# DRCL-USC/Hector_Simulation

Measured on NVIDIA H100. Metric: QP solves/sec (batched MPC ticks), horizon N=10, higher is better.
Workload: dtype f32 assembly (bit-exact to reference arithmetic) / f64 solve

## Files before the change

### hector_simulation_b200/csrc/hmpc_capi.cu

```cuda
#include <cuda_runtime.h>
#include <dlfcn.h>
#include <unistd.h>

#include <algorithm>
#include <chrono>
#include <cstddef>
#include <cstdint>
#include <cstdio>
#include <cstdlib>
#include <atomic>
#include <condition_variable>
#include <cstring>
#include <ctime>
#include <functional>
#include <mutex>
#include <string>
#include <thread>
#include <vector>

#include "../../include/hector_mpc_b200.h"
#include "hmpc_device.cuh"
#include "hmpc_chain.h"

static_assert(sizeof(update_data_t) == 3016, "update_data_t must match convexMPC_interface.h:19-37");
static_assert(sizeof(problem_setup) == 16, "problem_setup must match convexMPC_interface.h:11-17");

namespace {

thread_local std::string g_err;

bool cuda_fail(cudaError_t e, const char* what)
{
  if (e == cudaSuccess) return false;
  g_err = std::string(what) + ": " + cudaGetErrorString(e);
  return true;
}
#define CK(call)                          \
  do {                                    \
    if (cuda_fail((call), #call)) return HMPC_ERR_CUDA; \
  } while (0)

class HostPool {
 public:
  explicit HostPool(int nworkers)
  {
    for (int i = 0; i < nworkers; i++) workers_.emplace_back([this, i] { run(i); });
  }
  ~HostPool()
  {
    {
      std::lock_guard<std::mutex> lk(m_);
      stop_ = true;
      gen_++;
    }
    cv_.notify_all();
    for (auto& t : workers_) t.join();
  }
  int size() const { return (int)workers_.size() + 1; }
  void parallel(const std::function<void(int, int)>& fn)
  {
    const int np = size();
    if (np == 1) { fn(0, 1); return; }
    fn_ = &fn;
    pending_.store(np - 1, std::memory_order_release);
    {
      std::lock_guard<std::mutex> lk(m_);
      gen_++;
    }
    cv_.notify_all();
    fn(0, np);
    while (pending_.load(std::memory_order_acquire) != 0) std::this_thread::yield();
  }

 private:
  void run(int idx)
  {
    unsigned seen = 0;
    for (;;) {
      bool got = false;
      const auto t0 = std::chrono::steady_clock::now();
      while (std::chrono::steady_clock::now() - t0 < std::chrono::microseconds(50)) {
        if (gen_relaxed() != seen) { got = true; break; }
      }
      if (!got) {
        std::unique_lock<std::mutex> lk(m_);
        cv_.wait(lk, [&] { return gen_ != seen; });
      }
      {
        std::lock_guard<std::mutex> lk(m_);
        seen = gen_;
        if (stop_) return;
      }
      (*fn_)(idx + 1, size());
      pending_.fetch_sub(1, std::memory_order_acq_rel);
    }
  }
  unsigned gen_relaxed()
  {
    std::lock_guard<std::mutex> lk(m_);
    return gen_;
  }
  std::vector<std::thread> workers_;
  std::mutex m_;
  std::condition_variable cv_;
  unsigned gen_ = 0;
  bool stop_ = false;
  const std::function<void(int, int)>* fn_ = nullptr;
  std::atomic<int> pending_{0};
};

constexpr int NCHUNK = 4;

constexpr int EAGER_SLOT = 0, CAPTURE_SLOT = 1, CLS_SLOTS = 2;
static_assert(CAPTURE_SLOT < CLS_SLOTS, "d_cls holds CLS_SLOTS slots");

struct ResultRows { float* wrench; int* status; float* tau; size_t bytes; };

using hmpc::ClassCfg;

}

struct hmpc_ctx {
  int device = 0, max_batch = 0, horizon = 0, rec_stride = 0, sm_count = 0;
  hmpc::SolverSettings cfg;
  ClassCfg cls[3];
  int ncls = 0;
  ClassCfg ref{};
  ClassCfg mcls[3], mref{};
  float* d_mq = nullptr;
  size_t mq_off[4] = {};
  unsigned char* h_multi = nullptr;
  float* d_smtraj = nullptr;
  unsigned char* h_smulti = nullptr;
  int* d_ref = nullptr;
  unsigned char* d_rec = nullptr;
  unsigned char* d_out = nullptr;
  int* d_status = nullptr;
  int* d_counts = nullptr;
  int* d_lists = nullptr;
  int* d_cls = nullptr;
  unsigned char* h_mask = nullptr;
  unsigned eager_calls = 0;
  unsigned char* h_rec = nullptr;
  unsigned char* h_out = nullptr;
  unsigned char* d_states = nullptr;
  unsigned char* h_states = nullptr;
  int* h_cls = nullptr;
  cudaStream_t stream = nullptr;
  cudaStream_t xstream[3] = {nullptr, nullptr, nullptr};
  HostPool* pool = nullptr;
  void* nccl = nullptr;
  int shard_rank = 0, shard_world = 1;
  float* shard_buf[2] = {nullptr, nullptr};
  unsigned shard_tick = 0;
  cudaStream_t gstream = nullptr;
  cudaEvent_t solved = nullptr, gathered[2] = {nullptr, nullptr};
  int* d_ws = nullptr;
  int warm_start = 1;
  int* d_shift = nullptr;
  int* h_shift = nullptr;
  double* h_pred = nullptr;
  unsigned char* h_cert = nullptr;
  struct Pin { char* base; size_t bytes; };
  struct Run { uintptr_t lo, hi; };
  std::vector<Pin> pins;
  std::vector<Run> runs;
  bool pinned(const void* p, size_t bytes) const
  {
    const char* q = static_cast<const char*>(p);
    for (const Pin& r : pins)
      if (q >= r.base && q + bytes <= r.base + r.bytes) return true;
    return false;
  }
  size_t row_bytes() const { return (size_t)12 * horizon * 4 + 4 + 40; }
  ResultRows rows(unsigned char* base, int b0, int nb, bool tau = true) const
  {
    const size_t nw = (size_t)12 * horizon;
    unsigned char* p = base + (size_t)b0 * row_bytes();
    return {reinterpret_cast<float*>(p), reinterpret_cast<int*>(p + (size_t)nb * nw * 4),
            tau ? reinterpret_cast<float*>(p + (size_t)nb * (nw * 4 + 4)) : nullptr, (size_t)nb * (nw * 4 + 4 + (tau ? 40 : 0))};
  }
};

namespace {

cudaError_t prep_class(const ClassCfg& c, int* occ)
{
  cudaError_t e = cudaErrorInvalidDeviceFunction;
#define HMPC_PREP(ID, NT, MB, NF, CL) HMPC_PREP_K(ID, (hmpc::hmpc_solve_kernel<NT, MB, NF, CL>), NT)
#define HMPC_PREP_MQ(ID, NT, MB, NF, CL) HMPC_PREP_K(ID, (hmpc::hmpc_solve_kernel<NT, MB, NF, CL, true>), NT)
#define HMPC_PREP_K(ID, KERNEL, NT)                                                                    \
  case ID: {                                                                                           \
    auto k = KERNEL;                                                                                   \
    e = cudaFuncSetAttribute(k, cudaFuncAttributeMaxDynamicSharedMemorySize, 227 * 1024);              \
    if (e == cudaSuccess) e = cudaOccupancyMaxActiveBlocksPerMultiprocessor(occ, k, NT, c.smem);       \
    break;                                                                                             \
  }
  switch (c.variant) { HMPC_VARIANTS(HMPC_PREP) HMPC_MQ_VARIANTS(HMPC_PREP_MQ) }
#undef HMPC_PREP
#undef HMPC_PREP_MQ
#undef HMPC_PREP_K
  return e;
}

bool pdl_enabled()
{
  static const bool on = !(getenv("HMPC_PDL") && atoi(getenv("HMPC_PDL")) == 0);
  return on;
}

template <typename... KArgs, typename... Args>
cudaError_t launch_chain(void (*kernel)(KArgs...), dim3 grid, dim3 block, size_t smem, cudaStream_t st, bool pdl, Args... args)
{
  cudaLaunchConfig_t cfg{};
  cfg.gridDim = grid;
  cfg.blockDim = block;
  cfg.dynamicSmemBytes = smem;
  cfg.stream = st;
  cudaLaunchAttribute attr[1];
  attr[0].id = cudaLaunchAttributeProgrammaticStreamSerialization;
  attr[0].val.programmaticStreamSerializationAllowed = 1;
  cfg.attrs = attr;
  cfg.numAttrs = pdl ? 1 : 0;
  return cudaLaunchKernelEx(&cfg, kernel, args...);
}

int build_classes(hmpc_ctx* c)
{
  c->ncls = hmpc::plan_classes(c->horizon, c->cls, c->ref);
  if (c->ncls == 0 || hmpc::plan_classes(c->horizon, c->mcls, c->mref, true) != c->ncls) {
    g_err = "horizon too long for the built kernel variants";
    return HMPC_ERR_ARG;
  }
  size_t mq_rows = 0;
  for (int i = 0; i <= 2 * c->ncls + 1; i++) {
    const bool mq = i > c->ncls;
    const int j = mq ? i - c->ncls - 1 : i;
    ClassCfg& k = mq ? (j < c->ncls ? c->mcls[j] : c->mref) : (j < c->ncls ? c->cls[j] : c->ref);
    int occ = 0;
    if (cuda_fail(prep_class(k, &occ), "kernel attribute/occupancy (is this an sm_90a device?)")) return HMPC_ERR_CUDA;
    if (occ < 1) { g_err = "kernel does not fit on this device"; return HMPC_ERR_CUDA; }
    k.grid_cap = occ * c->sm_count;
    if (mq) {
      c->mq_off[j < c->ncls ? j : 3] = mq_rows * hmpc::mq_scratch_floats(c->horizon);
      mq_rows += hmpc::mq_scratch_ctas(k, c->max_batch);
    }
  }
  if (cuda_fail(cudaMalloc(&c->d_mq, mq_rows * hmpc::mq_scratch_floats(c->horizon) * sizeof(float)), "cudaMalloc multi-query scratch"))
    return HMPC_ERR_CUDA;
  return HMPC_OK;
}

long long* g_dbg_clk = nullptr;

int launch_class(const hmpc_ctx* c, int cls, const hmpc::SolveIO& io, const hmpc::ChainLists& lists, int count, cudaStream_t st,
                 bool pdl = false, const hmpc::MultiIO* mq = nullptr)
{
  const ClassCfg& k = cls == hmpc::REFINE_CLASS ? (mq ? c->mref : c->ref) : (mq ? c->mcls[cls] : c->cls[cls]);
  hmpc::KernelArgs ka = mq ? hmpc::multi_launch_args(c->cfg, c->horizon, c->ncls, cls, k, io, lists, *mq)
                           : hmpc::launch_args(c->cfg, c->horizon, c->ncls, cls, k, io, lists);
  ka.dbg_clk = ka.dbg_H ? nullptr : g_dbg_clk;
  const int grid = count < k.grid_cap ? count : k.grid_cap;
  cudaError_t e = cudaErrorInvalidDeviceFunction;
#define HMPC_LAUNCH(ID, NT, MB, NF, CL) \
  case ID: e = launch_chain(hmpc::hmpc_solve_kernel<NT, MB, NF, CL>, dim3(grid), dim3(NT), (size_t)k.smem, st, pdl, ka); break;
#define HMPC_LAUNCH_MQ(ID, NT, MB, NF, CL) \
  case ID: e = launch_chain(hmpc::hmpc_solve_kernel<NT, MB, NF, CL, true>, dim3(grid), dim3(NT), (size_t)k.smem, st, pdl, ka); break;
  switch (k.variant) { HMPC_VARIANTS(HMPC_LAUNCH) HMPC_MQ_VARIANTS(HMPC_LAUNCH_MQ) }
#undef HMPC_LAUNCH
#undef HMPC_LAUNCH_MQ
  CK(e);
  CK(cudaGetLastError());
  return HMPC_OK;
}

int launch_prepare(const hmpc::PrepareArgs& pa, cudaStream_t st, bool pdl)
{
  CK(launch_chain(hmpc::hmpc_prepare_kernel, dim3(hmpc::prepare_grid(pa.batch)), dim3(hmpc::PREPARE_THREADS), 0, st, pdl,
                  pa.states, pa.batch, pa.N, pa.dtMPC, pa.records, pa.rec_stride, pa.list, pa.count));
  CK(cudaGetLastError());
  return HMPC_OK;
}

int launch_prepare_traj(const hmpc::PrepareTrajArgs& pa, cudaStream_t st, bool pdl)
{
  CK(launch_chain(hmpc::hmpc_prepare_traj_kernel, dim3(hmpc::prepare_grid(pa.batch * pa.K)), dim3(hmpc::PREPARE_THREADS), 0, st,
                  pdl, pa.states, pa.batch, pa.K, pa.cmd, pa.N, pa.dtMPC, pa.traj, pa.list, pa.count));
  CK(cudaGetLastError());
  return HMPC_OK;
}

int launch_carry(const unsigned char* mask, int batch, int N, const float* prev, float* cur, cudaStream_t st)
{
  hmpc::hmpc_carry_kernel<<<hmpc::carry_grid(batch, N), hmpc::CARRY_THREADS, 0, st>>>(
      mask, batch, hmpc::carry_row_vecs(N), reinterpret_cast<const float4*>(prev), reinterpret_cast<float4*>(cur));
  CK(cudaGetLastError());
  return HMPC_OK;
}

template <typename T>
int launch_predict(const hmpc_ctx* c, const void* rows, int row_stride, int B, const unsigned char* mask, const T* wrench,
                   T* pred, cudaStream_t st)
{
  hmpc::hmpc_predict_kernel<T><<<hmpc::predict_grid(B), hmpc::PREDICT_THREADS, 0, st>>>(
      static_cast<const unsigned char*>(rows), row_stride, B, c->horizon, c->cfg.dt, mask, wrench, pred);
  CK(cudaGetLastError());
  return HMPC_OK;
}

template <typename T>
int launch_certify(const hmpc_ctx* c, const void* rows, hmpc::RowLayout lay, int B, const unsigned char* mask, const T* wrench,
                   hmpc_certificate_t* cert, T* lambda, cudaStream_t st)
{
  hmpc::hmpc_certify_kernel<T><<<hmpc::certify_grid(B), hmpc::CERT_THREADS, 0, st>>>(
      static_cast<const unsigned char*>(rows), lay, B, c->horizon, c->cfg.dt, c->cfg.f_max, mask, wrench,
      reinterpret_cast<hmpc::CertOut*>(cert), lambda, nullptr);
  CK(cudaGetLastError());
  return HMPC_OK;
}

template <typename T>
int launch_multi_cost(const hmpc_ctx* c, const void* rows, hmpc::RowLayout lay, int B, int K, const unsigned char* mask,
                      const float* traj, const T* wrench, double* cost, cudaStream_t st)
{
  hmpc::hmpc_multi_cost_kernel<T><<<hmpc::multi_cost_grid((long long)B * K), hmpc::PREDICT_THREADS, 0, st>>>(
      static_cast<const unsigned char*>(rows), lay, B, K, c->horizon, c->cfg.dt, mask, traj, wrench, cost);
  CK(cudaGetLastError());
  return HMPC_OK;
}

template <typename T>
int launch_pick(const hmpc_ctx* c, void* records, int B, int K, const unsigned char* mask, const float* traj, const T* wrench,
                const int* status, const double* cost, int* best, float* tau, cudaStream_t st)
{
  hmpc::hmpc_pick_kernel<T><<<hmpc::pick_grid(B), hmpc::PREDICT_THREADS, 0, st>>>(
      static_cast<unsigned char*>(records), c->rec_stride, B, K, c->horizon, c->cfg.f_max, mask, traj, wrench, status, cost, best,
      tau);
  CK(cudaGetLastError());
  return HMPC_OK;
}

}

static_assert(sizeof(hmpc_certificate_t) == sizeof(hmpc::CertOut) && offsetof(hmpc_certificate_t, flags) ==
              offsetof(hmpc::CertOut, flags), "hmpc_certificate_t is the kernel's CertOut");
static_assert(HMPC_CERT_PASS == hmpc::CERT_PASS && HMPC_CERT_NONFINITE == hmpc::CERT_NONFINITE &&
              HMPC_CERT_SWING == hmpc::CERT_SWING && HMPC_CERT_STATIONARITY == hmpc::CERT_STATIONARITY &&
              HMPC_CERT_PRIMAL == hmpc::CERT_PRIMAL && HMPC_CERT_COMPLEMENTARITY == hmpc::CERT_COMPL,
              "certificate flag bits");
static_assert(HMPC_CERT_STATIONARITY_TOL == hmpc::CERT_STAT_TOL && HMPC_CERT_PRIMAL_TOL == hmpc::CERT_PRIMAL_TOL &&
              HMPC_CERT_COMPLEMENTARITY_TOL == hmpc::CERT_COMPL_TOL, "certificate thresholds");
static_assert(sizeof(update_data_t) == 3016 && offsetof(update_data_t, Alpha_K) == 1896 && offsetof(update_data_t, traj) == 168 &&
              offsetof(update_data_t, gait) == 1944, "hmpc_chain.h: update_rows");

HMPC_EXTERNC size_t hmpc_record_bytes(int horizon)
{
  if (horizon < 1 || horizon > 18) return 0;
  size_t b = (size_t)(54 + 12 * horizon) * 4 + (size_t)2 * horizon;
  return (b + 15) / 16 * 16;
}

HMPC_EXTERNC int hmpc_pack_records(const update_data_t* in, int n, int horizon, void* out)
{
  const size_t stride = hmpc_record_bytes(horizon);
  if (!in || !out || n < 0 || stride == 0) { g_err = "hmpc_pack_records: bad argument"; return HMPC_ERR_ARG; }
  unsigned char* o = static_cast<unsigned char*>(out);
  for (int i = 0; i < n; i++, o += stride) {
    const update_data_t& u = in[i];
    if (i + 2 < n) {
      const char* nx = reinterpret_cast<const char*>(&in[i + 2]);
      for (int off = 0; off < (42 + 12 * horizon) * 4; off += 64) __builtin_prefetch(nx + off);
      __builtin_prefetch(nx + offsetof(update_data_t, Alpha_K));
      __builtin_prefetch(nx + offsetof(update_data_t, gait));
    }
    float* f = reinterpret_cast<float*>(o);
    memcpy(f, u.p, 42 * 4);
    memcpy(f + 42, u.Alpha_K, 48);
    memcpy(f + 54, u.traj, (size_t)48 * horizon);
    unsigned char* g = o + (size_t)(54 + 12 * horizon) * 4;
    memcpy(g, u.gait, (size_t)2 * horizon);
    memset(g + 2 * horizon, 0, stride - ((size_t)(54 + 12 * horizon) * 4 + 2 * horizon));
  }
  return HMPC_OK;
}

HMPC_EXTERNC const char* hmpc_last_error(void) { return g_err.c_str(); }

struct Id128 { char b[128]; };
namespace {
struct NcclApi {
  void* h = nullptr;
  int (*GetUniqueId)(void*) = nullptr;
  int (*CommInitRank)(void**, int, Id128, int) = nullptr;
  int (*AllGather)(const void*, void*, size_t, int, void*, cudaStream_t) = nullptr;
  int (*CommDestroy)(void*) = nullptr;
  const char* (*GetErrorString)(int) = nullptr;
};
}
namespace {
NcclApi g_nccl;
bool nccl_load()
{
  if (g_nccl.h) return true;
  void* h = dlopen("libnccl.so.2", RTLD_NOW | RTLD_GLOBAL);
  if (!h) h = dlopen("libnccl.so", RTLD_NOW | RTLD_GLOBAL);
  if (!h) { g_err = std::string("NCCL not found: ") + dlerror(); return false; }
  g_nccl.GetUniqueId = reinterpret_cast<int (*)(void*)>(dlsym(h, "ncclGetUniqueId"));
  g_nccl.CommInitRank = reinterpret_cast<int (*)(void**, int, Id128, int)>(dlsym(h, "ncclCommInitRank"));
  g_nccl.AllGather = reinterpret_cast<int (*)(const void*, void*, size_t, int, void*, cudaStream_t)>(dlsym(h, "ncclAllGather"));
  g_nccl.CommDestroy = reinterpret_cast<int (*)(void*)>(dlsym(h, "ncclCommDestroy"));
  g_nccl.GetErrorString = reinterpret_cast<const char* (*)(int)>(dlsym(h, "ncclGetErrorString"));
// ... 155 lines not shown
  if (!bad) {
    const char* br = getenv("HMPC_BLOCK_ROUNDS");
    if (br) c->cfg.block_rounds = atoi(br);
    if (const char* bm = getenv("HMPC_BLOCK_MIN")) c->cfg.block_min = atoi(bm);
    if (const char* km = getenv("HMPC_KAPPA_MAX")) c->cfg.kappa_max = atof(km);
    if (const char* kr = getenv("HMPC_KAPPA_REFINE")) c->cfg.kappa_refine = atof(kr);
    if (const char* kx = getenv("HMPC_KAPPA_MAX_REFINED")) c->cfg.kappa_max_refined = atof(kx);
    const char* ls = getenv("HMPC_LOCKSTEP");
    if (ls) c->cfg.lockstep = atoi(ls);
    const char* wm = getenv("HMPC_WARM_START");
    if (wm) c->warm_start = atoi(wm);
  }
  if (!bad && max_batch >= 256) {
    const char* e = getenv("HMPC_HOST_THREADS");
    int nt = e ? atoi(e) : 4;
    const int hw = (int)std::thread::hardware_concurrency();
    if (hw > 0 && nt > hw) nt = hw;
    if (nt > 1) c->pool = new HostPool(nt - 1);
  }
  if (bad) {
    std::string keep = g_err;
    hmpc_destroy(c);
    g_err = keep;
    return nullptr;
  }
  return c;
}

HMPC_EXTERNC int hmpc_set_problem(hmpc_ctx* c, const problem_setup* s)
{
  if (!c || !s) { g_err = "hmpc_set_problem: null argument"; return HMPC_ERR_ARG; }
  if (s->horizon != c->horizon) { g_err = "hmpc_set_problem: horizon differs from the context's"; return HMPC_ERR_ARG; }
  c->cfg.dt = s->dt;
  c->cfg.f_max = s->f_max;
  return HMPC_OK;
}

namespace {
int enqueue_solve(hmpc_ctx* c, const hmpc::SolveIO& io, cudaStream_t st, const hmpc::MultiIO* mq = nullptr)
{
  if (io.batch > c->max_batch) { g_err = "batch exceeds the context's capacity"; return HMPC_ERR_ARG; }
  CK(cudaSetDevice(c->device));
  cudaStreamCaptureStatus cap = cudaStreamCaptureStatusNone;
  CK(cudaStreamIsCapturing(st, &cap));
  const bool capturing = cap != cudaStreamCaptureStatusNone;
  const int slot = capturing ? CAPTURE_SLOT : EAGER_SLOT;
  const hmpc::ClassSlot s{c->d_cls + (size_t)slot * hmpc::ClassSlot::cls_slot_ints(c->max_batch), c->max_batch,
                          capturing ? 0 : (int)(c->eager_calls++ & 1u)};
  if (capturing) CK(cudaMemsetAsync(s.base, 0, hmpc::ClassSlot::HEAD_INTS * sizeof(int), st));
  const hmpc::ChainLists lists = hmpc::slot_lists(s, io.mask != nullptr, c->cfg.refine);
  const bool pdl = pdl_enabled();
  if (io.mask) {
    CK(launch_chain(hmpc::hmpc_select_kernel<hmpc::SELECT_THREADS>, dim3(1), dim3(hmpc::SELECT_THREADS), 0, st, pdl, io.mask,
                    io.batch, s.list0(), s.counts()));
    CK(cudaGetLastError());
  }
  if (io.states) {
    if (int rc = launch_prepare(hmpc::prepare_args(c->horizon, io, lists), st, pdl)) return rc;
    if (mq && mq->cmd)
      if (int rc = launch_prepare_traj(hmpc::prepare_traj_args(c->horizon, io, lists, *mq), st, pdl)) return rc;
  }
  const int items = mq ? io.batch * mq->K : io.batch;
  for (int i = 0; i < c->ncls; i++)
    if (int rc = launch_class(c, i, io, lists, i == 0 ? io.batch : items, st, pdl, mq)) return rc;
  if (c->cfg.refine) return launch_class(c, hmpc::REFINE_CLASS, io, lists, items, st, pdl, mq);
  return HMPC_OK;
}

hmpc::SolveIO device_call(const hmpc_ctx* c, const void* d_records, int B, float* d_wrench, int* d_status, float* d_tau, bool warm)
{
  hmpc::SolveIO io;
  io.records = d_records;
  io.batch = B;
  io.wrench = d_wrench;
  io.status = d_status;
  io.tau = d_tau;
  if (warm && c->warm_start) io.ws = c->d_ws, io.warm = true;
  return io;
}

struct Chunk { int b0, nb; cudaStream_t st; hmpc::SolveIO io; int *lists, *d_lists, *ref; };

int enqueue_solve_hostlists(hmpc_ctx* c, const Chunk& ch, bool zero_copy)
{
  int* h_block = ch.lists;
  int* d_block = zero_copy ? h_block : ch.d_lists;
  if (!zero_copy) {
    const size_t ints = h_block[1] > 0 ? hmpc::host_list(h_block, c->max_batch, 1) - h_block + h_block[1] : hmpc::HOST_LIST_HEAD + h_block[0];
    CK(cudaMemcpyAsync(d_block, h_block, ints * sizeof(int), cudaMemcpyHostToDevice, ch.st));
  }
  const hmpc::ChainLists lists = hmpc::host_lists(d_block, c->max_batch, ch.ref, false);
  if (ch.ref) CK(cudaMemsetAsync(lists.ref_count, 0, sizeof(int), ch.st));
  for (int i = 0; i < 2; i++)
    if (h_block[i] > 0)
      if (int rc = launch_class(c, i, ch.io, lists, h_block[i], ch.st)) return rc;
  return HMPC_OK;
}

int enqueue_overflow_retry(hmpc_ctx* c, const Chunk& ch, const int* h_status, const unsigned char* mask)
{
  const int mb = c->max_batch, nb = ch.nb;
  int* h_block = ch.lists;
  std::vector<char> was_cls1(nb, 0);
  for (int j = 0; j < h_block[1]; j++) was_cls1[hmpc::host_list(h_block, mb, 1)[j]] = 1;
  int n[3] = {0, 0, 0};
  for (int i = 0; i < nb; i++) {
    if ((mask && !mask[i]) || HMPC_STATUS_CODE(h_status[i]) != hmpc::ST_WS_CAP) continue;
    const int next = was_cls1[i] ? 2 : 1;
    if (next < c->ncls) hmpc::host_list(h_block, mb, next)[n[next]++] = i;
  }
  h_block[0] = 0;
  h_block[1] = n[1];
  h_block[2] = n[2];
  h_block[3] = 0;
  CK(cudaMemcpyAsync(ch.d_lists, h_block, (hmpc::host_list(h_block, mb, 2) - h_block + n[2]) * sizeof(int), cudaMemcpyHostToDevice, ch.st));
  const hmpc::ChainLists lists = hmpc::host_lists(ch.d_lists, mb, ch.ref, true);
  for (int i = 1; i < c->ncls; i++) {
    const int cnt = (i == 1) ? n[1] : n[1] + n[2];
    if (cnt > 0)
      if (int rc = launch_class(c, i, ch.io, lists, cnt, ch.st)) return rc;
  }
  return HMPC_OK;
}

int enqueue_refine_retry(hmpc_ctx* c, const Chunk& ch)
{
  return launch_class(c, hmpc::REFINE_CLASS, ch.io, hmpc::host_lists(ch.d_lists, c->max_batch, ch.ref, false), ch.nb, ch.st);
}
}

static int check_device_records(const hmpc_ctx* c, const void* d_records, int B, const char* who)
{
  if (B > c->max_batch) { g_err = std::string(who) + ": batch exceeds the context's capacity"; return HMPC_ERR_ARG; }
  if (reinterpret_cast<uintptr_t>(d_records) & 15u) { g_err = std::string(who) + ": d_records must be 16-byte aligned"; return HMPC_ERR_ARG; }
  return HMPC_OK;
}

HMPC_EXTERNC void hmpc_debug_set_clock_buffer(long long* d_buf) { g_dbg_clk = d_buf; }

namespace { int g_fail_next_solves = 0; }
HMPC_EXTERNC void hmpc_debug_fail_next_solves(int n) { g_fail_next_solves = n; }

HMPC_EXTERNC int hmpc_launches_per_solve(const hmpc_ctx* c) { return c ? c->ncls + (c->cfg.refine ? 1 : 0) : 0; }

HMPC_EXTERNC int hmpc_set_refinement(hmpc_ctx* c, int on)
{
  if (!c) { g_err = "hmpc_set_refinement: null context"; return HMPC_ERR_ARG; }
  c->cfg.refine = on ? 1 : 0;
  return HMPC_OK;
}

HMPC_EXTERNC int hmpc_class_config(const hmpc_ctx* c, int cls, int* out)
{
  if (!c || !out || cls < 0 || (cls >= c->ncls && cls != HMPC_REFINEMENT_CLASS)) return HMPC_ERR_ARG;
  const ClassCfg& k = cls == HMPC_REFINEMENT_CLASS ? c->ref : c->cls[cls];
  out[0] = k.threads; out[1] = k.smem; out[2] = k.qmax; out[3] = k.grid_cap; out[4] = k.nb_cap;
  out[5] = 8;
  return HMPC_OK;
}

HMPC_EXTERNC int hmpc_solve_device(hmpc_ctx* c, const void* d_records, int B, float* d_wrench, int* d_status,
                                   void* stream)
{
  if (!c || !d_records || !d_wrench || !d_status || B < 0) { g_err = "hmpc_solve_device: bad argument"; return HMPC_ERR_ARG; }
  if (B == 0) return HMPC_OK;
  if (int rc = check_device_records(c, d_records, B, "hmpc_solve_device")) return rc;
  return enqueue_solve(c, device_call(c, d_records, B, d_wrench, d_status, nullptr, false), static_cast<cudaStream_t>(stream));
}

HMPC_EXTERNC int hmpc_solve_device_ex(hmpc_ctx* c, const void* d_records, int B, float* d_wrench, int* d_status,
                                      float* d_tau, void* stream)
{
  if (!c || !d_records || !d_wrench || !d_status || B < 0) { g_err = "hmpc_solve_device_ex: bad argument"; return HMPC_ERR_ARG; }
  if (B == 0) return HMPC_OK;
  if (int rc = check_device_records(c, d_records, B, "hmpc_solve_device_ex")) return rc;
  return enqueue_solve(c, device_call(c, d_records, B, d_wrench, d_status, d_tau, false), static_cast<cudaStream_t>(stream));
}

HMPC_EXTERNC int hmpc_solve_device_warm(hmpc_ctx* c, const void* d_records, int B, float* d_wrench, int* d_status, float* d_tau,
                                        const int* d_shift, void* stream)
{
  if (!c || !d_records || !d_wrench || !d_status || B < 0) { g_err = "hmpc_solve_device_warm: bad argument"; return HMPC_ERR_ARG; }
  if (B == 0) return HMPC_OK;
  if (int rc = check_device_records(c, d_records, B, "hmpc_solve_device_warm")) return rc;
  hmpc::SolveIO io = device_call(c, d_records, B, d_wrench, d_status, d_tau, true);
  io.shifts = d_shift;
  return enqueue_solve(c, io, static_cast<cudaStream_t>(stream));
}

HMPC_EXTERNC int hmpc_solve_device_masked(hmpc_ctx* c, const void* d_records, int B, const unsigned char* d_mask, float* d_wrench,
                                          int* d_status, float* d_tau, const int* d_shift, void* stream)
{
  if (!c || !d_records || !d_mask || !d_wrench || !d_status || B < 0) {
    g_err = "hmpc_solve_device_masked: bad argument";
    return HMPC_ERR_ARG;
  }
  if (B == 0) return HMPC_OK;
  if (int rc = check_device_records(c, d_records, B, "hmpc_solve_device_masked")) return rc;
  hmpc::SolveIO io = device_call(c, d_records, B, d_wrench, d_status, d_tau, true);
  io.shifts = d_shift;
  io.mask = d_mask;
  return enqueue_solve(c, io, static_cast<cudaStream_t>(stream));
}

HMPC_EXTERNC int hmpc_assemble_device(hmpc_ctx* c, const void* d_records, int B, float* d_H, float* d_g,
                                      float* d_Fblk, float* d_lb, float* d_ub, void* stream)
{
  if (!c || !d_records || !d_H || !d_g || !d_Fblk || !d_lb || !d_ub || B < 0) {
    g_err = "hmpc_assemble_device: bad argument";
    return HMPC_ERR_ARG;
  }
  if (B == 0) return HMPC_OK;
  if (int rc = check_device_records(c, d_records, B, "hmpc_assemble_device")) return rc;
  CK(cudaSetDevice(c->device));
  hmpc::SolveIO io = device_call(c, d_records, B, nullptr, c->d_status, nullptr, false);
  io.dump_H = d_H;
  io.dump_g = d_g;
  io.dump_F = d_Fblk;
  io.dump_lb = d_lb;
  io.dump_ub = d_ub;
  hmpc::ChainLists lists;
  lists.counts = c->d_counts;
  return launch_class(c, c->ncls - 1, io, lists, B, static_cast<cudaStream_t>(stream));
}

static_assert(sizeof(hmpc_state_t) == 352 && offsetof(hmpc_state_t, gait) == 39 * 8, "hmpc_state_t layout (hmpc_prepare_kernel)");

HMPC_EXTERNC int hmpc_prepare_device(hmpc_ctx* c, const hmpc_state_t* d_states, int B, double dtMPC, void* d_records,
                                     void* stream)
{
  if (!c || !d_states || !d_records || B < 0) { g_err = "hmpc_prepare_device: bad argument"; return HMPC_ERR_ARG; }
  if (B == 0) return HMPC_OK;
  CK(cudaSetDevice(c->device));
  hmpc::SolveIO io;
  io.states = d_states;
  io.records = d_records;
  io.batch = B;
  io.dt_mpc = dtMPC;
  return launch_prepare(hmpc::prepare_args(c->horizon, io, hmpc::ChainLists{}), static_cast<cudaStream_t>(stream), false);
}

HMPC_EXTERNC int hmpc_solve_states_device_masked(hmpc_ctx* c, const hmpc_state_t* d_states, int B, const unsigned char* d_mask,
                                                 double dtMPC, void* d_records, float* d_wrench, int* d_status, float* d_tau,
                                                 const int* d_shift, void* stream)
{
  if (!c || !d_states || !d_mask || !d_records || !d_wrench || !d_status || B < 0) {
    g_err = "hmpc_solve_states_device_masked: bad argument";
    return HMPC_ERR_ARG;
  }
  if (B == 0) return HMPC_OK;
  if (int rc = check_device_records(c, d_records, B, "hmpc_solve_states_device_masked")) return rc;
  hmpc::SolveIO io = device_call(c, d_records, B, d_wrench, d_status, d_tau, true);
  io.shifts = d_shift;
  io.mask = d_mask;
  io.states = d_states;
  io.dt_mpc = dtMPC;
  return enqueue_solve(c, io, static_cast<cudaStream_t>(stream));
}

HMPC_EXTERNC int hmpc_predict_device(hmpc_ctx* c, const void* d_records, int B, const unsigned char* d_mask, const float* d_wrench,
                                     float* d_pred, void* stream)
{
  if (!c || !d_records || !d_wrench || !d_pred || B < 0 || B > c->max_batch) {
    g_err = "hmpc_predict_device: bad argument (null pointer or batch > capacity)";
    return HMPC_ERR_ARG;
  }
  if (B == 0) return HMPC_OK;
  CK(cudaSetDevice(c->device));
  return launch_predict(c, d_records, c->rec_stride, B, d_mask, d_wrench, d_pred, static_cast<cudaStream_t>(stream));
}

namespace { int g_predict_in_place = -1; }
HMPC_EXTERNC int hmpc_debug_last_predict_in_place(void) { return g_predict_in_place; }

HMPC_EXTERNC int hmpc_predict_batch(hmpc_ctx* c, const update_data_t* in, int B, const unsigned char* mask, const double* wrench,
                                    double* pred_out)
{
  if (!c || !in || !wrench || !pred_out || B < 0 || B > c->max_batch) {
    g_err = "hmpc_predict_batch: bad argument (null pointer or batch > capacity)";
    return HMPC_ERR_ARG;
  }
  if (B == 0) return HMPC_OK;
  if (mask && std::all_of(mask, mask + B, [](unsigned char m) { return m == 0; })) return HMPC_OK;
  CK(cudaSetDevice(c->device));
  const size_t nw = (size_t)12 * c->horizon, rs = (size_t)c->rec_stride;
  const unsigned char* m = nullptr;
  if (mask) {
    memcpy(c->h_mask, mask, (size_t)B);
    m = c->h_mask;
  }
  auto listed = [&](int i) { return !mask || mask[i] != 0; };
  if (c->pinned(in, (size_t)B * sizeof(update_data_t)) && c->pinned(wrench, B * nw * sizeof(double)) &&
      c->pinned(pred_out, B * nw * sizeof(double))) {
    g_predict_in_place = 1;
    if (int rc = launch_predict(c, in, (int)sizeof(update_data_t), B, m, wrench, pred_out, c->stream)) return rc;
    CK(cudaStreamSynchronize(c->stream));
    return HMPC_OK;
  }
  g_predict_in_place = 0;
  if (!c->h_pred) CK(cudaMallocHost(&c->h_pred, 2 * (size_t)c->max_batch * nw * sizeof(double)));
  double* hw = c->h_pred;
  double* hp = c->h_pred + (size_t)c->max_batch * nw;
  for (int i = 0; i < B; i++)
    if (listed(i)) {
      memcpy(c->h_rec + i * rs, in[i].p, 19 * sizeof(float));
      memcpy(hw + i * nw, wrench + i * nw, nw * sizeof(double));
    }
  if (int rc = launch_predict(c, c->h_rec, c->rec_stride, B, m, hw, hp, c->stream)) return rc;
// ... 835 lines not shown
```

### hector_simulation_b200/csrc/hmpc_chain.h

```cpp
#pragma once
#include <cstddef>

namespace hmpc {

constexpr int MQ_VARIANT = 100;
#define HMPC_VARIANTS(X) \
  X(0, 128, 6, 10, 0)    \
  X(1, 256, 2, 10, 1)    \
  X(20, 64, 1, 0, 3)     \
  X(21, 128, 1, 0, 3)    \
  X(22, 192, 1, 0, 3)    \
  X(23, 256, 1, 0, 3)    \
  X(24, 384, 1, 0, 3)    \
  X(10, 64, 8, 0, 0)     \
  X(11, 128, 6, 0, 0)    \
  X(12, 192, 3, 0, 0)    \
  X(13, 256, 2, 0, 0)    \
  X(14, 384, 1, 0, 0)    \
  X(15, 64, 8, 0, 1)     \
  X(16, 128, 6, 0, 1)    \
  X(17, 192, 3, 0, 1)    \
  X(18, 256, 2, 0, 1)    \
  X(19, 384, 1, 0, 1)
#define HMPC_MQ_VARIANTS(X) \
  X(100, 128, 6, 10, 0) \
  X(101, 256, 2, 10, 1) \
  X(120, 64, 1, 0, 3)   \
  X(121, 128, 1, 0, 3)  \
  X(122, 192, 1, 0, 3)  \
  X(123, 256, 1, 0, 3)  \
  X(124, 384, 1, 0, 3)  \
  X(110, 64, 8, 0, 0)   \
  X(111, 128, 6, 0, 0)  \
  X(112, 192, 3, 0, 0)  \
  X(113, 256, 2, 0, 0)  \
  X(114, 384, 1, 0, 0)  \
  X(115, 64, 8, 0, 1)   \
  X(116, 128, 6, 0, 1)  \
  X(117, 192, 3, 0, 1)  \
  X(118, 256, 2, 0, 1)  \
  X(119, 384, 1, 0, 1)

constexpr int REFINE_CLASS = 3;
constexpr int SMEM_MAX = 226 * 1024;

struct ClassCfg {
  int nb_hi, nb_cap, qmax, threads, smem, grid_cap, variant, tcap;
  Layout L;
};

inline int pick_variant(int N, int kcls, int warps, bool fixed, int* threads, bool mq = false)
{
  int v = -1;
#define HMPC_PICK(ID, NT, MB, NF, CL) \
  if (CL == kcls && NF == 0 && NT >= 32 * warps && (v < 0 || NT < *threads)) v = ID, *threads = NT;
  HMPC_VARIANTS(HMPC_PICK)
#undef HMPC_PICK
#define HMPC_PICK(ID, NT, MB, NF, CL) \
  if (CL == kcls && NF == N && fixed && v >= 0) v = ID, *threads = NT;
  HMPC_VARIANTS(HMPC_PICK)
#undef HMPC_PICK
  return (v >= 0 && mq) ? MQ_VARIANT + v : v;
}

inline int plan_classes(int N, ClassCfg cls[3], ClassCfg& ref, bool mq = false)
{
  const int rs = record_stride(N);
  for (int i = 0; i < 2; i++) {
    ClassCfg& k = cls[i];
    k = ClassCfg{};
    k.nb_cap = k.nb_hi = class_nb_cap(N, i);
    k.variant = pick_variant(N, i, class_warps(N, i), true, &k.threads, mq);
    if (k.variant < 0) return 0;
    k.qmax = class_qmax(N, i);
    k.tcap = class_tcap(N, i);
    k.L = make_layout(N, k.nb_cap, k.qmax, rs, k.threads / 32, k.tcap);
    k.smem = k.L.total;
  }
  ClassCfg& k = cls[2];
  k = cls[1];
  k.variant = pick_variant(N, 1, class_warps(N, 1), false, &k.threads, mq);
  k.qmax = 6 * k.nb_cap;
  k.tcap = 0;
  k.L = make_layout(N, k.nb_cap, k.qmax, rs, k.threads / 32, 0);
  while (k.L.total > SMEM_MAX && k.qmax > cls[1].qmax) {
    k.qmax -= 4;
    k.L = make_layout(N, k.nb_cap, k.qmax, rs, k.threads / 32, 0);
  }
  k.smem = k.L.total;
  const int ncls = k.qmax > cls[1].qmax ? 3 : 2;
  for (int nb = 2 * N;; nb = N) {
    ref = ClassCfg{};
    ref.nb_cap = ref.nb_hi = nb;
    ref.variant = pick_variant(N, REFINE_CLASS, class_warps(N, nb == N ? 0 : 1), false, &ref.threads, mq);
    if (ref.variant < 0) return 0;
    ref.qmax = 6 * nb;
    ref.L = refine_layout(N, nb, ref.qmax, rs, ref.threads / 32);
    while (ref.L.total > SMEM_MAX && ref.qmax > 4) {
      ref.qmax -= 4;
      ref.L = refine_layout(N, nb, ref.qmax, rs, ref.threads / 32);
    }
    ref.smem = ref.L.total;
    if (nb == N || (ref.L.total <= SMEM_MAX && ref.qmax >= class_qmax(N, 1))) break;
  }
  return ncls;
}

struct ClassSlot {
  enum : int { W_WAVE = 3, W_REF = 4, PARITY_INTS = 8, HEAD_INTS = 2 * PARITY_INTS };
  static_assert(W_REF < 5, "the class-0 launch clears 5 words of the next parity");
  int* base;
  int max_batch;
  int par;
  static size_t cls_slot_ints(int max_batch) { return HEAD_INTS + 4 * (size_t)max_batch; }
  int* counts() const { return base + PARITY_INTS * par; }
  int* counts_next() const { return base + PARITY_INTS * (par ^ 1); }
  unsigned* wave() const { return reinterpret_cast<unsigned*>(counts() + W_WAVE); }
  int* ref_count() const { return counts() + W_REF; }
  int* list(int i) const { return base + HEAD_INTS + (size_t)(i - 1) * max_batch; }
  int* ref_list() const { return list(3); }
  int* list0() const { return list(4); }
};

constexpr int HOST_LIST_HEAD = 4;
inline size_t host_lists_ints(int max_batch) { return HOST_LIST_HEAD + 3 * (size_t)max_batch; }
inline int* host_list(int* block, int max_batch, int i) { return block + HOST_LIST_HEAD + (size_t)i * max_batch; }

inline void classify_host(int N, float f_max, int nb_hi, const unsigned char* gait0, size_t gait_stride, int nb, int* block,
                          int max_batch, const unsigned char* mask = nullptr)
{
  for (int w = 0; w < HOST_LIST_HEAD; w++) block[w] = 0;
  for (int i = 0; i < nb; i++) {
    if (mask && !mask[i]) continue;
    int k = 0;
    for (int e = 0; e < 2 * N; e++) {
      const float ub = f_max * (float)gait0[(size_t)i * gait_stride + e];
      k += !(ub < 0.0001f && ub > -0.0001f);
    }
    const int cl = (k <= nb_hi) ? 0 : 1;
    host_list(block, max_batch, cl)[block[cl]++] = i;
  }
}

struct SolverSettings {
  float dt = 0.04f, f_max = 500.f;
  int max_iter = 500;
  double tol_kkt = 1e-9;
  double tol_dep = 1e-11;
  double kappa_max = 1.5e5;
  double kappa_refine = 1.5e4;
  double kappa_max_refined = 1e9;
  int refine = 0;
  int block_rounds = 4;
  int block_min = 2;
  int lockstep = 1;
};

struct SolveIO {
  const void* records = nullptr;
  const void* raw = nullptr;
  const void* states = nullptr;
  double dt_mpc = 0.0;
  int batch = 0;
  float* wrench = nullptr;
  double* wrench64 = nullptr;
  int* status = nullptr;
  float* tau = nullptr;
  int* ws = nullptr;
  bool warm = false;
  int shift = 1;
  const int* shifts = nullptr;
  const unsigned char* mask = nullptr;
  float *dump_H = nullptr, *dump_g = nullptr, *dump_F = nullptr, *dump_lb = nullptr, *dump_ub = nullptr;
};

struct ChainLists {
  int* counts = nullptr;
  int* list[3] = {};
  int* ref_count = nullptr;
  int* ref_list = nullptr;
  int* counts_next = nullptr;
  unsigned* wave = nullptr;
  bool escalate = false;
};

inline ChainLists slot_lists(const ClassSlot& s, bool masked, bool refine)
{
  ChainLists l;
  l.counts = s.counts();
  l.list[0] = masked ? s.list0() : nullptr;
  l.list[1] = s.list(1);
  l.list[2] = s.list(2);
  if (refine) l.ref_count = s.ref_count(), l.ref_list = s.ref_list();
  l.escalate = true;
  l.counts_next = s.counts_next();
  l.wave = s.wave();
  return l;
}

inline ChainLists host_lists(int* block, int max_batch, int* ref, bool escalate)
{
  ChainLists l;
  l.counts = block;
  for (int i = 0; i < 3; i++) l.list[i] = host_list(block, max_batch, i);
  if (ref) l.ref_count = ref, l.ref_list = ref + 1;
  l.escalate = escalate;
  return l;
}

constexpr int PREPARE_THREADS = 64;
inline int prepare_grid(int batch) { return (batch + PREPARE_THREADS - 1) / PREPARE_THREADS; }
struct PrepareArgs {
  const unsigned char* states;
  int batch, N;
  double dtMPC;
  unsigned char* records;
  int rec_stride;
  const int* list;
  const int* count;
};
inline PrepareArgs prepare_args(int N, const SolveIO& io, const ChainLists& lists)
{
  PrepareArgs pa{};
  pa.states = static_cast<const unsigned char*>(io.states);
  pa.batch = io.batch;
  pa.N = N;
  pa.dtMPC = io.dt_mpc;
  pa.records = static_cast<unsigned char*>(const_cast<void*>(io.records));
  pa.rec_stride = record_stride(N);
  pa.list = lists.list[0];
  pa.count = lists.list[0] ? lists.counts : nullptr;
  return pa;
}

inline int carry_row_vecs(int N) { return 3 * N; }
inline int carry_grid(int batch, int N)
{
  return (int)(((long long)batch * carry_row_vecs(N) + CARRY_THREADS - 1) / CARRY_THREADS);
}

inline int predict_grid(int batch)
{
  constexpr int warps = PREDICT_THREADS / 32;
  return (batch + warps - 1) / warps;
}

inline int certify_grid(int batch)
{
  constexpr int warps = CERT_THREADS / 32;
  return (batch + warps - 1) / warps;
}
inline RowLayout packed_rows(int N) { return RowLayout{record_stride(N), 42 * 4, 54 * 4, (54 + 12 * N) * 4}; }
inline RowLayout update_rows() { return RowLayout{3016, 1896, 168, 1944}; }

inline KernelArgs launch_args(const SolverSettings& S, int N, int ncls, int cls, const ClassCfg& k, const SolveIO& io,
                              const ChainLists& lists)
{
  const bool refinement = cls == REFINE_CLASS;
// ... 94 lines not shown
```

### hector_simulation_b200/csrc/hmpc_device.cuh

```cuda
#pragma once
#include <cuda_runtime.h>
#include <stdint.h>

namespace hmpc {

#define FM(a, b) __fmul_rn((a), (b))
#define FA(a, b) __fadd_rn((a), (b))
#define FS(a, b) __fsub_rn((a), (b))
#define FD(a, b) __fdiv_rn((a), (b))
#define DM(a, b) __dmul_rn((a), (b))
#define DA(a, b) __dadd_rn((a), (b))
#define DS(a, b) __dsub_rn((a), (b))

enum : int { ST_OK = 0, ST_ITER_CAP = 1, ST_WS_CAP = 2, ST_INFEASIBLE = 3, ST_NOT_SPD = 4 };

struct Layout {
  int H, gq, x0, nrm, fz, blk, keep, misc, uni;
  int T, Sv, lam, dv, rr, wsl, zb;
  int Pb, Ws;
  int rec, x0f, Acd, Bcd, P, M, dd, fbl, comb;
  int Hc, gc;
  int total;
};

__host__ __device__ constexpr int align16(int x) { return (x + 15) & ~15; }

__host__ __device__ constexpr int toff(int I, int J) { return (I * (I + 1) / 2 + J) * 64; }

__host__ __device__ constexpr Layout make_layout(int N, int nb_cap, int qmax, int rec_stride, int nwarps, int tcap)
{
  Layout L{};
  const int n = 6 * nb_cap;
  const int nt8 = (n + 7) / 8, ntile = nt8 * (nt8 + 1) / 2;
  int o = 0;
  L.H = o;    o += ntile * 64 * 8;
  L.gq = o;   o += nt8 * 8 * 8;
  L.x0 = o;   o += n * 8;
  L.nrm = o;  o += 2 * 10 * 6 * 8;
  L.fz = o;   o += align16(nb_cap * 8);
  L.blk = o;  o += align16((nb_cap + 2 * N) * 4);
  L.keep = o; o += 64;
  L.misc = o; o += 512;
  L.uni = o;
  int s = L.uni;
  const int ns = qmax + 1;
  L.T = s;    s += (tcap + 1) * n * 8;
  L.Sv = s;   s += ns * (ns + 1) / 2 * 8;
  L.lam = s;  s += ns * 8;
  L.dv = s;   s += 2 * (ns + 2) * 8;
  L.rr = s;   s += ns * 8;
  L.wsl = s;  s += align16(ns * 4);
  L.zb = L.gq;
  const int sweep_bytes = 2 * nt8 * 64 * 8 + nwarps * 2 * 64 * 8;
  int w = (sweep_bytes <= ntile * 64 * 8) ? L.H : L.uni;
  L.Pb = w;   w += 2 * nt8 * 64 * 8;
  L.Ws = w;   w += nwarps * 2 * 64 * 8;
  if (sweep_bytes <= ntile * 64 * 8) w = L.uni;
  int a = L.uni;
  L.rec = a;  a += align16(rec_stride);
  L.x0f = a;  a += 16 * 4;
  L.Acd = a;  a += align16(169 * 4);
  L.Bcd = a;  a += align16(156 * 4);
  L.P = a;    a += 2 * align16(169 * 4);
  L.M = a;    a += align16(N * 72 * 4);
  L.dd = a;   a += align16(12 * N * 4);
  L.fbl = a;  a += 192 * 4;
  L.comb = a; a += align16(4 * N * 4);
  int m = s > a ? s : a;
  m = m > w ? m : w;
  L.total = align16(m);
  return L;
}

__host__ __device__ constexpr Layout refine_layout(int N, int nb_cap, int qmax, int rec_stride, int nwarps)
{
  Layout L = make_layout(N, nb_cap, qmax, rec_stride, nwarps, 0);
  const int n = 6 * nb_cap, nt8 = (n + 7) / 8;
  L.Hc = L.total;
  L.gc = L.Hc + align16(nt8 * (nt8 + 1) / 2 * 64 * 4);
  L.total = align16(L.gc + n * 8);
  return L;
}

__host__ __device__ constexpr int record_stride(int N) { return align16((54 + 12 * N) * 4 + 2 * N); }

__host__ __device__ constexpr int class_nb_cap(int N, int cls) { return N * (1 + cls); }
__host__ __device__ constexpr int class_tcap(int N, int cls)
{
  const int n = 6 * class_nb_cap(N, cls);
  const int t = cls == 0 ? N + 4 : (N <= 10 ? 31 : 0);
  return t < n ? t : n;
}
__host__ __device__ constexpr int class_qmax(int N, int cls)
{
  const int n = 6 * class_nb_cap(N, cls);
  const int q = cls == 0 ? 2 * N + 4 : (N <= 10 ? 31 : 96);
  return q < n ? q : n;
}
__host__ __device__ constexpr int class_warps(int N, int cls)
{
  const int nb = class_nb_cap(N, cls), n = 6 * nb, nt8 = (n + 7) / 8;
  const int w_sweep = (nt8 + 1) / 2, w_rows = (nb + 2) / 3;
  return w_sweep > w_rows ? w_sweep : w_rows;
}
__host__ __device__ constexpr Layout class_layout(int N, int cls, int nwarps)
{
  return make_layout(N, class_nb_cap(N, cls), class_qmax(N, cls), record_stride(N), nwarps, class_tcap(N, cls));
}

struct KernelArgs {
  const unsigned char* records;
  const unsigned char* raw_records;
  int rec_stride;
  int batch;
  int horizon;
  float dt;
  float f_max;
  const int* list;
  int* counts;
  int cls;
  int* esc_list;
  int split_nb;
  int* ref_list;
  int* ref_count;
  int* counts_next;
  unsigned* wave_sync;
  int nb_cap;
  int qmax;
  int max_iter;
  double tol_kkt;
  double tol_dep;
  int tcap;
  int block_rounds;
  int block_min;
  double kappa_max;
  int warm_start;
  int ws_shift;
  const int* ws_shifts;
  int* ws_state;
  float* wrench;
  double* wrench64;
  int* status;
  float* dbg_H;
  float* dbg_g;
  float* dbg_F;
  float* dbg_lb;
  float* dbg_ub;
  float* tau;
  long long* dbg_clk;
  Layout L;
  const float* mq_traj;
  int mq_k;
  float* mq_scratch;
};

__host__ __device__ constexpr int mq_scratch_floats(int N) { return 16 + 172 + 156 + 12 + 72 * N; }

__device__ __forceinline__ uint32_t smem_u32(const void* p) { return (uint32_t)__cvta_generic_to_shared(p); }

__device__ __forceinline__ void pdl_trigger() { asm volatile("griddepcontrol.launch_dependents;" ::: "memory"); }
__device__ __forceinline__ void pdl_wait() { asm volatile("griddepcontrol.wait;" ::: "memory"); }

__device__ __forceinline__ void mbar_init(uint64_t* bar, int count)
{
  asm volatile("mbarrier.init.shared::cta.b64 [%0], %1;" ::"r"(smem_u32(bar)), "r"(count));
}
__device__ __forceinline__ void mbar_expect_tx(uint64_t* bar, uint32_t bytes)
{
  asm volatile("mbarrier.arrive.expect_tx.shared::cta.b64 _, [%0], %1;" ::"r"(smem_u32(bar)), "r"(bytes) : "memory");
}
__device__ __forceinline__ void mbar_wait(uint64_t* bar, uint32_t phase)
{
  asm volatile(
      "{\n\t.reg .pred p;\n\t"
      "WAIT_%=:\n\t"
      "mbarrier.try_wait.parity.shared::cta.b64 p, [%0], %1;\n\t"
      "@p bra DONE_%=;\n\t"
      "bra WAIT_%=;\n\t"
      "DONE_%=:\n\t}" ::"r"(smem_u32(bar)), "r"(phase) : "memory");
}
__device__ __forceinline__ void bulk_g2s(void* dst, const void* src, uint32_t bytes, uint64_t* bar)
{
  asm volatile("cp.async.bulk.shared::cluster.global.mbarrier::complete_tx::bytes [%0], [%1], %2, [%3];" ::"r"(
                   smem_u32(dst)),
               "l"(src), "r"(bytes), "r"(smem_u32(bar))
               : "memory");
}

__device__ __forceinline__ int leg_of(int c12) { return (c12 / 3) & 1; }
__device__ __forceinline__ int loc_of(int c12) { return (c12 % 3) + (c12 >= 6 ? 3 : 0); }
__device__ __forceinline__ int col12_of(int leg, int loc) { return (loc < 3) ? 3 * leg + loc : 6 + 3 * leg + (loc - 3); }

__device__ __forceinline__ void hput(float* Hf, int i, int j, float v)
{
  const int I = i >> 3, J = j >> 3;
  Hf[toff(I, J) + ((i & 7) << 3) + (j & 7)] = v;
  if (I == J) Hf[toff(I, I) + ((j & 7) << 3) + (i & 7)] = v;
}

__device__ __forceinline__ double hinv_dot6(const double* Hi, int i, int j0, const double* v)
{
  const int I = i >> 3, ir = i & 7;
  const int J0 = j0 >> 3, c0 = j0 & 7, J1 = J0 + 1;
  const int sA = (I >= J0) ? 1 : 8, sB = (I >= J1) ? 1 : 8;
  const double* pA = Hi + ((I >= J0) ? toff(I, J0) + ir * 8 + c0 : toff(J0, I) + c0 * 8 + ir);
  const double* pB = Hi + ((I >= J1) ? toff(I, J1) + ir * 8 : toff(J1, I) + ir) - (8 - c0) * sB;
  double acc = 0.0;
#pragma unroll
  for (int c = 0; c < 6; c++) acc = fma((c0 + c < 8) ? pA[c * sA] : pB[c * sB], v[c], acc);
  return acc;
}

__device__ __forceinline__ double hinv_rowdot(const double* Hi, int i, int nt8, const double* v)
{
  const int I = i >> 3, ir = i & 7;
  double acc0 = 0.0, acc1 = 0.0;
  for (int J = 0; J < nt8; J++) {
    const double* p = Hi + ((J <= I) ? toff(I, J) + ir * 8 : toff(J, I) + ir);
    const int st = (J <= I) ? 1 : 8;
    const double* vv = v + 8 * J;
#pragma unroll
    for (int c = 0; c < 8; c += 2) {
      acc0 = fma(p[c * st], vv[c], acc0);
      acc1 = fma(p[(c + 1) * st], vv[c + 1], acc1);
    }
  }
  return acc0 + acc1;
}

__device__ __forceinline__ double dot6(const double* a, const double* b)
{
  double acc = a[0] * b[0];
#pragma unroll
  for (int c = 1; c < 6; c++) acc = fma(a[c], b[c], acc);
  return acc;
}

__device__ __forceinline__ void dmma884(double& c0, double& c1, double a, double b)
{
  asm("mma.sync.aligned.m8n8k4.row.col.f64.f64.f64.f64 {%0,%1}, {%2}, {%3}, {%0,%1};" : "+d"(c0), "+d"(c1) : "d"(a), "d"(b));
}

__device__ __forceinline__ int frag_pair(int lane) { return ((lane & 2) << 4) + ((lane >> 2) << 2) + ((lane & 1) << 1); }
__device__ __forceinline__ int frag_elem(int r, int c) { return ((c >> 2) << 5) + (r << 2) + (c & 3); }

__device__ __forceinline__ float cof3(const float* m, int i, int j)
{
  int i1 = (i + 1) % 3, i2 = (i + 2) % 3, j1 = (j + 1) % 3, j2 = (j + 2) % 3;
  return FS(FM(m[i1 * 3 + j1], m[i2 * 3 + j2]), FM(m[i1 * 3 + j2], m[i2 * 3 + j1]));
}
__device__ inline void inverse3(const float* m, float* inv)
{
  float c00 = cof3(m, 0, 0), c10 = cof3(m, 1, 0), c20 = cof3(m, 2, 0);
  float det = FA(FA(FM(c00, m[0]), FM(c10, m[3])), FM(c20, m[6]));
  float id = FD(1.0f, det);
  inv[0] = FM(c00, id);
  inv[1] = FM(c10, id);
  inv[2] = FM(c20, id);
  inv[3] = FM(cof3(m, 0, 1), id);
  inv[4] = FM(cof3(m, 1, 1), id);
  inv[5] = FM(cof3(m, 2, 1), id);
  inv[6] = FM(cof3(m, 0, 2), id);
  inv[7] = FM(cof3(m, 1, 2), id);
  inv[8] = FM(cof3(m, 2, 2), id);
}
__device__ inline void mul3(const float* A, const float* B, float* C)
{
  for (int i = 0; i < 3; i++)
    for (int j = 0; j < 3; j++) {
      float acc = FM(A[i * 3], B[j]);
      acc = FA(acc, FM(A[i * 3 + 1], B[3 + j]));
      acc = FA(acc, FM(A[i * 3 + 2], B[6 + j]));
      C[i * 3 + j] = acc;
    }
}
__device__ inline void quat_to_R(const float* qq, float* R)
{
  float w = qq[0], x = qq[1], y = qq[2], z = qq[3];
  float tx = FM(2.f, x), ty = FM(2.f, y), tz = FM(2.f, z);
  float twx = FM(tx, w), twy = FM(ty, w), twz = FM(tz, w);
  float txx = FM(tx, x), txy = FM(ty, x), txz = FM(tz, x);
  float tyy = FM(ty, y), tyz = FM(tz, y), tzz = FM(tz, z);
  R[0] = FS(1.f, FA(tyy, tzz));
  R[1] = FS(txy, twz);
  R[2] = FA(txz, twy);
  R[3] = FA(txy, twz);
  R[4] = FS(1.f, FA(txx, tzz));
  R[5] = FS(tyz, twx);
  R[6] = FS(txz, twy);
  R[7] = FA(tyz, twx);
  R[8] = FS(1.f, FA(txx, tyy));
}

__device__ __noinline__ void sincos_f64(double x, double* s, double* c) { sincos(x, s, c); }
__device__ __noinline__ double fmod_f64(double x, double y) { return fmod(x, y); }
__device__ __noinline__ double atan2_f64(double y, double x) { return atan2(y, x); }
__device__ __noinline__ double asin_f64(double x) { return asin(x); }

__device__ inline void foot_rotation(const double* sc, float* Rf)
{
  const double s0 = sc[0], c0 = sc[1], s1 = sc[2], c1 = sc[3], s2 = sc[4], c2 = sc[5], s3 = sc[6], c3 = sc[7], s4 = sc[8],
               c4 = sc[9], s234 = sc[10], c234 = sc[11];
  double a = DA(DM(c0, s2), DM(DM(c2, s0), s1));
  double b = DS(DM(c0, c2), DM(DM(s0, s1), s2));
  double c = DA(DM(c2, s0), DM(DM(c0, s1), s2));
  double d = DS(DM(s0, s2), DM(DM(c0, c2), s1));
  double c3a_s3b = DA(DM(c3, a), DM(s3, b));
  double s3a_c3b = DS(DM(s3, a), DM(c3, b));
  double c3c_s3d = DS(DM(c3, c), DM(s3, d));
  double s3c_c3d = DA(DM(s3, c), DM(c3, d));
  Rf[0] = (float)DS(DM(-s4, c3a_s3b), DM(c4, s3a_c3b));
  Rf[1] = (float)DM(-c1, s0);
  Rf[2] = (float)DS(DM(c4, c3a_s3b), DM(s4, s3a_c3b));
  Rf[3] = (float)DS(DM(c4, c3c_s3d), DM(s4, s3c_c3d));
  Rf[4] = (float)DM(c0, c1);
  Rf[5] = (float)DA(DM(c4, s3c_c3d), DM(s4, c3c_s3d));
  Rf[6] = (float)DM(-s234, c1);
  Rf[7] = (float)s1;
  Rf[8] = (float)DM(c234, c1);
}

__device__ inline void role_leg(const float* rf, int lane, float* Fblk, unsigned char* scr)
{
  const double PI = 3.14159265359;
  float* qf = reinterpret_cast<float*>(scr);
  double* sc = reinterpret_cast<double*>(scr + 48);
  if (lane < 10) {
    const int i = lane % 5;
    float q = rf[19 + lane];
    if (i == 2) q = (float)DA((double)q, DM(0.3, PI));
    if (i == 3) q = (float)DS((double)q, DM(0.6, PI));
    if (i == 4) q = (float)DA((double)q, DM(0.3, PI));
    q = (float)fmod_f64((double)q, DM(2.0, PI));
    qf[lane] = q;
    sincos_f64((double)q, sc + 12 * (lane / 5) + 2 * i, sc + 12 * (lane / 5) + 2 * i + 1);
  }
  __syncwarp();
  if (lane >= 2) return;
  const int leg = lane;
  const float* q = qf + 5 * leg;
  const float q234 = FA(FA(q[2], q[3]), q[4]);
  sincos_f64((double)q234, sc + 12 * leg + 10, sc + 12 * leg + 11);
  float R[9], Rf[9];
  quat_to_R(rf + 6, R);
  foot_rotation(sc + 12 * leg, Rf);
  const float mu = 2.0f, lt = 0.09f, lh = 0.06f;
  const int r0 = 8 * leg, cF = 3 * leg, cM = 6 + 3 * leg;
  Fblk[(r0 + 0) * 12 + cF + 0] = -mu; Fblk[(r0 + 0) * 12 + cF + 2] = 1.f;
  Fblk[(r0 + 1) * 12 + cF + 0] = mu;  Fblk[(r0 + 1) * 12 + cF + 2] = 1.f;
  Fblk[(r0 + 2) * 12 + cF + 1] = -mu; Fblk[(r0 + 2) * 12 + cF + 2] = 1.f;
  Fblk[(r0 + 3) * 12 + cF + 1] = mu;  Fblk[(r0 + 3) * 12 + cF + 2] = 1.f;
  float v1t[3] = {FM(-lt, Rf[2]), FM(-lt, Rf[5]), FM(-lt, Rf[8])};
  float v1h[3] = {FM(-lh, Rf[2]), FM(-lh, Rf[5]), FM(-lh, Rf[8])};
  for (int j = 0; j < 3; j++) {
    float xw = FA(FA(FM(Rf[0], R[j * 3]), FM(Rf[3], R[j * 3 + 1])), FM(Rf[6], R[j * 3 + 2]));
    float yw = FA(FA(FM(Rf[1], R[j * 3]), FM(Rf[4], R[j * 3 + 1])), FM(Rf[7], R[j * 3 + 2]));
    float zt = FA(FA(FM(v1t[0], R[j * 3]), FM(v1t[1], R[j * 3 + 1])), FM(v1t[2], R[j * 3 + 2]));
    float zh = FA(FA(FM(v1h[0], R[j * 3]), FM(v1h[1], R[j * 3 + 1])), FM(v1h[2], R[j * 3 + 2]));
    Fblk[(r0 + 4) * 12 + cM + j] = xw;
    Fblk[(r0 + 5) * 12 + cF + j] = zt;
    Fblk[(r0 + 5) * 12 + cM + j] = yw;
    Fblk[(r0 + 6) * 12 + cF + j] = zh;
    Fblk[(r0 + 6) * 12 + cM + j] = (leg == 0) ? -yw : yw;
  }
  Fblk[(r0 + 7) * 12 + cF + 2] = 2.f;
}
__device__ inline void role_state(const float* rf, float dt, float* x0f, float* Acd, int lane, unsigned char* scr)
{
  float* rpy = reinterpret_cast<float*>(scr);
  double* sc = reinterpret_cast<double*>(scr + 16);
  if (lane < 3) {
    const float qw = rf[6], qx = rf[7], qy = rf[8], qz = rf[9];
    if (lane == 0) {
      rpy[0] = (float)atan2_f64((double)FM(2.f, FA(FM(qw, qx), FM(qy, qz))), DS(1.0, (double)FM(2.f, FA(FM(qx, qx), FM(qy, qy)))));
    } else if (lane == 1) {
      double as_d = DM(2.0, (double)FS(FM(qw, qy), FM(qx, qz)));
      if (!(as_d < .99999)) as_d = .99999;
      const float as = (float)as_d;
      rpy[1] = (float)asin_f64((double)as);
    } else {
      rpy[2] = (float)atan2_f64((double)FM(2.f, FA(FM(qw, qz), FM(qx, qy))), DS(1.0, (double)FM(2.f, FA(FM(qy, qy), FM(qz, qz)))));
    }
  }
  __syncwarp();
  if (lane < 2) sincos_f64((double)rpy[1 + lane], sc + 2 * lane, sc + 2 * lane + 1);
  __syncwarp();
  if (lane != 0) return;
// ... 383 lines not shown
        rel = fmin(fmax(rel, -0.4), 0.4);
        feet[3 * leg + a] = np_[a] + R[a * 3] * hip[0] + R[a * 3 + 1] * hip[1] + R[a * 3 + 2] * hip[2] + rel;
      }
      feet[3 * leg + 2] = 0.0;
    }
  }
  for (int st = 0; st < N; st++)
    for (int leg = 0; leg < 2; leg++) gait[2 * st + leg] = (unsigned char)gait_contact(it + st, N, li[leg], li[2 + leg]);
  for (int leg = 0; leg < 2; leg++) {
    const double hip[3] = {-0.005, leg == 0 ? -0.057 : 0.057, -0.126};
    const double d0 = feet[3 * leg] - np_[0], d1 = feet[3 * leg + 1] - np_[1], d2 = feet[3 * leg + 2] - np_[2];
    for (int a = 0; a < 3; a++) lp[3 * leg + a] = R[a] * d0 + R[3 + a] * d1 + R[6 + a] * d2 - hip[a];
  }
}

__device__ __forceinline__ double bezier_f64(double y0, double yf, double x)
{
  const double b = DA(DM(DM(x, x), x), DM(3.0, DM(DM(x, x), DS(1.0, x))));
  return DA(y0, DM(b, DS(yf, y0)));
}
__device__ __forceinline__ double clamp_f64(double v, double lo, double hi) { return fmax(lo, fmin(v, hi)); }
__device__ __forceinline__ double dot3_rn(double a0, double b0, double a1, double b1, double a2, double b2)
{
  return DA(DA(DM(a0, b0), DM(a1, b1)), DM(a2, b2));
}
__global__ void hmpc_swing_kernel(const unsigned char* states, const unsigned char* loop, const double* phase,
                                  unsigned char* swing, int batch, int n_iterations, double dt, double dtSwing,
                                  unsigned char* cmd)
{
  const int i = blockIdx.x * blockDim.x + threadIdx.x;
  if (i >= batch) return;
  const double* s = reinterpret_cast<const double*>(states + (size_t)i * 352);
  const double* pos = s; const double* vw = s + 3; const double* qt = s + 6;
  const double* lq = s + 16; const double* lp = s + 26; const double* sd = s + 32;
  const int* li = reinterpret_cast<const int*>(loop + (size_t)i * 80 + 48);
  double* sw_p0 = reinterpret_cast<double*>(swing + (size_t)i * 72);
  double* sw_time = sw_p0 + 6;
  int* sw_first = reinterpret_cast<int*>(swing + (size_t)i * 72 + 64);
  double* out = reinterpret_cast<double*>(cmd + (size_t)i * 232);
  int* out_swing = reinterpret_cast<int*>(cmd + (size_t)i * 232 + 224);
  for (int k = 0; k < 28; k++) out[k] = 0.0;
  out_swing[0] = out_swing[1] = 0;
  double R[9];
  quat_to_R_f64(qt, R);
  const double hipy[2] = {-0.057, 0.057};
  double pfw[2][3];
  for (int leg = 0; leg < 2; leg++) {
    const double hp0 = DA(-0.005, lp[3 * leg]), hp1 = DA(hipy[leg], lp[3 * leg + 1]), hp2 = DA(-0.126, lp[3 * leg + 2]);
    for (int a = 0; a < 3; a++) pfw[leg][a] = DA(pos[a], dot3_rn(R[a * 3], hp0, R[a * 3 + 1], hp1, R[a * 3 + 2], hp2));
    pfw[leg][2] = 0.0;
  }
  double sst[2];
  for (int leg = 0; leg < 2; leg++) {
    const double offp = __ddiv_rn((double)li[leg], (double)n_iterations);
    const double durp = __ddiv_rn((double)li[2 + leg], (double)n_iterations);
    double so = DA(offp, durp);
    if (so > 1) so = DS(so, 1.);
    const double sdur = DS(1., durp);
    double pr = DS(phase[i], so);
    if (pr < 0) pr = DA(pr, 1.);
    if (pr > sdur) pr = 0.;
    else pr = __ddiv_rn(pr, sdur);
    sst[leg] = pr;
  }
  const int g_stance = li[2], g_swing = n_iterations - li[2];
  for (int leg = 0; leg < 2; leg++) {
    if (sw_first[leg]) {
      sw_time[leg] = DM(dtSwing, (double)g_swing);
    } else {
      sw_time[leg] = DS(sw_time[leg], dt);
      if (sw_time[leg] <= 0) sw_first[leg] = 1;
    }
  }
  double vdw[3];
  for (int a = 0; a < 3; a++) vdw[a] = dot3_rn(R[a * 3], sd[2], R[a * 3 + 1], sd[3], R[a * 3 + 2], 0.0);
  double Pf[2][3];
  for (int leg = 0; leg < 2; leg++) {
    for (int a = 0; a < 3; a++)
      Pf[leg][a] = DA(DA(pos[a], dot3_rn(R[a * 3], -0.005, R[a * 3 + 1], hipy[leg], R[a * 3 + 2], -0.126)), DM(vw[a], sw_time[leg]));
    for (int a = 0; a < 2; a++) {
      const double rel = DA(DM(DM(DM(DM(1.75, vw[a]), 0.5), (double)g_stance), dtSwing), DM(0.1, DS(vw[a], vdw[a])));
      const float relf = fminf(fmaxf((float)rel, -(float)0.3), (float)0.3);
      Pf[leg][a] = DA(Pf[leg][a], (double)relf);
    }
    Pf[leg][2] = 0.0;
    for (int a = 0; a < 3; a++) out[3 * leg + a] = Pf[leg][a];
  }
  const double PI = 3.14159265358979323846;
  for (int leg = 0; leg < 2; leg++) {
    if (!(sst[leg] > 0)) continue;
    out_swing[leg] = 1;
    if (sw_first[leg]) {
      sw_first[leg] = 0;
      for (int a = 0; a < 3; a++) sw_p0[3 * leg + a] = pfw[leg][a];
    }
    const double ph = sst[leg], height = 0.15;
    const double* p0 = sw_p0 + 3 * leg;
    double pd[3];
    for (int a = 0; a < 2; a++) pd[a] = bezier_f64(p0[a], Pf[leg][a], ph);
    pd[2] = (ph < 0.5) ? bezier_f64(p0[2], DA(p0[2], height), DM(ph, 2.0)) : bezier_f64(DA(p0[2], height), Pf[leg][2], DS(DM(ph, 2.0), 1.0));
    const double side_w = (leg == 1) ? 1.0 : -1.0;
    const double hoff[3] = {-0.015, DM(side_w, -0.055), 0.0};
    const double d0 = DS(pd[0], pos[0]), d1 = DS(pd[1], pos[1]), d2 = DS(pd[2], pos[2]);
    double pb[3];
    for (int a = 0; a < 3; a++) {
      pb[a] = DA(dot3_rn(R[a], d0, R[3 + a], d1, R[6 + a], d2), hoff[a]);
      out[6 + 3 * leg + a] = pb[a];
      out[12 + 3 * leg + a] = dot3_rn(R[a], DS(0.0, vw[0]), R[3 + a], DS(0.0, vw[1]), R[6 + a], DS(0.0, vw[2]));
    }
    const double side = (leg == 0) ? -1.0 : 1.0;
    const double f0 = DS(pb[0], DS(0.0465, 0.06)), f1 = DS(pb[1], 0.0), f2 = DS(pb[2], DA(-0.126, DM(-0.0705, 2.0)));
    const double d3 = sqrt(DA(DA(DM(f0, f0), DM(f1, f1)), DM(f2, f2)));
    const double dyz = sqrt(DA(DM(f1, f1), DM(f2, f2)));
    const double dh = 0.0205;
    const double dv_ = sqrt(fmax(0.00001, DS(DM(dyz, dyz), DM(dh, dh))));
    const double dxz = sqrt(DS(DM(d3, d3), DM(dh, dh)));
    const double a1 = clamp_f64(__ddiv_rn(dxz, DM(2.0, 0.22)), -1.0, 1.0);
    const double a2 = clamp_f64(__ddiv_rn(dv_, dxz), -1.0, 1.0);
    double divisor = fabs(f0);
    divisor = (divisor == 0.0) ? 1e-6 : divisor;
    double* q = out + 18 + 5 * leg;
    q[0] = 0.0;
    q[1] = DA(asin(clamp_f64(__ddiv_rn(f1, dyz), -1.0, 1.0)), asin(clamp_f64(__ddiv_rn(DM(dh, side), dyz), -1.0, 1.0)));
    q[2] = DS(acos(a1), __ddiv_rn(DM(acos(a2), f0), divisor));
    q[3] = DS(DM(2.0, asin(clamp_f64(__ddiv_rn(__ddiv_rn(dxz, 2.0), 0.22), -1.0, 1.0))), PI);
    q[4] = DS(-lq[5 * leg + 3], lq[5 * leg + 2]);
    q[2] = DS(q[2], DM(0.3, PI));
    q[3] = DA(q[3], DM(0.6, PI));
    q[4] = DS(q[4], DM(0.3, PI));
  }
}

#ifdef HMPC_WARP_STAMPS
#define HMPC_STAMP(i) do { } while (0)
#define HMPC_WSTAMP(e) do { if (ka.dbg_clk && lane == 0 && wid < 4 && k == HMPC_WARP_STAMPS) ka.dbg_clk[(size_t)inst * 32 + wid * 8 + (e)] = clock64(); } while (0)
#else
#define HMPC_STAMP(i) do { if (ka.dbg_clk && tid == 0) ka.dbg_clk[(size_t)inst * 32 + (i)] = clock64(); } while (0)
#define HMPC_WSTAMP(e) do { } while (0)
#endif
constexpr int WS_STATE_INTS = 40;

__device__ __forceinline__ int mq_robot(int ent, int K, bool items) { return !items ? ent : (ent < 0 ? -1 - ent : ent / K); }
__device__ __forceinline__ int mq_first(int ent, int K, bool items) { return (items && ent >= 0) ? ent % K : 0; }
__device__ __forceinline__ int mq_end(int ent, int K, bool items) { return (items && ent >= 0) ? ent % K + 1 : K; }

template <int NT, int MINB, int NF, int CLS, bool MQ = false>
__global__ void __launch_bounds__(NT, MINB) hmpc_solve_kernel(const KernelArgs ka)
{
  extern __shared__ __align__(16) unsigned char smem[];
  const int tid = threadIdx.x;
  const int lane = tid & 31, wid = tid >> 5;
  constexpr int NW = NT / 32;
  constexpr bool FIX = NF > 0;
  const int N = FIX ? NF : ka.horizon;
  const int nb_cap = FIX ? class_nb_cap(NF, CLS) : ka.nb_cap;
  const int qmax = FIX ? class_qmax(NF > 0 ? NF : 1, CLS) : ka.qmax;
  const int rec_stride = FIX ? record_stride(NF) : ka.rec_stride;
  const int tcap = FIX ? class_tcap(NF > 0 ? NF : 1, CLS) : ka.tcap;
  Layout L;
  if constexpr (FIX) {
    constexpr Layout LC = class_layout(NF, CLS, NW);
    L = LC;
  } else {
    L = ka.L;
  }
  const bool dump = (ka.dbg_H != nullptr);

  float* Hf = reinterpret_cast<float*>(smem + L.H);
  double* Hd = reinterpret_cast<double*>(smem + L.H);
  double* gq = reinterpret_cast<double*>(smem + L.gq);
  double* x0 = reinterpret_cast<double*>(smem + L.x0);
  double* nrm = reinterpret_cast<double*>(smem + L.nrm);
  double* fz = reinterpret_cast<double*>(smem + L.fz);
  int* blk_sl = reinterpret_cast<int*>(smem + L.blk);
  int* sl_blk = blk_sl + nb_cap;
  unsigned* redk = reinterpret_cast<unsigned*>(smem + L.misc);
  int* redi = reinterpret_cast<int*>(smem + L.misc + 128);
  double* redv = reinterpret_cast<double*>(smem + L.misc + 256);
  int* flags = reinterpret_cast<int*>(smem + L.misc + 384);
  uint64_t* bar = reinterpret_cast<uint64_t*>(smem + L.misc + 448);
  double* dsc = reinterpret_cast<double*>(smem + L.misc + 456);
  unsigned* amask = reinterpret_cast<unsigned*>(smem + L.misc + 480);

  double* T = reinterpret_cast<double*>(smem + L.T);
  double* Sv = reinterpret_cast<double*>(smem + L.Sv);
  double* lam = reinterpret_cast<double*>(smem + L.lam);
  double* dvs = reinterpret_cast<double*>(smem + L.dv);
  double* rr = reinterpret_cast<double*>(smem + L.rr);
  int* wsl = reinterpret_cast<int*>(smem + L.wsl);
  double* zb = reinterpret_cast<double*>(smem + L.zb);

  unsigned char* rec = smem + L.rec;
  const float* rf = reinterpret_cast<const float*>(rec);
  float* x0f = reinterpret_cast<float*>(smem + L.x0f);
  float* Acd = reinterpret_cast<float*>(smem + L.Acd);
  float* Bcd = reinterpret_cast<float*>(smem + L.Bcd);
  float* Mb = reinterpret_cast<float*>(smem + L.M);
  float* dd = reinterpret_cast<float*>(smem + L.dd);
  float* Fblk = reinterpret_cast<float*>(smem + L.fbl);
  int* comb = reinterpret_cast<int*>(smem + L.comb);

  pdl_trigger();
  if (tid == 0) {
    mbar_init(bar, 1);
    asm volatile("fence.mbarrier_init.release.cluster;" ::: "memory");
  }
  __syncthreads();
  uint32_t phase = 0;
  pdl_wait();
  if (ka.counts_next && blockIdx.x == 0 && tid < 5) ka.counts_next[tid] = 0;
  const int count = ka.list ? ka.counts[ka.cls] : ka.batch;

  const int trips = (count + (int)gridDim.x - 1) / (int)gridDim.x;
  bool lockstep = ka.wave_sync != nullptr && trips > 2;
  for (int trip = 0; trip < trips; trip++) {
    const int idx = blockIdx.x + trip * gridDim.x;
    if (lockstep && trip > 0) {
      if (tid == 0) {
        __threadfence();
        atomicAdd(ka.wave_sync, 1u);
        const unsigned target = (unsigned)trip * gridDim.x;
        const long long t0 = clock64();
        bool ok = true;
        while (atomicAdd(ka.wave_sync, 0u) < target) {
          if (clock64() - t0 > 400000ll) { ok = false; break; }
        }
        flags[15] = ok ? 1 : 0;
      }
      __syncthreads();
      if (!flags[15]) lockstep = false;
      __syncthreads();
    }
    if (idx >= count) continue;
    const int inst = MQ ? mq_robot(ka.list ? ka.list[idx] : idx, ka.mq_k, CLS == 3 || ka.cls > 0)
                        : (ka.list ? ka.list[idx] : idx);
    const int k0 = MQ ? mq_first(ka.list ? ka.list[idx] : idx, ka.mq_k, CLS == 3 || ka.cls > 0) : 0;
    const int k1 = MQ ? mq_end(ka.list ? ka.list[idx] : idx, ka.mq_k, CLS == 3 || ka.cls > 0) : 1;
    HMPC_STAMP(0);
    const bool raw = ka.raw_records != nullptr;
    if (raw) {
      const unsigned char* src = ka.raw_records + (size_t)inst * 3016;
      const int nt = 6 * N, ng = (2 * N + 7) / 8;
      for (int e = tid; e < 27 + nt + ng; e += NT) {
        int so, dw;
        if (e < 21) { so = 8 * e; dw = e; }
        else if (e < 27) { so = 1896 + 8 * (e - 21); dw = e; }
        else if (e < 27 + nt) { so = 168 + 8 * (e - 27); dw = e; }
        else { so = 1944 + 8 * (e - 27 - nt); dw = e; }
        reinterpret_cast<uint2*>(rec)[dw] = *reinterpret_cast<const uint2*>(src + so);
      }
    } else if (tid == 0) {
      asm volatile("fence.proxy.async.shared::cta;" ::: "memory");
      mbar_expect_tx(bar, (uint32_t)rec_stride);
      bulk_g2s(rec, ka.records + (size_t)inst * rec_stride, (uint32_t)rec_stride, bar);
    }
    if (raw) {
      __syncthreads();
    } else {
      mbar_wait(bar, phase);
      phase ^= 1;
    }

    const unsigned char* gait = rec + (54 + 12 * N) * 4;
    if (wid == 0) {
      bool stance = false;
      if (lane < 2 * N) {
        const float ub = FM(ka.f_max, (float)gait[lane]);
        stance = !(ub < 0.0001f && ub > -0.0001f) || dump;
      }
      const unsigned mask = __ballot_sync(0xffffffffu, stance);
      const int k = __popc(mask & ((1u << lane) - 1u));
      if (lane < 2 * N) {
        sl_blk[lane] = (stance && k < nb_cap) ? k : -1;
        if (stance && k < nb_cap) {
          blk_sl[k] = lane;
          fz[k] = (double)FM(ka.f_max, (float)gait[lane]);
        }
      }
      unsigned st0 = 0, st1 = 0;
      for (int s = 0; s < N; s++) {
        st0 |= ((mask >> (2 * s)) & 1u) << s;
        st1 |= ((mask >> (2 * s + 1)) & 1u) << s;
      }
      int ncomb = 0;
      {
        int pk[2], km[2];
#pragma unroll
        for (int h = 0; h < 2; h++) {
          const int c = 32 * h + lane;
          const int li = (c / N) >> 1, lj = (c / N) & 1, delta = c % N;
          unsigned need = 0;
          if (c < 4 * N) need = (li ? st1 : st0) & ((lj ? st1 : st0) >> delta);
          km[h] = need ? N - 1 - delta - (__ffs(need) - 1) : -1;
          pk[h] = li | (lj << 1) | (delta << 2) | (km[h] << 8);
        }
        const unsigned lt = (1u << lane) - 1u;
        for (int v = N - 1; v >= 0; v--) {
#pragma unroll
          for (int h = 0; h < 2; h++) {
            const unsigned has = __ballot_sync(0xffffffffu, km[h] == v);
            if (km[h] == v) comb[ncomb + __popc(has & lt)] = pk[h];
            ncomb += __popc(has);
          }
        }
      }
      if (lane == 0) {
        flags[0] = __popc(mask);
        flags[1] = (int)st0;
        flags[2] = (int)st1;
        flags[3] = ST_OK;
        flags[6] = ncomb;
      }
    }
    if (tid < 14) reinterpret_cast<float*>(smem + L.keep)[tid] = (tid < 10) ? rf[19 + tid] : rf[6 + tid - 10];
    {
      constexpr int WL = (NW > 3) ? 3 : 0, W1 = (NW > 1) ? 1 : 0, W2 = (NW > 2) ? 2 : 0;
      unsigned char* scr = smem + L.P;
      if (wid == WL) {
        for (int e = lane; e < 192; e += 32) Fblk[e] = 0.f;
        __syncwarp();
        role_leg(rf, lane, Fblk, scr);
      }
      if (wid == W1) {
        for (int e = lane; e < 169; e += 32) Acd[e] = 0.f;
        __syncwarp();
        role_state(rf, ka.dt, x0f, Acd, lane, scr + 256);
      }
      if (wid == W2) {
        for (int e = lane; e < 156; e += 32) Bcd[e] = 0.f;
        __syncwarp();
        if (lane == 31) role_inertia(rf, ka.dt, Bcd);
      }
    }
    __syncthreads();
    const int NB = flags[0];
    if constexpr (CLS == 3) {
      if (NB > nb_cap) {
        __syncthreads();
        continue;
      }
    }
    if (ka.split_nb >= 0 && NB > ka.split_nb) {
      if (tid == 0) {
        const int slot = atomicAdd(&ka.counts[ka.cls + 1], 1);
        ka.esc_list[slot] = MQ ? -1 - inst : inst;
      }
      __syncthreads();
      continue;
    }
    const int n = 6 * NB, m = 10 * NB;
    const int NT8 = (n + 7) >> 3;
    const unsigned stmask[2] = {(unsigned)flags[1], (unsigned)flags[2]};

    for (int e = n + tid; e < 8 * NT8; e += NT) gq[e] = 0.0;
    __syncthreads();

    for (int e = tid; e < 2 * 10 * 6; e += NT) {
      const int leg = e / 60, t = (e / 6) % 10, c = e % 6;
      const int col = col12_of(leg, c);
      const int row = (t < 5) ? t : (t == 5 ? 4 : (t < 8 ? t - 1 : 7));
      const bool neg = (t == 5 || t == 6 || t == 7 || t == 9);
      const float v = Fblk[(8 * leg + row) * 12 + col];
      nrm[e] = (double)(neg ? -v : v);
    }

    float* const mqs = MQ ? ka.mq_scratch + (size_t)blockIdx.x * mq_scratch_floats(N) : nullptr;
    bool illc_h = false;
    int kq = k0;
  next_candidate:
    const bool first = kq == k0;
    const int row = MQ ? inst * ka.mq_k + kq : inst;
    const float* trj = MQ ? ka.mq_traj + (size_t)row * 12 * N : nullptr;
    if (MQ && !first) {
      float* wts = reinterpret_cast<float*>(rec) + 30;
      for (int e = tid; e < mq_scratch_floats(N); e += NT) {
        const float v = mqs[e];
        if (e < 16) x0f[e] = v;
        else if (e < 16 + 172) { if (e < 16 + 169) Acd[e - 16] = v; }
        else if (e < 344) Bcd[e - 188] = v;
        else if (e < 356) wts[e - 344] = v;
        else Mb[e - 356] = v;
      }
      __syncthreads();
    }

    HMPC_STAMP(1);
    for (int it = tid; it < 48; it += NT) {
      if (it < 36) {
        if (MQ && !first) continue;
        const int r = it / 12, c = it % 12;
        const float a0 = Acd[r * 13 + 6], a1 = Acd[r * 13 + 7], a2 = Acd[r * 13 + 8], ad = Acd[(3 + r) * 13 + 9 + r];
        const float b6 = Bcd[6 * 12 + c], b7 = Bcd[7 * 12 + c], b8 = Bcd[8 * 12 + c], b9 = Bcd[(9 + r) * 12 + c];
        float p0 = 0.f, p1 = 0.f, p2 = 0.f, pd = 0.f;
        float* dst = Mb + r * 12 + leg_of(c) * 6 + loc_of(c);
        for (int k = 0; k < N; k++) {
          dst[k * 72] = FA(FA(FM(p0, b6), FM(p1, b7)), FM(p2, b8));
          dst[k * 72 + 36] = FM(pd, b9);
          p0 = FA(a0, p0);
          p1 = FA(a1, p1);
          p2 = FA(a2, p2);
          pd = FA(ad, pd);
        }
      } else {
        const int r = it - 36;
        const float xr_ = x0f[r];
        if (r < 3) {
          const float a0 = Acd[r * 13 + 6], a1 = Acd[r * 13 + 7], a2 = Acd[r * 13 + 8];
          float p0 = 0.f, p1 = 0.f, p2 = 0.f;
          for (int s = 0; s < N; s++) {
            p0 = FA(a0, p0);
            p1 = FA(a1, p1);
            p2 = FA(a2, p2);
            const float acc = FA(FA(FA(xr_, FM(p0, x0f[6])), FM(p1, x0f[7])), FM(p2, x0f[8]));
            dd[12 * s + r] = FS(acc, (MQ ? trj[12 * s + r] : rf[54 + 12 * s + r]));
          }
        } else if (r < 6) {
          const float ad = Acd[r * 13 + r + 6], ag = Acd[11 * 13 + 12];
          float pd = 0.f, p5 = 0.f;
          for (int s = 0; s < N; s++) {
            p5 = FA(FM(pd, ag), p5);
            pd = FA(ad, pd);
            float acc = FA(xr_, FM(pd, x0f[r + 6]));
            if (r == 5) acc = FA(acc, FM(p5, x0f[12]));
            dd[12 * s + r] = FS(acc, (MQ ? trj[12 * s + r] : rf[54 + 12 * s + r]));
          }
        } else {
          const float ag = Acd[11 * 13 + 12];
          float p11 = 0.f;
          for (int s = 0; s < N; s++) {
            p11 = FA(ag, p11);
            const float acc = (r == 11) ? FA(xr_, FM(p11, x0f[12])) : xr_;
            dd[12 * s + r] = FS(acc, (MQ ? trj[12 * s + r] : rf[54 + 12 * s + r]));
          }
        }
      }
    }
    __syncthreads();
    if (MQ && first && k1 - k0 > 1) {
      for (int e = tid; e < mq_scratch_floats(N); e += NT) {
        float v = 0.f;
        if (e < 16) v = x0f[e];
        else if (e < 16 + 172) { if (e < 16 + 169) v = Acd[e - 16]; }
        else if (e < 344) v = Bcd[e - 188];
        else if (e < 356) v = rf[30 + e - 344];
        else v = Mb[e - 356];
        mqs[e] = v;
      }
    }

    HMPC_STAMP(2);
    if (dump) {
      float* oF = ka.dbg_F + (size_t)inst * 192;
      for (int e = tid; e < 192; e += NT) oF[e] = Fblk[e];
      float* olb = ka.dbg_lb + (size_t)inst * 16 * N;
      float* oub = ka.dbg_ub + (size_t)inst * 16 * N;
      for (int e = tid; e < 16 * N; e += NT) {
        const int s = e / 16, r = e % 16, leg = r / 8, rr_ = r % 8;
        float lo = 0.f, hi = 0.f;
        if (rr_ < 4) hi = (float)5e10;
        else if (rr_ == 4) hi = 0.01f;
        else if (rr_ < 7) lo = (float)(-5e10);
        else hi = FM(ka.f_max, (float)gait[2 * s + leg]);
        olb[e] = lo;
        oub[e] = hi;
      }
    }
    {
      float wr[12];
#pragma unroll
      for (int r = 0; r < 12; r++) wr[r] = rf[30 + r];
      const int nitems = (!MQ || first) ? flags[6] * 6 : 0;
      for (int chunk = wid; chunk * 32 < nitems; chunk += NW) {
        const int it = chunk * 32 + lane;
        if (it >= nitems) continue;
        const int cm = comb[it / 6], ci = it % 6;
        const int li = cm & 1, lj = (cm >> 1) & 1, delta = (cm >> 2) & 63, Kmax = cm >> 8;
        const unsigned need = stmask[li] & (stmask[lj] >> delta);
        const int ii = col12_of(li, ci);
        float acc[6] = {0.f, 0.f, 0.f, 0.f, 0.f, 0.f};
        float prod[3][6];
#pragma unroll
        for (int r = 0; r < 3; r++) {
          const float tv = FM(Bcd[(6 + r) * 12 + ii], wr[6 + r]);
#pragma unroll
          for (int c = 0; c < 6; c++) prod[r][c] = FM(tv, Bcd[(6 + r) * 12 + col12_of(lj, c)]);
        }
        const bool fax = ci < 3;
        const int rax = fax ? ci : 0;
        const float w3 = rf[30 + 3 + rax];
        const float prod9 = FM(FM(Bcd[(9 + rax) * 12 + ii], rf[30 + 9 + rax]), Bcd[(9 + rax) * 12 + col12_of(lj, rax)]);
        for (int K = 0; K <= Kmax; K++) {
          const float* Mi = Mb + (K + delta) * 72 + 6 * li + ci;
          const float2* Mj = reinterpret_cast<const float2*>(Mb + K * 72 + 6 * lj);
          float mi[3];
          float2 mj[3][3];
#pragma unroll
          for (int r = 0; r < 3; r++) {
            mi[r] = Mi[r * 12];
            mj[r][0] = Mj[r * 6];
            mj[r][1] = Mj[r * 6 + 1];
            mj[r][2] = Mj[r * 6 + 2];
          }
          const float m3i = Mi[(3 + rax) * 12];
          const float m3j = Mb[K * 72 + (3 + rax) * 12 + 6 * lj + rax];
#pragma unroll
          for (int r = 0; r < 3; r++) {
            const float tv = FM(mi[r], wr[r]);
            acc[0] = FA(acc[0], FM(tv, mj[r][0].x));
            acc[1] = FA(acc[1], FM(tv, mj[r][0].y));
            acc[2] = FA(acc[2], FM(tv, mj[r][1].x));
            acc[3] = FA(acc[3], FM(tv, mj[r][1].y));
            acc[4] = FA(acc[4], FM(tv, mj[r][2].x));
            acc[5] = FA(acc[5], FM(tv, mj[r][2].y));
          }
          if (fax) {
            const float t3 = FM(FM(m3i, w3), m3j);
#pragma unroll
            for (int c = 0; c < 3; c++) acc[c] = (c == rax) ? FA(acc[c], t3) : acc[c];
          }
#pragma unroll
          for (int r = 0; r < 3; r++)
#pragma unroll
            for (int c = 0; c < 6; c++) acc[c] = FA(acc[c], prod[r][c]);
          if (fax) {
#pragma unroll
            for (int c = 0; c < 3; c++) acc[c] = (c == rax) ? FA(acc[c], prod9) : acc[c];
          }
          const int a = N - 1 - K - delta, b = a + delta;
          if ((need >> a) & 1u) {
            if (!dump && delta > 0) {
              const int col = 6 * sl_blk[2 * a + li] + ci, row0 = 6 * sl_blk[2 * b + lj];
              const int I0 = row0 >> 3, r0 = row0 & 7, Jc = col >> 3, cb = col & 7;
              float* t0 = Hf + toff(I0, Jc);
              float* t1 = t0 + (I0 + 1) * 64;
#pragma unroll
              for (int cj = 0; cj < 6; cj++) {
                const float hv = FM(2.f, FA(acc[cj], 0.f));
                const int r = r0 + cj;
                float* t = (r < 8) ? t0 : t1;
                t[((r & 7) << 3) + cb] = hv;
                if (((r < 8) ? I0 : I0 + 1) == Jc) t[(cb << 3) + (r & 7)] = hv;
              }
            } else {
              const int ka_ = dump ? 0 : sl_blk[2 * a + li], kb_ = dump ? 0 : sl_blk[2 * b + lj];
#pragma unroll
              for (int cj = 0; cj < 6; cj++) {
                const int jj = col12_of(lj, cj);
                if (delta == 0 && ii > jj) continue;
                const float alpha = (delta == 0 && ii == jj) ? rf[42 + ii] : 0.f;
                const float hv = FM(2.f, FA(acc[cj], alpha));
                if (dump) {
                  float* oH = ka.dbg_H + (size_t)inst * (144 * N * N);
                  oH[(size_t)(12 * a + ii) * (12 * N) + 12 * b + jj] = hv;
                  oH[(size_t)(12 * b + jj) * (12 * N) + 12 * a + ii] = hv;
                } else {
                  const int gi = 6 * ka_ + ci, gj = 6 * kb_ + cj;
                  hput(Hf, gi > gj ? gi : gj, gi > gj ? gj : gi, hv);
                }
              }
            }
          }
        }
      }
    HMPC_STAMP(7);
      for (int e = tid; e < N * 12; e += NT) {
        const int a = e / 12, ii = e % 12, li = leg_of(ii);
        if (!((stmask[li] >> a) & 1u)) continue;
        float acc = 0.f;
        float t6[6];
#pragma unroll
        for (int r = 0; r < 6; r++) t6[r] = FM(FM(Bcd[(6 + r) * 12 + ii], wr[6 + r]), 2.f);
        for (int s = a; s < N; s++) {
          const float* Mi = Mb + (s - a) * 72 + 6 * li + loc_of(ii);
          const float* dk = dd + 12 * s;
          float mi[6], dkr[12];
#pragma unroll
          for (int r = 0; r < 6; r++) mi[r] = Mi[r * 12];
#pragma unroll
          for (int r = 0; r < 12; r++) dkr[r] = dk[r];
#pragma unroll
          for (int r = 0; r < 6; r++) acc = FA(acc, FM(FM(FM(mi[r], wr[r]), 2.f), dkr[r]));
#pragma unroll
          for (int r = 0; r < 6; r++) acc = FA(acc, FM(t6[r], dkr[6 + r]));
        }
        if (dump) ka.dbg_g[(size_t)inst * 12 * N + e] = acc;
        else gq[6 * sl_blk[2 * a + li] + loc_of(ii)] = (double)acc;
      }
    }
    __syncthreads();
    if (dump) continue;

    if (NB == 0) {
      if constexpr (MQ) {
        const size_t r0 = (size_t)inst * ka.mq_k + kq;
        for (int e = tid; e < (k1 - kq) * 12 * N; e += NT) {
          if (ka.wrench) ka.wrench[r0 * 12 * N + e] = 0.f;
          if (ka.wrench64) ka.wrench64[r0 * 12 * N + e] = 0.0;
        }
        for (int e = tid; e < k1 - kq; e += NT) ka.status[r0 + e] = ST_OK;
      } else {
        for (int e = tid; e < 12 * N; e += NT) {
          if (ka.wrench) ka.wrench[(size_t)inst * 12 * N + e] = 0.f;
          if (ka.wrench64) ka.wrench64[(size_t)inst * 12 * N + e] = 0.0;
        }
        if (ka.tau && tid < 10) ka.tau[(size_t)inst * 10 + tid] = 0.f;
        if (tid == 0) {
          ka.status[inst] = ST_OK;
          if (ka.ws_state) ka.ws_state[(size_t)inst * WS_STATE_INTS] = 0;
        }
      }
      __syncthreads();
      continue;
    }
    if constexpr (CLS == 3) {
      float* Hc = reinterpret_cast<float*>(smem + L.Hc);
      double* gc = reinterpret_cast<double*>(smem + L.gc);
      if (!MQ || first)
        for (int e = tid; e < tri(NT8) * 64; e += NT) Hc[e] = Hf[e];
      for (int e = tid; e < n; e += NT) gc[e] = gq[e];
    }

    HMPC_STAMP(3);
    if (!MQ || first) {
      constexpr int TS = 2 * NW + 1;
      const int rA = wid, rB = NT8 - 1 - wid;
      const bool hasA = rA <= rB, hasB = rA < rB;
      const int g = lane >> 2, t4 = lane & 3;
      const int fp = frag_pair(lane);
      const int ft = frag_elem(2 * t4, g);
      double c0[TS], c1[TS];
#pragma unroll
      for (int t = 0; t < TS; t++) { c0[t] = 0.0; c1[t] = 0.0; }
      for (int i = tid; i < n; i += NT) x0[i] = (double)Hf[toff(i >> 3, i >> 3) + (i & 7) * 9];
      {
        const int i = 8 * rB + g, j = 2 * t4;
        const float* src = Hf + toff(rB, 0) + g * 8 + 2 * t4;
#pragma unroll
        for (int J = 0; J < 2 * NW; J++)
          if (hasB && J <= rB) {
            const float2 v = *reinterpret_cast<const float2*>(src + J * 64);
            c0[J] = (i < n && 8 * J + j < n) ? (double)v.x : (i == 8 * J + j ? 1.0 : 0.0);
            c1[J] = (i < n && 8 * J + j + 1 < n) ? (double)v.y : (i == 8 * J + j + 1 ? 1.0 : 0.0);
          }
      }
      {
        const int i = 8 * rA + g, j = 2 * t4;
        const float* src = Hf + toff(rA, 0) + g * 8 + 2 * t4;
#pragma unroll
        for (int J = 0; J < NW; J++)
          if (hasA && J <= rA) {
            const float2 v = *reinterpret_cast<const float2*>(src + J * 64);
            c0[TS - 1 - J] = (i < n && 8 * J + j < n) ? (double)v.x : (i == 8 * J + j ? 1.0 : 0.0);
            c1[TS - 1 - J] = (i < n && 8 * J + j + 1 < n) ? (double)v.y : (i == 8 * J + j + 1 ? 1.0 : 0.0);
          }
      }
      double* Pbuf = reinterpret_cast<double*>(smem + L.Pb);
      double* WsA = reinterpret_cast<double*>(smem + L.Ws) + wid * 128;
      double* WsB = WsA + 64;
      bool bad = false;
      __syncthreads();
      if (hasB) *reinterpret_cast<double2*>(Pbuf + rB * 64 + fp) = make_double2(c0[0], c1[0]);
      if (hasA) {
        double d0 = c0[TS - 1], d1 = c1[TS - 1];
        if (rA == 0) bad |= tile_inverse_spd(d0, d1, lane);
        *reinterpret_cast<double2*>(Pbuf + rA * 64 + fp) = make_double2(d0, d1);
      }
      __syncthreads();
      for (int k = 0; k < NT8; k++) {
        const double* pbl = Pbuf + (k & 1) * NT8 * 64 + lane;
        double* Pn = Pbuf + ((k + 1) & 1) * NT8 * 64;
        const int kn = k + 1;
        const bool genA = hasA && rA != k, genB = hasB && rB != k;
        double wA0 = 0.0, wA1 = 0.0, wB0 = 0.0, wB1 = 0.0;
        HMPC_WSTAMP(0);
        {
          const double di0 = pbl[k * 64], di1 = pbl[k * 64 + 32];
          if (genA) {
            double W0 = 0.0, W1 = 0.0;
            dmma884(W0, W1, pbl[rA * 64], di0);
            dmma884(W0, W1, pbl[rA * 64 + 32], di1);
            *reinterpret_cast<double2*>(WsA + fp) = make_double2(-W0, -W1);
          }
          if (genB) {
            double W0 = 0.0, W1 = 0.0;
            dmma884(W0, W1, pbl[rB * 64], di0);
            dmma884(W0, W1, pbl[rB * 64 + 32], di1);
            *reinterpret_cast<double2*>(WsB + fp) = make_double2(-W0, -W1);
          }
          __syncwarp();
          if (genA) { wA0 = WsA[lane]; wA1 = WsA[32 + lane]; }
          if (genB) { wB0 = WsB[lane]; wB1 = WsB[32 + lane]; }
        }
        if (k == 1) HMPC_STAMP(20);
        HMPC_WSTAMP(1);
        if (kn < NT8 && ((hasA && rA == kn) || (hasB && rB == kn))) {
          const bool inA = hasA && rA == kn;
          double d0 = 0.0, d1 = 0.0;
#pragma unroll
          for (int J = 0; J < 2 * NW; J++)
            if (J == kn) {
              if (J < NW && inA) { d0 = c0[TS - 1 - (J < NW ? J : 0)]; d1 = c1[TS - 1 - (J < NW ? J : 0)]; }
              else { d0 = c0[J]; d1 = c1[J]; }
            }
          dmma884(d0, d1, inA ? wA0 : wB0, pbl[kn * 64]);
          dmma884(d0, d1, inA ? wA1 : wB1, pbl[kn * 64 + 32]);
          bad |= tile_inverse_spd(d0, d1, lane);
          *reinterpret_cast<double2*>(Pn + kn * 64 + fp) = make_double2(d0, d1);
        }
        if (k == 1) HMPC_STAMP(21);
        HMPC_WSTAMP(2);
        {
          const int limA = genA ? rA : -1, limB = genB ? rB : -1;
          const int pubA = (hasA && rA > kn) ? kn : -1, pubB = (hasB && rB > kn) ? kn : -1;
          double* PnA = Pn + rA * 64 + fp;
          double* PnB = Pn + rB * 64 + fp;
#pragma unroll
          for (int J = 0; J < 2 * NW; J++) {
            if (J > limB && J > limA) break;
            const double p0 = pbl[J * 64], p1 = pbl[J * 64 + 32];
            if (J <= limB) {
              if (J == k) {
                const double2 d = *reinterpret_cast<const double2*>(WsB + fp);
                c0[J] = -d.x;
                c1[J] = -d.y;
              } else {
                dmma884(c0[J], c1[J], wB0, p0);
                dmma884(c0[J], c1[J], wB1, p1);
              }
              if (J == pubB) *reinterpret_cast<double2*>(PnB) = make_double2(c0[J], c1[J]);
            }
            if (J < NW && J <= limA) {
              constexpr int dummy = 0;
              const int sa = TS - 1 - (J < NW ? J : dummy);
              if (J == k) {
                const double2 d = *reinterpret_cast<const double2*>(WsA + fp);
                c0[sa] = -d.x;
                c1[sa] = -d.y;
              } else {
                dmma884(c0[sa], c1[sa], wA0, p0);
                dmma884(c0[sa], c1[sa], wA1, p1);
              }
              if (J == pubA) *reinterpret_cast<double2*>(PnA) = make_double2(c0[sa], c1[sa]);
            }
          }
        }
        if (k == 1) HMPC_STAMP(22);
        HMPC_WSTAMP(3);
        if ((hasB && rB == k) || (hasA && rA == k)) {
          const bool inA = hasA && rA == k;
          const double di0 = pbl[k * 64], di1 = pbl[k * 64 + 32];
          const double2 dk = *reinterpret_cast<const double2*>(Pbuf + (k & 1) * NT8 * 64 + k * 64 + fp);
#pragma unroll
          for (int J = 0; J < 2 * NW; J++) {
            if (J > k) break;
            double v0 = -dk.x, v1 = -dk.y;
            if (J < k) {
              v0 = 0.0;
              v1 = 0.0;
              dmma884(v0, v1, di0, pbl[J * 64]);
              dmma884(v0, v1, di1, pbl[J * 64 + 32]);
            }
            if (J < NW && inA) { c0[TS - 1 - (J < NW ? J : 0)] = v0; c1[TS - 1 - (J < NW ? J : 0)] = v1; }
            else { c0[J] = v0; c1[J] = v1; }
          }
        }
        if (kn < NT8 && ((hasB && rB == kn) || (hasA && rA == kn))) {
          const bool inA = hasA && rA == kn;
#pragma unroll
          for (int J = 0; J < 2 * NW; J++) {
            if (J >= kn) break;
            const double v0 = (J < NW && inA) ? c0[TS - 1 - (J < NW ? J : 0)] : c0[J];
            const double v1 = (J < NW && inA) ? c1[TS - 1 - (J < NW ? J : 0)] : c1[J];
            Pn[J * 64 + ft] = v0;
            Pn[J * 64 + ft + 4] = v1;
          }
        }
        if (k == 1) HMPC_STAMP(23);
        HMPC_WSTAMP(4);
        __syncthreads();
        HMPC_WSTAMP(5);
        if (k == 1) HMPC_STAMP(24);
        if (k == 0) HMPC_STAMP(19);
      }
      {
        double* dstB = Hd + toff(rB, 0) + g * 8 + 2 * t4;
        double* dstA = Hd + toff(rA, 0) + g * 8 + 2 * t4;
#pragma unroll
        for (int J = 0; J < 2 * NW; J++) {
          if (hasB && J <= rB) *reinterpret_cast<double2*>(dstB + J * 64) = make_double2(-c0[J], -c1[J]);
          if (J < NW && hasA && J <= rA)
            *reinterpret_cast<double2*>(dstA + J * 64) = make_double2(-c0[TS - 1 - (J < NW ? J : 0)], -c1[TS - 1 - (J < NW ? J : 0)]);
        }
      }
      if (__any_sync(0xffffffffu, bad) && lane == 0) flags[3] = ST_NOT_SPD;
      __syncthreads();
    }

    HMPC_STAMP(4);
    const int vi = NT - 1 - tid;
    const int ke = 3 * wid + lane / 10;
    const bool isvar = vi < n, iscon = lane < 30 && ke < NB;
    const int erow = iscon ? 10 * ke + (lane - 10 * (lane / 10)) : 0x7fffffff;
    double xreg = 0.0;
    bool illc = false;
    if (isvar) {
      xreg = -hinv_rowdot(Hd, vi, NT8, gq);
      if (!MQ || first) illc_h = x0[vi] * Hd[toff(vi >> 3, vi >> 3) + (vi & 7) * 9] > ka.kappa_max;
      illc = illc_h;
      x0[vi] = xreg;
    }
    {
      const unsigned key = __float_as_uint(fabsf((float)xreg));
      const unsigned kmax = __reduce_max_sync(0xffffffffu, key);
      if (lane == 0) redk[16 + wid] = kmax;
    }
    if (tid < 8) amask[tid] = 0u;
    if (tid == 0) { flags[7] = 0; flags[8] = 0; flags[9] = 0; flags[11] = 0; }
    const int ill = __syncthreads_or((int)illc);
    double tol;
    {
      unsigned kx = redk[16];
      for (int w = 1; w < NW; w++) kx = redk[16 + w] > kx ? redk[16 + w] : kx;
      tol = ka.tol_kkt * fmax(1.0, (double)__uint_as_float(kx));
    }
    double ne[6] = {0.0, 0.0, 0.0, 0.0, 0.0, 0.0};
    double se = 0.0, rhs_e = 0.0;
    int nie = 0, myslot = -1;
    bool act = false;
    if (iscon) {
      const int te = lane - 10 * (lane / 10);
      nie = (blk_sl[ke] & 1) * 10 + te;
      const double* nn = nrm + nie * 6;
#pragma unroll
      for (int c = 0; c < 6; c++) ne[c] = nn[c];
      rhs_e = (te == 5) ? -(double)0.01f : ((te == 9) ? -fz[ke] : 0.0);
      se = dot6(ne, x0 + 6 * ke) - rhs_e;
    }

    int q = 0, iters = 0;
    int code = flags[3];
    if (ill && code == ST_OK) code = ST_NOT_SPD;

    if (qmax <= 31 && tcap > 0) {
      int* newslot = reinterpret_cast<int*>(rr);
      int slot_cap = (int)((sqrtf(8.f * (float)NT + 1.f) - 1.f) * 0.5f);
      while (tri(slot_cap + 1) <= NT) slot_cap++;
      while (tri(slot_cap) > NT) slot_cap--;
      slot_cap = slot_cap < tcap ? slot_cap : tcap;
      double* colb = dvs;
      const int cst = qmax + 3;
      bool warm = false;
      unsigned* wmark = reinterpret_cast<unsigned*>(redi + 16);
      if (ka.warm_start && ka.ws_state) {
        const int* ws = ka.ws_state + (size_t)inst * WS_STATE_INTS;
        const int cnt = ws[0];
        const int shift = ka.ws_shifts ? ka.ws_shifts[inst] : ka.ws_shift;
        if (shift >= 0 && cnt > 0 && cnt < WS_STATE_INTS) {
          if (tid < 16) wmark[tid] = 0u;
          __syncthreads();
          if (tid < cnt) {
            const int ent = ws[1 + tid];
            const int sl = (ent >> 8) - 2 * shift;
            if (sl >= 0 && sl < 2 * N) {
              const int kb = sl_blk[sl];
              if (kb >= 0) {
                const int e = 10 * kb + (ent & 0xff) % 10;
                atomicOr(&wmark[e >> 5], 1u << (e & 31));
              }
            }
            if ((ent >> 8) >= 2 * (N - 1)) {
              for (int sn = sl + 2; sn >= 0 && sn < 2 * N; sn += 2) {
                const int kb = sl_blk[sn];
                if (kb >= 0) {
                  const int e = 10 * kb + (ent & 0xff) % 10;
                  atomicOr(&wmark[e >> 5], 1u << (e & 31));
                }
              }
            }
          }
          __syncthreads();
          warm = true;
        }
      }
      for (int round = 0; code == ST_OK && round < ka.block_rounds; round++) {
        if (round == 0) HMPC_STAMP(8);
        const unsigned gm = (lane < 30) ? (0x3ffu << (10 * (lane / 10))) : (1u << lane);
        const float sf = (iscon && !act) ? (float)se : 3.0e38f;
        const unsigned key = fkey(sf);
        const unsigned kmin = __reduce_min_sync(gm, key);
        const unsigned tie = __ballot_sync(0xffffffffu, key == kmin) & gm;
        bool cand = iscon && !act && se < -tol && key == kmin && (__ffs(tie) - 1) == lane;
        if (warm) cand = iscon && ((wmark[erow >> 5] >> (erow & 31)) & 1u);
        const bool warm_round = warm;
        warm = false;
        const unsigned cm = __ballot_sync(0xffffffffu, cand);
        if (lane == 0) redi[wid] = __popc(cm);
        __syncthreads();
        int nadd = 0, rank = __popc(cm & ((1u << lane) - 1u));
        for (int w = 0; w < NW; w++) {
          const int c = redi[w];
          nadd += c;
          if (w < wid) rank += c;
        }
        const unsigned am0 = amask[0];
        __syncthreads();
        if (nadd == 0 || (am0 >> slot_cap) != 0u) break;
        if (round > 0 && nadd < ka.block_min) break;
        const int room = slot_cap - __popc(am0);
        if (nadd > room) nadd = room;
        if (nadd <= 0) break;
        if (rank >= nadd) cand = false;
        unsigned mybit = 0u;
        if (cand) {
          unsigned fm = ~am0;
          for (int r = 0; r < rank; r++) fm &= fm - 1;
          const int sl = __ffs(fm) - 1;
          myslot = sl;
          wsl[sl] = ws_pack(ke, nie);
          newslot[rank] = sl;
          mybit = 1u << sl;
        }
        mybit = __reduce_or_sync(0xffffffffu, mybit);
        if (lane == 0 && mybit) atomicOr(&amask[0], mybit);
        __syncthreads();
        if (round == 0) HMPC_STAMP(9);
        if (isvar) {
          for (int r = 0; r < nadd; r++) {
            const int sl = newslot[r], w = wsl[sl];
            T[sl * n + vi] = hinv_dot6(Hd, vi, 6 * (w >> 8), nrm + (w & 0xff) * 6);
          }
        }
        __syncthreads();
        if (round == 0) HMPC_STAMP(10);
        int verdict = 0;
        for (int attempt = 0; attempt < 4; attempt++) {
          const unsigned am = amask[0];
          const int qh = 32 - __clz(am);
          const bool own = tid < tri(qh);
          int i = 0, j = 0;
          double a = 0.0, bi = 0.0;
          if (own) {
            i = (int)((sqrtf(8.f * (float)tid + 1.f) - 1.f) * 0.5f);
            while (tri(i + 1) <= tid) i++;
            while (tri(i) > tid) i--;
            j = tid - tri(i);
            const bool ui = (am >> i) & 1u, uj = (am >> j) & 1u;
            a = (i == j) ? 1.0 : 0.0;
            if (ui && uj) {
              const int w = wsl[i], ki = w >> 8;
              const double* ni = nrm + (w & 0xff) * 6;
              a = dot6(ni, T + j * n + 6 * ki);
              if (i == j) {
                const int te = (w & 0xff) % 10;
                bi = ((te == 5) ? -(double)0.01f : ((te == 9) ? -fz[ki] : 0.0)) - dot6(ni, x0 + 6 * ki);
              }
            } else if (ui != uj) {
              a = 0.0;
            }
          }
          const bool diag = own && i == j;
          bool sing = false;
          if (own && j == 0) {
            colb[i] = a;
            if (i == 0) {
              colb[qh] = bi;
              colb[qh + 1] = fast_rcp(a);
              sing = !(a > 1e-13);
            }
          }
          if (round == 0 && attempt == 0) HMPC_STAMP(11);
          __syncthreads();
          for (int pv = 0; pv < qh; pv++) {
            if (own) {
              const double* cc = colb + (pv & 1) * cst;
              double* cn = colb + ((pv + 1) & 1) * cst;
              const double inv = cc[qh + 1];
              const double ci = cc[i], cj = cc[j];
              if (diag) bi = (i == pv) ? cc[qh] * inv : fma(-ci * inv, cc[qh], bi);
              if (i == pv) a = (j == pv) ? -inv : cj * inv;
              else if (j == pv) a = ci * inv;
              else a = fma(-ci * inv, cj, a);
              const int pn = pv + 1;
              if (pn < qh) {
                if (j == pn) cn[i] = a;
                else if (i == pn) cn[j] = a;
                if (diag && i == pn) {
                  cn[qh] = bi;
                  cn[qh + 1] = fast_rcp(a);
                  sing |= !(a > 1e-13);
                }
              }
            }
            __syncthreads();
          }
          if (round == 0 && attempt == 0) HMPC_STAMP(12);
          bool neg = false;
          if (own) {
            Sv[tid] = -a;
            if (diag) {
              const bool used = (am >> i) & 1u;
              lam[i] = used ? bi : 0.0;
              neg = used && !(bi > 0.0);
            }
          }
          const int anyneg = __syncthreads_or((int)neg | ((int)sing << 1));
          if (anyneg & 2) { verdict = 1; break; }
          if (!(anyneg & 1)) break;
          if (attempt == 3) { verdict = 1; break; }
          if (myslot >= 0 && !(lam[myslot] > 0.0)) {
            atomicAnd(&amask[0], ~(1u << myslot));
            myslot = -1;
            act = false;
            atomicAdd(&flags[11], 1);
          }
          __syncthreads();
        }
        if (round == 0) HMPC_STAMP(13);
        if (verdict != 0 || amask[0] == 0u) {
          __syncthreads();
          if (tid == 0) { amask[0] = 0u; flags[7] = 0; flags[8] = 0; flags[9] = 0; }
          q = 0;
          act = false;
          myslot = -1;
          if (isvar) xreg = x0[vi];
          if (iscon) se = dot6(ne, x0 + 6 * ke) - rhs_e;
          __syncthreads();
          break;
        }
        const unsigned amf = amask[0];
        const int qhf2 = 32 - __clz(amf);
        if (iscon) act = myslot >= 0;
        q = __popc(amf);
        if (!warm_round) iters += nadd;
        if (tid == 0) {
          flags[9] = qhf2;
          flags[7] = __ffs(~amf) - 1;
        }
        if (isvar) {
          double acc = x0[vi];
          for (int j = 0; j < qhf2; j++)
            if ((amf >> j) & 1u) acc = fma(lam[j], T[j * n + vi], acc);
          xreg = acc;
          zb[vi] = acc;
        }
        __syncthreads();
        if (round == 0) HMPC_STAMP(14);
        if (iscon) se = dot6(ne, zb + 6 * ke) - rhs_e;
        if (round == 0) HMPC_STAMP(15);
      }
      iters += flags[11];
    }
    HMPC_STAMP(16);
    bool noise_stop = false;
    while (code == ST_OK) {
      const float sf = (iscon && !act) ? (float)se : 3.0e38f;
      const unsigned key = fkey(sf);
      const unsigned kmin = __reduce_min_sync(0xffffffffu, key);
      const int imin = __reduce_min_sync(0xffffffffu, key == kmin ? erow : 0x7fffffff);
      if (iscon && erow == imin) redv[wid] = se;
      if (lane == 0) { redk[wid] = kmin; redi[wid] = imin; }
      __syncthreads();
      unsigned kb = redk[0];
      int p = redi[0], wb = 0;
      for (int w = 1; w < NW; w++) {
        const unsigned ok = redk[w];
        if (ok < kb) { kb = ok; p = redi[w]; wb = w; }
      }
      if (kb == fkey(3.0e38f)) break;
      double sp = redv[wb];
      if (!(sp < -tol)) break;
      const int kp = p / 10, nip = (blk_sl[kp] & 1) * 10 + (p - 10 * kp);
      const double* np_ = nrm + nip * 6;
      const int f = flags[7];
      double* Tf = T + (f < tcap ? f : tcap) * n;
      if (isvar) Tf[vi] = hinv_dot6(Hd, vi, 6 * kp, np_);
      __syncthreads();

      double lam_p = 0.0;
      while (true) {
        iters++;
        if (iters > ka.max_iter) { code = ST_ITER_CAP; break; }
        if (wid == 0) {
          const int qhi = flags[9];
          for (int s2 = lane; s2 < qhi; s2 += 32) {
            double d = 0.0;
            if ((amask[s2 >> 5] >> (s2 & 31)) & 1u) {
              const int w = wsl[s2];
              d = dot6(nrm + (w & 0xff) * 6, Tf + 6 * (w >> 8));
            }
            dvs[s2] = d;
          }
          const double cHc = dot6(np_, Tf + 6 * kp);
          __syncwarp();
          double part = 0.0, tloc = __longlong_as_double(0x7ff0000000000000ll);
          int lloc = 0x7fffffff;
          for (int s2 = lane; s2 < qhi; s2 += 32) {
            const int rs = tri(s2);
            double a0 = 0.0, a1 = 0.0;
            int j = 0;
            for (; j + 1 < qhi; j += 2) {
              a0 = fma((j <= s2) ? Sv[rs + j] : Sv[tri(j) + s2], dvs[j], a0);
              a1 = fma((j + 1 <= s2) ? Sv[rs + j + 1] : Sv[tri(j + 1) + s2], dvs[j + 1], a1);
            }
            if (j < qhi) a0 = fma((j <= s2) ? Sv[rs + j] : Sv[tri(j) + s2], dvs[j], a0);
            const double acc = a0 + a1;
            rr[s2] = acc;
            part = fma(dvs[s2], acc, part);
            if (acc > 0.0) {
              const double ratio = lam[s2] * fast_rcp(acc);
              if (ratio < tloc) { tloc = ratio; lloc = s2; }
            }
          }
#pragma unroll
          for (int o = 16; o > 0; o >>= 1) part += __shfl_xor_sync(0xffffffffu, part, o);
          const double zn = cHc - part;
          const unsigned thi = (unsigned)__double2hiint(tloc), tlo = (unsigned)__double2loint(tloc);
          const unsigned mhi = __reduce_min_sync(0xffffffffu, thi);
          const unsigned mlo = __reduce_min_sync(0xffffffffu, thi == mhi ? tlo : 0xffffffffu);
          const int l1 = __reduce_min_sync(0xffffffffu, (thi == mhi && tlo == mlo) ? lloc : 0x7fffffff);
          const double t1 = (l1 == 0x7fffffff) ? 1e300 : __hiloint2double((int)mhi, (int)mlo);
          const bool dependent = !(zn > ka.tol_dep * cHc);
          const double t2 = dependent ? 1e300 : fmax(0.0, -sp * fast_rcp(zn));
          const double t = fmin(t1, t2);
          int decision;
          if (!(t < 1e299)) decision = (-sp <= 100.0 * tol) ? 4 : 2;
          else if (t2 <= t1) decision = (q >= qmax) ? 3 : 0;
          else decision = 1;
          __syncwarp();
          if (decision < 2) {
            for (int s2 = lane; s2 < qhi; s2 += 32) lam[s2] = fmax(0.0, lam[s2] - t * rr[s2]);
          }
          int qhn = qhi;
          if (decision == 0) {
            const double izn = fast_rcp(zn);
            qhn = (f + 1 > qhi) ? f + 1 : qhi;
            for (int s2 = lane; s2 < qhn; s2 += 32) {
              const int rs = tri(s2);
              if (s2 == f) {
                for (int j = 0; j < f; j++) Sv[rs + j] = -rr[j] * izn;
                Sv[rs + f] = izn;
              } else {
                const double rs_ = rr[s2] * izn;
                for (int j = 0; j <= s2; j++) Sv[rs + j] = (j == f) ? -rs_ : fma(rs_, rr[j], Sv[rs + j]);
              }
            }
            __syncwarp();
            if (lane == 0) {
              wsl[f] = ws_pack(kp, nip);
              lam[f] = lam_p + t;
              amask[f >> 5] |= 1u << (f & 31);
            }
          } else if (decision == 1) {
            lam_p += t;
            for (int s2 = lane; s2 < qhi; s2 += 32) dvs[s2] = (s2 >= l1) ? Sv[tri(s2) + l1] : Sv[tri(l1) + s2];
            __syncwarp();
            const double ipv = fast_rcp(dvs[l1]);
            for (int s2 = lane; s2 < qhi; s2 += 32) {
              const int rs = tri(s2);
              const double cs = dvs[s2] * ipv;
              for (int j = 0; j <= s2; j++) Sv[rs + j] = (j == l1 || s2 == l1) ? 0.0 : fma(-cs, dvs[j], Sv[rs + j]);
            }
            if (lane == 0) {
              const int w = wsl[l1];
              flags[5] = (w >> 8) * 10 + ((w & 0xff) % 10);
              lam[l1] = 0.0;
              amask[l1 >> 5] &= ~(1u << (l1 & 31));
            }
          }
          __syncwarp();
          if (lane == 0) {
            flags[4] = decision;
            flags[8] = qhi;
            flags[9] = qhn;
            dsc[0] = dependent ? 0.0 : t;
            int fn = 0;
            if (qmax <= 31) fn = __ffs(~amask[0]) - 1;
            else
              while (fn < qmax && ((amask[fn >> 5] >> (fn & 31)) & 1u)) fn++;
            flags[7] = fn;
          }
        }
        __syncthreads();
        const int decision = flags[4];
        if (decision >= 2) {
          if (decision == 4) { noise_stop = true; break; }
          code = (decision == 2) ? ST_INFEASIBLE : ST_WS_CAP;
          break;
        }
        const double t = dsc[0];
        {
          const int qhe = flags[8];
          const int qc = qhe < tcap ? qhe : tcap;
          double z = 0.0;
          if (isvar) {
            double z0 = Tf[vi], z1 = 0.0;
            int j = 0;
            for (; j + 1 < qc; j += 2) {
              z0 = fma(-rr[j], T[j * n + vi], z0);
              z1 = fma(-rr[j + 1], T[(j + 1) * n + vi], z1);
            }
            if (j < qc) z0 = fma(-rr[j], T[j * n + vi], z0);
            z = z0 + z1;
          }
          if (qhe > tcap) {
            if (isvar) {
              const int kb = vi / 6, c = vi - 6 * kb;
              double acc = 0.0;
              for (int j = tcap; j < qhe; j++) {
                const int w = wsl[j];
                if ((w >> 8) == kb) acc = fma(rr[j], nrm[(w & 0xff) * 6 + c], acc);
              }
              gq[vi] = acc;
            }
            __syncthreads();
            if (isvar) z -= hinv_rowdot(Hd, vi, NT8, gq);
            __syncthreads();
          }
          if (isvar) {
            zb[vi] = z;
            xreg = fma(t, z, xreg);
          }
        }
        __syncthreads();
        if (iscon && t != 0.0) se = fma(t, dot6(ne, zb + 6 * ke), se);
        if (decision == 0) {
          if (erow == p) { act = true; myslot = f; }
          q++;
          break;
        }
        if (erow == flags[5]) { act = false; myslot = -1; }
        if (erow == p) dsc[1] = se;
        q--;
        __syncthreads();
        sp = dsc[1];
      }
      if (noise_stop) break;
    }

    HMPC_STAMP(5);
    __syncthreads();
    const int qhf = flags[9];
    const bool polish = code == ST_OK && !noise_stop;
    const int nref = (polish && q > 24) ? 2 : 0;
    for (int round = 0;; round++) {
      const bool beyond = polish && qhf > tcap;
      if (beyond) {
        if (isvar) {
          const int kb = vi / 6, c = vi - 6 * kb;
          double acc = 0.0;
          for (int j = tcap; j < qhf; j++) {
            const int w = wsl[j];
            if (((amask[j >> 5] >> (j & 31)) & 1u) && (w >> 8) == kb) acc = fma(lam[j], nrm[(w & 0xff) * 6 + c], acc);
          }
          gq[vi] = acc;
        }
        __syncthreads();
      }
      double xfin = xreg;
      if (isvar && polish) {
        xfin = x0[vi];
        const int qc = qhf < tcap ? qhf : tcap;
        for (int j = 0; j < qc; j++)
          if ((amask[j >> 5] >> (j & 31)) & 1u) xfin = fma(lam[j], T[j * n + vi], xfin);
        if (beyond) xfin += hinv_rowdot(Hd, vi, NT8, gq);
      }
      if (beyond) __syncthreads();
      if (isvar) zb[vi] = xfin;
      __syncthreads();
      if (round == nref) break;
      if (wid == 0) {
        for (int s2 = lane; s2 < qhf; s2 += 32) {
          double acc = 0.0;
          if ((amask[s2 >> 5] >> (s2 & 31)) & 1u) {
            const int w = wsl[s2], ki = w >> 8, te = (w & 0xff) % 10;
            acc = ((te == 5) ? -(double)0.01f : ((te == 9) ? -fz[ki] : 0.0)) - dot6(nrm + (w & 0xff) * 6, zb + 6 * ki);
          }
          dvs[s2] = acc;
        }
        __syncwarp();
        for (int s2 = lane; s2 < qhf; s2 += 32) {
          if (!((amask[s2 >> 5] >> (s2 & 31)) & 1u)) continue;
          const int rs = tri(s2);
          double acc = 0.0;
          for (int j = 0; j < qhf; j++) acc = fma((j <= s2) ? Sv[rs + j] : Sv[tri(j) + s2], dvs[j], acc);
          lam[s2] = fmax(0.0, lam[s2] + acc);
        }
      }
      __syncthreads();
    }

    if (ka.ws_state && wid == 0 && code != ST_WS_CAP) {
      int* ws = ka.ws_state + (size_t)inst * WS_STATE_INTS;
      const unsigned am = (code == ST_OK && qmax <= 31 && CLS != 3) ? amask[0] : 0u;
      if ((am >> lane) & 1u) {
        const int w = wsl[lane];
        ws[1 + __popc(am & ((1u << lane) - 1u))] = (blk_sl[w >> 8] << 8) | (w & 0xff);
      }
      if (lane == 0) ws[0] = __popc(am);
    }

    bool refined = false;
    if constexpr (CLS == 3) {
      const float* Hc = reinterpret_cast<const float*>(smem + L.Hc);
      const double* gc = reinterpret_cast<const double*>(smem + L.gc);
      double* xr = x0;
      double* ub = gq;
      double* yb = T;
      if (code == ST_OK) {
        if (isvar) xr[vi] = zb[vi];
        __syncthreads();
        bool conv = false, contracting = false;
        double dlast = 1e300;
        for (int round = 0; round < 4 && !conv; round++) {
          double rx = 0.0;
          if (isvar) {
            const int I = vi >> 3, ir = vi & 7;
            double hx = 0.0;
            for (int j = 0; j < n; j++) {
              const int J = j >> 3;
              const float h = (J <= I) ? Hc[toff(I, J) + ir * 8 + (j & 7)] : Hc[toff(J, I) + (j & 7) * 8 + ir];
              hx = fma((double)h, xr[j], hx);
            }
            const int kb = vi / 6, c = vi - 6 * kb;
            double atl = 0.0;
            for (int j = 0; j < qhf; j++) {
              const int w = wsl[j];
              if (((amask[j >> 5] >> (j & 31)) & 1u) && (w >> 8) == kb) atl = fma(lam[j], nrm[(w & 0xff) * 6 + c], atl);
            }
            rx = DS(DS(atl, hx), gc[vi]);
            ub[vi] = rx;
          }
          if (wid == 0) {
            for (int s2 = lane; s2 < qhf; s2 += 32) {
              double acc = 0.0;
              if ((amask[s2 >> 5] >> (s2 & 31)) & 1u) {
                const int w = wsl[s2], ki = w >> 8, te = (w & 0xff) % 10;
                acc = ((te == 5) ? -(double)0.01f : ((te == 9) ? -fz[ki] : 0.0)) - dot6(nrm + (w & 0xff) * 6, xr + 6 * ki);
              }
              dvs[s2] = acc;
            }
          }
          __syncthreads();
          if (isvar) yb[vi] = hinv_rowdot(Hd, vi, NT8, ub);
          __syncthreads();
          if (wid == 0) {
            for (int s2 = lane; s2 < qhf; s2 += 32) {
              double acc = 0.0;
              if ((amask[s2 >> 5] >> (s2 & 31)) & 1u) {
                const int w = wsl[s2];
                acc = dvs[s2] - dot6(nrm + (w & 0xff) * 6, yb + 6 * (w >> 8));
              }
              rr[s2] = acc;
            }
            __syncwarp();
            for (int s2 = lane; s2 < qhf; s2 += 32) {
              double acc = 0.0;
              if ((amask[s2 >> 5] >> (s2 & 31)) & 1u) {
                const int rs = tri(s2);
                for (int j = 0; j < qhf; j++) acc = fma((j <= s2) ? Sv[rs + j] : Sv[tri(j) + s2], rr[j], acc);
              }
              dvs[s2] = acc;
              lam[s2] += acc;
            }
          }
          __syncthreads();
          if (isvar) {
            const int kb = vi / 6, c = vi - 6 * kb;
            double acc = rx;
            for (int j = 0; j < qhf; j++) {
              const int w = wsl[j];
              if (((amask[j >> 5] >> (j & 31)) & 1u) && (w >> 8) == kb) acc = fma(dvs[j], nrm[(w & 0xff) * 6 + c], acc);
            }
            ub[vi] = acc;
          }
          __syncthreads();
          double dx = 0.0;
          if (isvar) {
            dx = hinv_rowdot(Hd, vi, NT8, ub);
            xr[vi] += dx;
          }
          {
            const unsigned km = __reduce_max_sync(0xffffffffu, __float_as_uint((float)fabs(dx)));
            if (lane == 0) redk[16 + wid] = km;
          }
          __syncthreads();
          unsigned kx = redk[16];
          for (int w = 1; w < NW; w++) kx = redk[16 + w] > kx ? redk[16 + w] : kx;
          const double dmax = (double)__uint_as_float(kx);
          contracting = dmax <= 0.5 * dlast;
          dlast = dmax;
          conv = dmax <= tol;
        }
        bool bad = !(conv || (contracting && dlast <= 1e3 * tol));
        if (iscon) bad |= dot6(ne, xr + 6 * ke) - rhs_e < -tol;
        if (wid == 0)
          for (int s2 = lane; s2 < qhf; s2 += 32) bad |= ((amask[s2 >> 5] >> (s2 & 31)) & 1u) && lam[s2] < -tol;
        refined = !__syncthreads_or((int)bad);
        if (isvar) zb[vi] = xr[vi];
        __syncthreads();
      }
      if (!refined) code = ST_NOT_SPD;
    }

    for (int e = tid; e < 12 * N; e += NT) {
      const int s = e / 12, c12 = e % 12, leg = leg_of(c12);
      const int k = sl_blk[2 * s + leg];
      const double v = (k >= 0) ? zb[6 * k + loc_of(c12)] : 0.0;
      if (ka.wrench) ka.wrench[(size_t)row * 12 * N + e] = (float)v;
      if (ka.wrench64) ka.wrench64[(size_t)row * 12 * N + e] = v;
    }
    if (ka.tau && tid < 10) {
      const float* kp_ = reinterpret_cast<const float*>(smem + L.keep);
      const int leg = tid / 5, j = tid % 5;
      const double PI = 3.14159265359;
      double q5[5];
#pragma unroll
      for (int i = 0; i < 5; i++) q5[i] = (double)kp_[5 * leg + i];
      q5[2] -= 0.3 * PI;
      q5[3] += 0.6 * PI;
      q5[4] -= 0.3 * PI;
      const double qw = kp_[10], qx = kp_[11], qy = kp_[12], qz = kp_[13];
      const double R[9] = {1 - 2 * (qy * qy + qz * qz), 2 * (qx * qy - qw * qz), 2 * (qx * qz + qw * qy),
                           2 * (qx * qy + qw * qz), 1 - 2 * (qx * qx + qz * qz), 2 * (qy * qz - qw * qx),
                           2 * (qx * qz - qw * qy), 2 * (qy * qz + qw * qx), 1 - 2 * (qx * qx + qy * qy)};
      const int k0 = sl_blk[leg];
      double fw[6] = {0, 0, 0, 0, 0, 0};
      if (k0 >= 0) {
        const double* w = zb + 6 * k0;
#pragma unroll
        for (int r = 0; r < 3; r++) {
          fw[r] = -(R[0 * 3 + r] * (double)(float)w[0] + R[1 * 3 + r] * (double)(float)w[1] + R[2 * 3 + r] * (double)(float)w[2]);
          fw[3 + r] = -(R[0 * 3 + r] * (double)(float)w[3] + R[1 * 3 + r] * (double)(float)w[4] + R[2 * 3 + r] * (double)(float)w[5]);
        }
      }
      ka.tau[(size_t)inst * 10 + tid] = (float)leg_torque(q5, leg, j, fw);
    }
    HMPC_STAMP(6);
    if (tid == 0) {
      if (code == ST_WS_CAP && ka.esc_list) {
        const int slot = atomicAdd(&ka.counts[ka.cls + 1], 1);
        ka.esc_list[slot] = row;
      }
      if (code == ST_NOT_SPD && flags[3] == ST_OK && ka.ref_list) {
        const int slot = atomicAdd(ka.ref_count, 1);
        ka.ref_list[slot] = row;
      }
      int sw = (code & 0xff) | ((iters & 0xfff) << 8) | ((q & 0xff) << 20);
      if constexpr (CLS == 3) sw |= refined ? (1 << 28) : 0;
      ka.status[row] = sw;
    }
    __syncthreads();
    if constexpr (MQ) {
      if (++kq < k1) goto next_candidate;
    }
  }
}

constexpr int SELECT_THREADS = 512;

template <int NT>
__global__ void __launch_bounds__(NT) hmpc_select_kernel(const unsigned char* mask, int batch, int* list, int* count)
{
  constexpr int NW = NT / 32;
  __shared__ int wtot[NW];
  const int tid = threadIdx.x, lane = tid & 31, wid = tid >> 5;
  pdl_trigger();
  pdl_wait();
  int base = 0;
  for (int t0 = 0; t0 < batch; t0 += NT) {
    const int i = t0 + tid;
    const bool on = i < batch && mask[i] != 0;
    const unsigned bal = __ballot_sync(0xffffffffu, on);
    if (lane == 0) wtot[wid] = __popc(bal);
    __syncthreads();
    int off = base, tot = 0;
    for (int w = 0; w < NW; w++) {
      const int n = wtot[w];
      off += w < wid ? n : 0;
      tot += n;
    }
    if (on) list[off + __popc(bal & ((1u << lane) - 1u))] = i;
    base += tot;
    __syncthreads();
  }
  if (tid == 0) *count = base;
}

constexpr int CARRY_THREADS = 256;

__global__ void __launch_bounds__(CARRY_THREADS) hmpc_carry_kernel(const unsigned char* mask, int batch, int row_vecs,
                                                                    const float4* prev, float4* cur)
{
  const long long v = (long long)blockIdx.x * blockDim.x + threadIdx.x;
  if (v >= (long long)batch * row_vecs) return;
  if (mask[v / row_vecs] == 0) cur[v] = prev[v];
}

template <bool ABS>
struct PlanRow {
  int nx, nu, xs[3], us[12];
  double ax[3], bu[12];
  __device__ __forceinline__ PlanRow(const float* Acd, const float* Bcd, int lane)
  {
    const int r = lane < 12 ? lane : 0;
    nx = r < 3 ? 3 : (r < 6 || r == 11) ? 1 : 0;
    nu = (r >= 6 && r < 9) ? 12 : (r >= 9 ? 2 : 0);
#pragma unroll
    for (int t = 0; t < 3; t++) {
      xs[t] = r < 3 ? 6 + t : (r < 6 ? r + 6 : 12);
      ax[t] = t < nx ? (double)Acd[r * 13 + xs[t]] : 0.0;
      if (ABS) ax[t] = fabs(ax[t]);
    }
#pragma unroll
    for (int t = 0; t < 12; t++) {
      us[t] = r < 9 ? t : (t == 0 ? r - 9 : r - 6);
      bu[t] = t < nu ? (double)Bcd[r * 12 + us[t]] : 0.0;
      if (ABS) bu[t] = fabs(bu[t]);
    }
  }
  __device__ __forceinline__ double step(double x, double u) const
  {
    double acc = x;
#pragma unroll
    for (int t = 0; t < 3; t++) {
      const double v = __shfl_sync(0xffffffffu, x, xs[t]);
      if (t < nx) acc = DA(acc, DM(ax[t], v));
    }
#pragma unroll
    for (int t = 0; t < 12; t++) {
      const double v = __shfl_sync(0xffffffffu, u, us[t]);
      if (t < nu) acc = DA(acc, DM(bu[t], v));
    }
    return acc;
  }
};

__device__ __forceinline__ double cost_step(double cost, double S, double Al, double x, double xd, double u)
{
  const double e = DS(x, xd);
  cost = DA(cost, DM(DM(S, e), e));
// ... 472 lines not shown
```

### hector_simulation_b200/interface.py

```python
from __future__ import annotations

import ctypes
import os

import numpy as np

from .scenarios import COMMAND_DTYPE, STATE_DTYPE, UPDATE_DTYPE

_HERE = os.path.dirname(os.path.abspath(__file__))
LIB_PATH = os.path.join(_HERE, "libhector_mpc_b200.so")

HMPC_OK, HMPC_ERR_ARG, HMPC_ERR_CUDA, HMPC_ERR_NOT_CONVERGED = 0, 1, 2, 3
ST_OK, ST_ITER_CAP, ST_WS_CAP, ST_INFEASIBLE, ST_NOT_SPD = 0, 1, 2, 3, 4

EXPORTS = [
    "setup_problem", "get_solution", "update_solver_settings", "update_problem_data",
    "hmpc_record_bytes", "hmpc_pack_records", "hmpc_create", "hmpc_destroy", "hmpc_last_error",
    "hmpc_set_problem", "hmpc_solve_batch", "hmpc_solve_device", "hmpc_launches_per_solve",
    "hmpc_assemble_device", "hmpc_class_config", "hmpc_solve_batch_ex", "hmpc_solve_device_ex",
    "hmpc_prepare_device", "hmpc_solve_batch_states", "hmpc_rollout_device", "hmpc_reset_warm_start",
    "hmpc_shard_unique_id", "hmpc_shard_init", "hmpc_solve_batch_sharded", "hmpc_shard_wait",
    "hmpc_pin_host_buffer", "hmpc_unpin_host_buffer", "hmpc_swing_device",
    "hmpc_reference_last_status", "hmpc_reference_last_rc",
    "hmpc_solve_device_warm", "hmpc_solve_batch_warm", "hmpc_reference_set_warm_start",
    "hmpc_set_refinement", "hmpc_reference_set_refinement",
    "hmpc_solve_device_masked", "hmpc_solve_batch_masked",
    "hmpc_solve_states_device_masked", "hmpc_solve_batch_states_warm", "hmpc_solve_batch_states_masked",
    "hmpc_solve_batch_sharded_warm", "hmpc_solve_batch_states_sharded_warm",
    "hmpc_predict_device", "hmpc_predict_batch", "hmpc_certify_device", "hmpc_certify_batch",
    "hmpc_solve_device_multi", "hmpc_solve_batch_multi",
    "hmpc_solve_states_device_multi", "hmpc_solve_batch_states_multi",
]
CERTIFICATE_DTYPE = np.dtype([("cost", "<f8"), ("stationarity", "<f8"), ("primal", "<f8"), ("complementarity", "<f8"),
                              ("n_active", "<i4"), ("flags", "<i4")])
CERT_PASS, CERT_NONFINITE, CERT_SWING, CERT_STATIONARITY, CERT_PRIMAL, CERT_COMPLEMENTARITY = 1, 2, 4, 8, 16, 32
REFINEMENT_CLASS = 3

SETUP_DTYPE = np.dtype([("dt", "<f4"), ("mu", "<f4"), ("f_max", "<f4"), ("horizon", "<i4")], align=True)

_lib = None


class HmpcError(RuntimeError):
    pass


def lib() -> ctypes.CDLL:
    global _lib
    if _lib is None:
        if not os.path.exists(LIB_PATH):
            raise HmpcError(f"{LIB_PATH} is missing: run `python -c 'import __graft_entry__ as g; g.build()'`")
        L = ctypes.CDLL(LIB_PATH)
        L.setup_problem.argtypes = [ctypes.c_double, ctypes.c_int, ctypes.c_double, ctypes.c_double]
        L.setup_problem.restype = None
        L.get_solution.argtypes = [ctypes.c_int]
        L.get_solution.restype = ctypes.c_double
        L.update_solver_settings.argtypes = [ctypes.c_int] + [ctypes.c_double] * 5
        L.update_solver_settings.restype = None
        dp = ctypes.POINTER(ctypes.c_double)
        L.update_problem_data.argtypes = [dp, dp, dp, dp, dp, dp, ctypes.c_double, dp, dp, dp, ctypes.POINTER(ctypes.c_int)]
        L.update_problem_data.restype = None
        L.hmpc_record_bytes.argtypes = [ctypes.c_int]
        L.hmpc_record_bytes.restype = ctypes.c_size_t
        L.hmpc_pack_records.argtypes = [ctypes.c_void_p, ctypes.c_int, ctypes.c_int, ctypes.c_void_p]
        L.hmpc_pack_records.restype = ctypes.c_int
        L.hmpc_create.argtypes = [ctypes.c_int, ctypes.c_int, ctypes.c_int]
        L.hmpc_create.restype = ctypes.c_void_p
        L.hmpc_destroy.argtypes = [ctypes.c_void_p]
        L.hmpc_destroy.restype = None
        L.hmpc_last_error.restype = ctypes.c_char_p
        L.hmpc_set_problem.argtypes = [ctypes.c_void_p, ctypes.c_void_p]
        L.hmpc_set_problem.restype = ctypes.c_int
        L.hmpc_solve_batch.argtypes = [ctypes.c_void_p, ctypes.c_void_p, ctypes.c_int, ctypes.c_void_p, ctypes.c_void_p]
        L.hmpc_solve_batch.restype = ctypes.c_int
        L.hmpc_solve_device.argtypes = [ctypes.c_void_p, ctypes.c_void_p, ctypes.c_int, ctypes.c_void_p, ctypes.c_void_p, ctypes.c_void_p]
        L.hmpc_solve_device.restype = ctypes.c_int
        L.hmpc_launches_per_solve.argtypes = [ctypes.c_void_p]
        L.hmpc_launches_per_solve.restype = ctypes.c_int
        L.hmpc_assemble_device.argtypes = [ctypes.c_void_p] * 2 + [ctypes.c_int] + [ctypes.c_void_p] * 6
        L.hmpc_assemble_device.restype = ctypes.c_int
        L.hmpc_reference_last_status.restype = ctypes.c_int
        L.hmpc_reference_last_rc.restype = ctypes.c_int
        L.hmpc_solve_batch_ex.argtypes = [ctypes.c_void_p, ctypes.c_void_p, ctypes.c_int] + [ctypes.c_void_p] * 3
        L.hmpc_solve_batch_ex.restype = ctypes.c_int
        L.hmpc_solve_device_ex.argtypes = [ctypes.c_void_p, ctypes.c_void_p, ctypes.c_int] + [ctypes.c_void_p] * 4
        L.hmpc_solve_device_ex.restype = ctypes.c_int
        L.hmpc_prepare_device.argtypes = [ctypes.c_void_p, ctypes.c_void_p, ctypes.c_int, ctypes.c_double, ctypes.c_void_p, ctypes.c_void_p]
        L.hmpc_prepare_device.restype = ctypes.c_int
        L.hmpc_solve_batch_states.argtypes = [ctypes.c_void_p, ctypes.c_void_p, ctypes.c_int, ctypes.c_double] + [ctypes.c_void_p] * 3
        L.hmpc_solve_batch_states.restype = ctypes.c_int
        L.hmpc_rollout_device.argtypes = [ctypes.c_void_p, ctypes.c_void_p, ctypes.c_void_p, ctypes.c_int, ctypes.c_int, ctypes.c_double,
                                          ctypes.c_void_p, ctypes.c_void_p, ctypes.c_void_p]
        L.hmpc_rollout_device.restype = ctypes.c_int
        L.hmpc_reset_warm_start.argtypes = [ctypes.c_void_p, ctypes.c_void_p]
        L.hmpc_reset_warm_start.restype = ctypes.c_int
        L.hmpc_shard_unique_id.argtypes = [ctypes.c_void_p]
        L.hmpc_shard_unique_id.restype = ctypes.c_int
        L.hmpc_shard_init.argtypes = [ctypes.c_void_p, ctypes.c_int, ctypes.c_int, ctypes.c_void_p]
        L.hmpc_shard_init.restype = ctypes.c_int
        L.hmpc_solve_batch_sharded.argtypes = [ctypes.c_void_p, ctypes.c_void_p, ctypes.c_int, ctypes.c_void_p, ctypes.c_void_p, ctypes.c_void_p]
        L.hmpc_solve_batch_sharded.restype = ctypes.c_int
        L.hmpc_shard_wait.argtypes = [ctypes.c_void_p]
        L.hmpc_shard_wait.restype = ctypes.c_int
        L.hmpc_pin_host_buffer.argtypes = [ctypes.c_void_p, ctypes.c_void_p, ctypes.c_size_t]
        L.hmpc_pin_host_buffer.restype = ctypes.c_int
        L.hmpc_unpin_host_buffer.argtypes = [ctypes.c_void_p, ctypes.c_void_p]
        L.hmpc_unpin_host_buffer.restype = ctypes.c_int
        L.hmpc_swing_device.argtypes = [ctypes.c_void_p] * 5 + [ctypes.c_int, ctypes.c_double, ctypes.c_double, ctypes.c_void_p, ctypes.c_void_p]
        L.hmpc_swing_device.restype = ctypes.c_int
        L.hmpc_class_config.argtypes = [ctypes.c_void_p, ctypes.c_int, ctypes.c_void_p]
        L.hmpc_class_config.restype = ctypes.c_int
        L.hmpc_solve_device_warm.argtypes = [ctypes.c_void_p, ctypes.c_void_p, ctypes.c_int] + [ctypes.c_void_p] * 5
        L.hmpc_solve_device_warm.restype = ctypes.c_int
        L.hmpc_solve_batch_warm.argtypes = [ctypes.c_void_p, ctypes.c_void_p, ctypes.c_int] + [ctypes.c_void_p] * 4
        L.hmpc_solve_batch_warm.restype = ctypes.c_int
        L.hmpc_reference_set_warm_start.argtypes = [ctypes.c_int]
        L.hmpc_reference_set_warm_start.restype = None
        L.hmpc_set_refinement.argtypes = [ctypes.c_void_p, ctypes.c_int]
        L.hmpc_set_refinement.restype = ctypes.c_int
        L.hmpc_reference_set_refinement.argtypes = [ctypes.c_int]
        L.hmpc_reference_set_refinement.restype = None
        L.hmpc_solve_device_masked.argtypes = [ctypes.c_void_p, ctypes.c_void_p, ctypes.c_int] + [ctypes.c_void_p] * 6
        L.hmpc_solve_device_masked.restype = ctypes.c_int
        L.hmpc_solve_batch_masked.argtypes = [ctypes.c_void_p, ctypes.c_void_p, ctypes.c_int] + [ctypes.c_void_p] * 5
        L.hmpc_solve_batch_masked.restype = ctypes.c_int
        L.hmpc_solve_states_device_masked.argtypes = ([ctypes.c_void_p, ctypes.c_void_p, ctypes.c_int, ctypes.c_void_p, ctypes.c_double]
                                                      + [ctypes.c_void_p] * 6)
        L.hmpc_solve_states_device_masked.restype = ctypes.c_int
        L.hmpc_solve_batch_states_warm.argtypes = [ctypes.c_void_p, ctypes.c_void_p, ctypes.c_int, ctypes.c_double] + [ctypes.c_void_p] * 4
        L.hmpc_solve_batch_states_warm.restype = ctypes.c_int
        L.hmpc_solve_batch_states_masked.argtypes = ([ctypes.c_void_p, ctypes.c_void_p, ctypes.c_int, ctypes.c_void_p, ctypes.c_double]
                                                     + [ctypes.c_void_p] * 4)
        L.hmpc_solve_batch_states_masked.restype = ctypes.c_int
        L.hmpc_solve_batch_sharded_warm.argtypes = [ctypes.c_void_p, ctypes.c_void_p, ctypes.c_int] + [ctypes.c_void_p] * 6
        L.hmpc_solve_batch_sharded_warm.restype = ctypes.c_int
        L.hmpc_solve_batch_states_sharded_warm.argtypes = ([ctypes.c_void_p, ctypes.c_void_p, ctypes.c_int, ctypes.c_void_p, ctypes.c_double]
                                                           + [ctypes.c_void_p] * 5)
        L.hmpc_solve_batch_states_sharded_warm.restype = ctypes.c_int
        L.hmpc_predict_device.argtypes = [ctypes.c_void_p, ctypes.c_void_p, ctypes.c_int] + [ctypes.c_void_p] * 4
        L.hmpc_predict_device.restype = ctypes.c_int
        L.hmpc_predict_batch.argtypes = [ctypes.c_void_p, ctypes.c_void_p, ctypes.c_int] + [ctypes.c_void_p] * 3
        L.hmpc_predict_batch.restype = ctypes.c_int
        L.hmpc_certify_device.argtypes = [ctypes.c_void_p, ctypes.c_void_p, ctypes.c_int] + [ctypes.c_void_p] * 5
        L.hmpc_certify_device.restype = ctypes.c_int
        L.hmpc_certify_batch.argtypes = [ctypes.c_void_p, ctypes.c_void_p, ctypes.c_int] + [ctypes.c_void_p] * 4
        L.hmpc_certify_batch.restype = ctypes.c_int
        L.hmpc_solve_device_multi.argtypes = [ctypes.c_void_p, ctypes.c_void_p, ctypes.c_int, ctypes.c_int] + [ctypes.c_void_p] * 6
        L.hmpc_solve_device_multi.restype = ctypes.c_int
        L.hmpc_solve_batch_multi.argtypes = [ctypes.c_void_p, ctypes.c_void_p, ctypes.c_int, ctypes.c_int] + [ctypes.c_void_p] * 5
        L.hmpc_solve_batch_multi.restype = ctypes.c_int
        L.hmpc_solve_states_device_multi.argtypes = ([ctypes.c_void_p, ctypes.c_void_p, ctypes.c_int, ctypes.c_int] + [ctypes.c_void_p] * 2
                                                     + [ctypes.c_double] + [ctypes.c_void_p] * 8)
        L.hmpc_solve_states_device_multi.restype = ctypes.c_int
        L.hmpc_solve_batch_states_multi.argtypes = ([ctypes.c_void_p, ctypes.c_void_p, ctypes.c_int, ctypes.c_int] + [ctypes.c_void_p] * 2
                                                    + [ctypes.c_double] + [ctypes.c_void_p] * 5)
        L.hmpc_solve_batch_states_multi.restype = ctypes.c_int
        _lib = L
    return _lib


def last_error() -> str:
    return lib().hmpc_last_error().decode()


def _check(rc: int, allow_not_converged: bool = False) -> int:
    if rc == HMPC_OK or (allow_not_converged and rc == HMPC_ERR_NOT_CONVERGED):
        return rc
    raise HmpcError(f"libhector_mpc_b200 rc={rc}: {last_error()}")


def setup_problem(dt: float, horizon: int, mu: float, f_max: float) -> None:
    lib().setup_problem(dt, horizon, mu, f_max)


def update_problem_data(p, v, q, w, r, joint_angles, yaw, weights, state_trajectory, Alpha_K, gait) -> None:
    def d(a):
        a = np.ascontiguousarray(a, dtype=np.float64)
        return a, a.ctypes.data_as(ctypes.POINTER(ctypes.c_double))
    keep = [d(a) for a in (p, v, q, w, r, joint_angles, weights, state_trajectory, Alpha_K)]
    g = np.ascontiguousarray(gait, dtype=np.int32)
    ptr = [k[1] for k in keep]
    lib().update_problem_data(ptr[0], ptr[1], ptr[2], ptr[3], ptr[4], ptr[5], float(yaw), ptr[6], ptr[7], ptr[8],
                              g.ctypes.data_as(ctypes.POINTER(ctypes.c_int)))


def get_solution(index: int) -> float:
    return lib().get_solution(index)


# ... 410 lines not shown
```

### include/hector_mpc_b200.h

```cpp
#ifndef HECTOR_MPC_B200_H
#define HECTOR_MPC_B200_H

#include <stddef.h>
#include <stdint.h>

#ifdef __cplusplus
#define HMPC_EXTERNC extern "C"
#else
#define HMPC_EXTERNC
#endif


#define K_MAX_GAIT_SEGMENTS 36

struct problem_setup
{
  float dt;
  float mu;
  float f_max;
  int horizon;
};

struct update_data_t
{
// ... 40 lines not shown
#define HMPC_MAX_HORIZON 16

HMPC_EXTERNC size_t hmpc_record_bytes(int horizon);
HMPC_EXTERNC int hmpc_pack_records(const struct update_data_t* in, int n, int horizon, void* out);

HMPC_EXTERNC hmpc_ctx* hmpc_create(int max_batch, int horizon, int device);
HMPC_EXTERNC void hmpc_destroy(hmpc_ctx* ctx);
HMPC_EXTERNC const char* hmpc_last_error(void);

HMPC_EXTERNC int hmpc_set_problem(hmpc_ctx* ctx, const struct problem_setup* setup);

HMPC_EXTERNC int hmpc_solve_batch(hmpc_ctx* ctx, const struct update_data_t* in, int B,
                                  double* wrench_out, int* status);

HMPC_EXTERNC int hmpc_solve_device(hmpc_ctx* ctx, const void* d_records, int B, float* d_wrench,
                                   int* d_status, void* stream);

HMPC_EXTERNC int hmpc_solve_batch_ex(hmpc_ctx* ctx, const struct update_data_t* in, int B, double* wrench_out,
                                     double* tau_out, int* status);
HMPC_EXTERNC int hmpc_solve_device_ex(hmpc_ctx* ctx, const void* d_records, int B, float* d_wrench, int* d_status,
                                      float* d_tau, void* stream);

HMPC_EXTERNC int hmpc_pin_host_buffer(hmpc_ctx* ctx, void* ptr, size_t bytes);
HMPC_EXTERNC int hmpc_unpin_host_buffer(hmpc_ctx* ctx, void* ptr);

struct hmpc_state_t
{
  double position[3];
  double vWorld[3];
  double orientation[4];
  double omegaWorld[3];
  double rpy[3];
  double leg_q[10];
  double leg_p[6];
  double state_des[5];
  double world_position_desired[2];
  unsigned char gait[K_MAX_GAIT_SEGMENTS];
  unsigned char pad[4];
};
HMPC_EXTERNC int hmpc_prepare_device(hmpc_ctx* ctx, const struct hmpc_state_t* d_states, int B, double dtMPC,
                                     void* d_records, void* stream);
HMPC_EXTERNC int hmpc_solve_batch_states(hmpc_ctx* ctx, const struct hmpc_state_t* in, int B, double dtMPC,
                                         double* wrench_out, double* tau_out, int* status);

struct hmpc_rollout_t
{
  double feet_world[6];
  int gait_offset[2];
  int gait_duration[2];
  int iteration;
  int failures;
  int iters_total;
  int ticks;
};
HMPC_EXTERNC int hmpc_reset_warm_start(hmpc_ctx* ctx, void* stream);

HMPC_EXTERNC int hmpc_solve_device_warm(hmpc_ctx* ctx, const void* d_records, int B, float* d_wrench, int* d_status,
                                        float* d_tau, const int* d_shift, void* stream);
HMPC_EXTERNC int hmpc_solve_batch_warm(hmpc_ctx* ctx, const struct update_data_t* in, int B, double* wrench_out,
                                       double* tau_out, int* status, const int* shift);
HMPC_EXTERNC int hmpc_solve_device_masked(hmpc_ctx* ctx, const void* d_records, int B, const unsigned char* d_mask,
                                          float* d_wrench, int* d_status, float* d_tau, const int* d_shift, void* stream);
HMPC_EXTERNC int hmpc_solve_batch_masked(hmpc_ctx* ctx, const struct update_data_t* in, int B, const unsigned char* mask,
                                         double* wrench_out, double* tau_out, int* status, const int* shift);
HMPC_EXTERNC int hmpc_solve_states_device_masked(hmpc_ctx* ctx, const struct hmpc_state_t* d_states, int B,
                                                 const unsigned char* d_mask, double dtMPC, void* d_records, float* d_wrench,
                                                 int* d_status, float* d_tau, const int* d_shift, void* stream);
HMPC_EXTERNC int hmpc_solve_batch_states_warm(hmpc_ctx* ctx, const struct hmpc_state_t* in, int B, double dtMPC,
                                              double* wrench_out, double* tau_out, int* status, const int* shift);
HMPC_EXTERNC int hmpc_solve_batch_states_masked(hmpc_ctx* ctx, const struct hmpc_state_t* in, int B, const unsigned char* mask,
                                                double dtMPC, double* wrench_out, double* tau_out, int* status,
                                                const int* shift);
HMPC_EXTERNC int hmpc_predict_device(hmpc_ctx* ctx, const void* d_records, int B, const unsigned char* d_mask,
                                     const float* d_wrench, float* d_pred, void* stream);
HMPC_EXTERNC int hmpc_predict_batch(hmpc_ctx* ctx, const struct update_data_t* in, int B, const unsigned char* mask,
                                    const double* wrench, double* pred_out);
typedef struct hmpc_certificate_t {
  double cost, stationarity, primal, complementarity;
  int n_active, flags;
} hmpc_certificate_t;
#define HMPC_CERT_PASS 1
#define HMPC_CERT_NONFINITE 2
#define HMPC_CERT_SWING 4
#define HMPC_CERT_STATIONARITY 8
#define HMPC_CERT_PRIMAL 16
#define HMPC_CERT_COMPLEMENTARITY 32
#define HMPC_CERT_STATIONARITY_TOL 2e-6
#define HMPC_CERT_PRIMAL_TOL 2e-7
#define HMPC_CERT_COMPLEMENTARITY_TOL 1e-9
HMPC_EXTERNC int hmpc_certify_device(hmpc_ctx* ctx, const void* d_records, int B, const unsigned char* d_mask,
                                     const float* d_wrench, hmpc_certificate_t* d_cert, float* d_lambda, void* stream);
HMPC_EXTERNC int hmpc_certify_batch(hmpc_ctx* ctx, const struct update_data_t* in, int B, const unsigned char* mask,
                                    const double* wrench, hmpc_certificate_t* cert_out, double* lambda_out);
HMPC_EXTERNC int hmpc_solve_device_multi(hmpc_ctx* ctx, const void* d_records, int B, int K, const float* d_traj,
                                         const unsigned char* d_mask, float* d_wrench, int* d_status, double* d_cost,
                                         void* stream);
HMPC_EXTERNC int hmpc_solve_batch_multi(hmpc_ctx* ctx, const struct update_data_t* in, int B, int K, const float* traj,
                                        const unsigned char* mask, double* wrench_out, int* status, double* cost_out);
HMPC_EXTERNC int hmpc_debug_last_multi_in_place(void);
struct hmpc_command_t {
  double state_des[5];
  double world_position_desired[2];
};
HMPC_EXTERNC int hmpc_solve_states_device_multi(hmpc_ctx* ctx, const struct hmpc_state_t* d_states, int B, int K,
                                                const struct hmpc_command_t* d_cmd, const unsigned char* d_mask, double dtMPC,
                                                void* d_records, float* d_traj, float* d_wrench, int* d_status, double* d_cost,
                                                int* d_best, float* d_tau, void* stream);
HMPC_EXTERNC int hmpc_solve_batch_states_multi(hmpc_ctx* ctx, const struct hmpc_state_t* in, int B, int K,
                                               const struct hmpc_command_t* cmd, const unsigned char* mask, double dtMPC,
                                               double* wrench_out, int* status, double* cost_out, int* best, double* tau_out);
HMPC_EXTERNC int hmpc_debug_last_states_multi_in_place(void);
HMPC_EXTERNC void hmpc_reference_set_warm_start(int on);
HMPC_EXTERNC int hmpc_rollout_device(hmpc_ctx* ctx, struct hmpc_state_t* d_states, struct hmpc_rollout_t* d_loop, int B,
                                     int ticks, double dtMPC, float* d_wrench_log, void* d_record_log, void* stream);

#define HMPC_SHARD_ID_BYTES 128
HMPC_EXTERNC int hmpc_shard_unique_id(void* id128);
HMPC_EXTERNC int hmpc_shard_init(hmpc_ctx* ctx, int rank, int world, const void* id128);
HMPC_EXTERNC int hmpc_solve_batch_sharded(hmpc_ctx* ctx, const update_data_t* in_local, int B_local, double* wrench_local,
                                          int* status_local, float* d_all);
HMPC_EXTERNC int hmpc_shard_wait(hmpc_ctx* ctx);
HMPC_EXTERNC int hmpc_solve_batch_sharded_warm(hmpc_ctx* ctx, const struct update_data_t* in_local, int B_local,
                                               const unsigned char* mask_local, double* wrench_local, double* tau_local,
                                               int* status_local, const int* shift_local, float* d_all);
HMPC_EXTERNC int hmpc_solve_batch_states_sharded_warm(hmpc_ctx* ctx, const struct hmpc_state_t* in_local, int B_local,
                                                      const unsigned char* mask_local, double dtMPC, double* wrench_local,
                                                      double* tau_local, int* status_local, const int* shift_local,
                                                      float* d_all);

struct hmpc_swing_t
{
  double p0[6];
  double swing_time[2];
  int first_swing[2];
};
struct hmpc_swing_cmd_t
{
  double pf[6];
  double p_des[6];
  double v_des[6];
  double q_des[10];
  int swing[2];
};
HMPC_EXTERNC int hmpc_swing_device(hmpc_ctx* ctx, const struct hmpc_state_t* d_states, const struct hmpc_rollout_t* d_loop,
                                   const double* d_phase, struct hmpc_swing_t* d_swing, int B, double dt, double dtSwing,
                                   struct hmpc_swing_cmd_t* d_cmd, void* stream);


HMPC_EXTERNC int hmpc_set_refinement(hmpc_ctx* ctx, int on);
HMPC_EXTERNC void hmpc_reference_set_refinement(int on);

HMPC_EXTERNC int hmpc_launches_per_solve(const hmpc_ctx* ctx);
#define HMPC_REFINEMENT_CLASS 3
HMPC_EXTERNC int hmpc_class_config(const hmpc_ctx* ctx, int cls, int* out);

HMPC_EXTERNC int hmpc_assemble_device(hmpc_ctx* ctx, const void* d_records, int B, float* d_H,
                                      float* d_g, float* d_Fblk, float* d_lb, float* d_ub,
                                      void* stream);

#endif
```

Before: 6.221 million.

## Add compact-smem class-0 variant so large batches fit in one wave

Adds a fixed-horizon class-0 kernel variant (128 threads, 8 CTAs/SM) that uses a compacted shared-memory layout: the last H tile row is trimmed to the real width, constraint normals are stored as float, the misc area is sized per warp count, and qmax is reduced by 4. It is launched only when the batch exceeds the normal class-0 grid capacity but fits in the larger one-wave capacity, so the tail wave is avoided. This trades a smaller active-set capacity and float normals for more resident CTAs per SM. Tile offset helpers are templated to handle the irregular last tile row.

```diff
diff --git a/hector_simulation_b200/csrc/hmpc_capi.cu b/hector_simulation_b200/csrc/hmpc_capi.cu
--- a/hector_simulation_b200/csrc/hmpc_capi.cu
+++ b/hector_simulation_b200/csrc/hmpc_capi.cu
@@ -126,6 +126,7 @@
   ClassCfg cls[3];
   int ncls = 0;
   ClassCfg ref{};
+  ClassCfg one_wave{};
   ClassCfg mcls[3], mref{};
   float* d_mq = nullptr;
   size_t mq_off[4] = {};
@@ -246,6 +247,11 @@
       mq_rows += hmpc::mq_scratch_ctas(k, c->max_batch);
     }
   }
+  if (hmpc::plan_one_wave(c->horizon, c->one_wave)) {
+    int occ = 0;
+    if (cuda_fail(prep_class(c->one_wave, &occ), "kernel attribute/occupancy (is this an sm_90a device?)")) return HMPC_ERR_CUDA;
+    c->one_wave.grid_cap = occ * c->sm_count > c->cls[0].grid_cap ? occ * c->sm_count : 0;
+  }
   if (cuda_fail(cudaMalloc(&c->d_mq, mq_rows * hmpc::mq_scratch_floats(c->horizon) * sizeof(float)), "cudaMalloc multi-query scratch"))
     return HMPC_ERR_CUDA;
   return HMPC_OK;
@@ -256,7 +262,9 @@
 int launch_class(const hmpc_ctx* c, int cls, const hmpc::SolveIO& io, const hmpc::ChainLists& lists, int count, cudaStream_t st,
                  bool pdl = false, const hmpc::MultiIO* mq = nullptr)
 {
-  const ClassCfg& k = cls == hmpc::REFINE_CLASS ? (mq ? c->mref : c->ref) : (mq ? c->mcls[cls] : c->cls[cls]);
+  const bool one_wave = cls == 0 && !mq && count > c->cls[0].grid_cap && count <= c->one_wave.grid_cap;
+  const ClassCfg& k = cls == hmpc::REFINE_CLASS ? (mq ? c->mref : c->ref)
+                                                : (mq ? c->mcls[cls] : (one_wave ? c->one_wave : c->cls[cls]));
   hmpc::KernelArgs ka = mq ? hmpc::multi_launch_args(c->cfg, c->horizon, c->ncls, cls, k, io, lists, *mq)
                            : hmpc::launch_args(c->cfg, c->horizon, c->ncls, cls, k, io, lists);
   ka.dbg_clk = ka.dbg_H ? nullptr : g_dbg_clk;
@@ -718,8 +726,9 @@
 
 HMPC_EXTERNC int hmpc_class_config(const hmpc_ctx* c, int cls, int* out)
 {
-  if (!c || !out || cls < 0 || (cls >= c->ncls && cls != HMPC_REFINEMENT_CLASS)) return HMPC_ERR_ARG;
-  const ClassCfg& k = cls == HMPC_REFINEMENT_CLASS ? c->ref : c->cls[cls];
+  if (!c || !out || cls < 0 || (cls >= c->ncls && cls != HMPC_REFINEMENT_CLASS && cls != HMPC_ONE_WAVE_CLASS))
+    return HMPC_ERR_ARG;
+  const ClassCfg& k = cls == HMPC_REFINEMENT_CLASS ? c->ref : (cls == HMPC_ONE_WAVE_CLASS ? c->one_wave : c->cls[cls]);
   out[0] = k.threads; out[1] = k.smem; out[2] = k.qmax; out[3] = k.grid_cap; out[4] = k.nb_cap;
   out[5] = 8;
   return HMPC_OK;
diff --git a/hector_simulation_b200/csrc/hmpc_chain.h b/hector_simulation_b200/csrc/hmpc_chain.h
--- a/hector_simulation_b200/csrc/hmpc_chain.h
+++ b/hector_simulation_b200/csrc/hmpc_chain.h
@@ -6,6 +6,7 @@
 constexpr int MQ_VARIANT = 100;
 #define HMPC_VARIANTS(X) \
   X(0, 128, 6, 10, 0)    \
+  X(2, 128, 8, 10, 0)    \
   X(1, 256, 2, 10, 1)    \
   X(20, 64, 1, 0, 3)     \
   X(21, 128, 1, 0, 3)    \
@@ -49,7 +50,7 @@
   Layout L;
 };
 
-inline int pick_variant(int N, int kcls, int warps, bool fixed, int* threads, bool mq = false)
+inline int pick_variant(int N, int kcls, int warps, bool fixed, int* threads, bool mq = false, bool one_wave = false)
 {
   int v = -1;
 #define HMPC_PICK(ID, NT, MB, NF, CL) \
@@ -57,7 +58,7 @@
   HMPC_VARIANTS(HMPC_PICK)
 #undef HMPC_PICK
 #define HMPC_PICK(ID, NT, MB, NF, CL) \
-  if (CL == kcls && NF == N && fixed && v >= 0) v = ID, *threads = NT;
+  if (CL == kcls && NF == N && fixed && v >= 0 && class_compact(NF, CL, NT / 32, MB) == one_wave) v = ID, *threads = NT;
   HMPC_VARIANTS(HMPC_PICK)
 #undef HMPC_PICK
   return (v >= 0 && mq) ? MQ_VARIANT + v : v;
@@ -104,6 +105,24 @@
     if (nb == N || (ref.L.total <= SMEM_MAX && ref.qmax >= class_qmax(N, 1))) break;
   }
   return ncls;
+}
+
+inline bool plan_one_wave(int N, ClassCfg& k)
+{
+  k = ClassCfg{};
+  k.nb_cap = k.nb_hi = class_nb_cap(N, 0);
+  k.variant = pick_variant(N, 0, class_warps(N, 0), true, &k.threads, false, true);
+  bool found = false;
+#define HMPC_ONE_WAVE(ID, NT, MB, NF, CL) \
+  if (ID == k.variant) found = class_compact(NF, CL, NT / 32, MB);
+  HMPC_VARIANTS(HMPC_ONE_WAVE)
+#undef HMPC_ONE_WAVE
+  if (!found) return false;
+  k.qmax = class_qmax(N, 0, true);
+  k.tcap = class_tcap(N, 0);
+  k.L = make_layout(N, k.nb_cap, k.qmax, record_stride(N), k.threads / 32, k.tcap, true);
+  k.smem = k.L.total;
+  return true;
 }
 
 struct ClassSlot {
diff --git a/hector_simulation_b200/csrc/hmpc_device.cuh b/hector_simulation_b200/csrc/hmpc_device.cuh
--- a/hector_simulation_b200/csrc/hmpc_device.cuh
+++ b/hector_simulation_b200/csrc/hmpc_device.cuh
@@ -1,6 +1,7 @@
 #pragma once
 #include <cuda_runtime.h>
 #include <stdint.h>
+#include <type_traits>
 
 namespace hmpc {
 
@@ -25,22 +26,40 @@
 
 __host__ __device__ constexpr int align16(int x) { return (x + 15) & ~15; }
 
-__host__ __device__ constexpr int toff(int I, int J) { return (I * (I + 1) / 2 + J) * 64; }
-
-__host__ __device__ constexpr Layout make_layout(int N, int nb_cap, int qmax, int rec_stride, int nwarps, int tcap)
+template <int LAST = -1, int ROWS = 8>
+__host__ __device__ constexpr int toff(int I, int J)
+{
+  if constexpr (LAST < 0) return (I * (I + 1) / 2 + J) * 64;
+  else return I * (I + 1) / 2 * 64 + J * (I == LAST ? 8 * ROWS : 64);
+}
+
+struct MiscMap {
+  int kh, redi, redv, flags, bar, dsc, amask, amask_words, wmark, wmark_words, bytes;
+};
+__host__ __device__ constexpr MiscMap misc_map(bool compact, int nwarps, int qmax)
+{
+  if (!compact) return MiscMap{16, 128, 256, 384, 448, 456, 480, 8, 192, 16, 512};
+  const int aw = (qmax + 1 + 31) / 32, o = 20 * nwarps;
+  return MiscMap{nwarps, 8 * nwarps, 12 * nwarps, o, o + 64, o + 72, o + 88, aw, 12 * nwarps, 2 * nwarps,
+                 align16(o + 88 + 4 * aw)};
+}
+
+__host__ __device__ constexpr Layout make_layout(int N, int nb_cap, int qmax, int rec_stride, int nwarps, int tcap,
+                                                 bool compact = false)
 {
   Layout L{};
   const int n = 6 * nb_cap;
   const int nt8 = (n + 7) / 8, ntile = nt8 * (nt8 + 1) / 2;
+  const int hbytes = (ntile * 64 - (compact ? nt8 * 8 * (8 * nt8 - n) : 0)) * 8;
   int o = 0;
-  L.H = o;    o += ntile * 64 * 8;
+  L.H = o;    o += hbytes;
   L.gq = o;   o += nt8 * 8 * 8;
   L.x0 = o;   o += n * 8;
-  L.nrm = o;  o += 2 * 10 * 6 * 8;
+  L.nrm = o;  o += 2 * 10 * 6 * (compact ? 4 : 8);
   L.fz = o;   o += align16(nb_cap * 8);
   L.blk = o;  o += align16((nb_cap + 2 * N) * 4);
   L.keep = o; o += 64;
-  L.misc = o; o += 512;
+  L.misc = o; o += misc_map(compact, nwarps, qmax).bytes;
   L.uni = o;
   int s = L.uni;
   const int ns = qmax + 1;
@@ -52,10 +71,10 @@
   L.wsl = s;  s += align16(ns * 4);
   L.zb = L.gq;
   const int sweep_bytes = 2 * nt8 * 64 * 8 + nwarps * 2 * 64 * 8;
-  int w = (sweep_bytes <= ntile * 64 * 8) ? L.H : L.uni;
+  int w = (sweep_bytes <= hbytes) ? L.H : L.uni;
   L.Pb = w;   w += 2 * nt8 * 64 * 8;
   L.Ws = w;   w += nwarps * 2 * 64 * 8;
-  if (sweep_bytes <= ntile * 64 * 8) w = L.uni;
+  if (sweep_bytes <= hbytes) w = L.uni;
   int a = L.uni;
   L.rec = a;  a += align16(rec_stride);
   L.x0f = a;  a += 16 * 4;
@@ -91,10 +110,10 @@
   const int t = cls == 0 ? N + 4 : (N <= 10 ? 31 : 0);
   return t < n ? t : n;
 }
-__host__ __device__ constexpr int class_qmax(int N, int cls)
+__host__ __device__ constexpr int class_qmax(int N, int cls, bool compact = false)
 {
   const int n = 6 * class_nb_cap(N, cls);
-  const int q = cls == 0 ? 2 * N + 4 : (N <= 10 ? 31 : 96);
+  const int q = cls == 0 ? 2 * N + (compact ? 0 : 4) : (N <= 10 ? 31 : 96);
   return q < n ? q : n;
 }
 __host__ __device__ constexpr int class_warps(int N, int cls)
@@ -103,9 +122,15 @@
   const int w_sweep = (nt8 + 1) / 2, w_rows = (nb + 2) / 3;
   return w_sweep > w_rows ? w_sweep : w_rows;
 }
-__host__ __device__ constexpr Layout class_layout(int N, int cls, int nwarps)
-{
-  return make_layout(N, class_nb_cap(N, cls), class_qmax(N, cls), record_stride(N), nwarps, class_tcap(N, cls));
+__host__ __device__ constexpr Layout class_layout(int N, int cls, int nwarps, bool compact = false)
+{
+  return make_layout(N, class_nb_cap(N, cls), class_qmax(N, cls, compact), record_stride(N), nwarps, class_tcap(N, cls),
+                     compact);
+}
+constexpr int SMEM_PER_SM = 228 * 1024, SMEM_RESERVED_PER_CTA = 1024;
+__host__ __device__ constexpr bool class_compact(int NF, int cls, int nwarps, int min_ctas)
+{
+  return NF > 0 && cls == 0 && min_ctas * (class_layout(NF, 0, nwarps).total + SMEM_RESERVED_PER_CTA) > SMEM_PER_SM;
 }
 
 struct KernelArgs {
@@ -191,32 +216,35 @@
 __device__ __forceinline__ int loc_of(int c12) { return (c12 % 3) + (c12 >= 6 ? 3 : 0); }
 __device__ __forceinline__ int col12_of(int leg, int loc) { return (loc < 3) ? 3 * leg + loc : 6 + 3 * leg + (loc - 3); }
 
+template <int HL = -1, int HR = 8>
 __device__ __forceinline__ void hput(float* Hf, int i, int j, float v)
 {
   const int I = i >> 3, J = j >> 3;
-  Hf[toff(I, J) + ((i & 7) << 3) + (j & 7)] = v;
-  if (I == J) Hf[toff(I, I) + ((j & 7) << 3) + (i & 7)] = v;
-}
-
-__device__ __forceinline__ double hinv_dot6(const double* Hi, int i, int j0, const double* v)
+  Hf[toff<HL, HR>(I, J) + ((i & 7) << 3) + (j & 7)] = v;
+  if (I == J) Hf[toff<HL, HR>(I, I) + ((j & 7) << 3) + (i & 7)] = v;
+}
+
+template <int HL = -1, int HR = 8, typename V>
+__device__ __forceinline__ double hinv_dot6(const double* Hi, int i, int j0, const V* v)
 {
   const int I = i >> 3, ir = i & 7;
   const int J0 = j0 >> 3, c0 = j0 & 7, J1 = J0 + 1;
   const int sA = (I >= J0) ? 1 : 8, sB = (I >= J1) ? 1 : 8;
-  const double* pA = Hi + ((I >= J0) ? toff(I, J0) + ir * 8 + c0 : toff(J0, I) + c0 * 8 + ir);
-  const double* pB = Hi + ((I >= J1) ? toff(I, J1) + ir * 8 : toff(J1, I) + ir) - (8 - c0) * sB;
+  const double* pA = Hi + ((I >= J0) ? toff<HL, HR>(I, J0) + ir * 8 + c0 : toff<HL, HR>(J0, I) + c0 * 8 + ir);
+  const double* pB = Hi + ((I >= J1) ? toff<HL, HR>(I, J1) + ir * 8 : toff<HL, HR>(J1, I) + ir) - (8 - c0) * sB;
   double acc = 0.0;
 #pragma unroll
-  for (int c = 0; c < 6; c++) acc = fma((c0 + c < 8) ? pA[c * sA] : pB[c * sB], v[c], acc);
+  for (int c = 0; c < 6; c++) acc = fma((c0 + c < 8) ? pA[c * sA] : pB[c * sB], (double)v[c], acc);
   return acc;
 }
 
+template <int HL = -1, int HR = 8>
 __device__ __forceinline__ double hinv_rowdot(const double* Hi, int i, int nt8, const double* v)
 {
   const int I = i >> 3, ir = i & 7;
   double acc0 = 0.0, acc1 = 0.0;
   for (int J = 0; J < nt8; J++) {
-    const double* p = Hi + ((J <= I) ? toff(I, J) + ir * 8 : toff(J, I) + ir);
+    const double* p = Hi + ((J <= I) ? toff<HL, HR>(I, J) + ir * 8 : toff<HL, HR>(J, I) + ir);
     const int st = (J <= I) ? 1 : 8;
     const double* vv = v + 8 * J;
 #pragma unroll
@@ -228,11 +256,12 @@
   return acc0 + acc1;
 }
 
-__device__ __forceinline__ double dot6(const double* a, const double* b)
-{
-  double acc = a[0] * b[0];
-#pragma unroll
-  for (int c = 1; c < 6; c++) acc = fma(a[c], b[c], acc);
+template <typename A>
+__device__ __forceinline__ double dot6(const A* a, const double* b)
+{
+  double acc = (double)a[0] * b[0];
+#pragma unroll
+  for (int c = 1; c < 6; c++) acc = fma((double)a[c], b[c], acc);
   return acc;
 }
 
@@ -922,35 +951,41 @@
   const int lane = tid & 31, wid = tid >> 5;
   constexpr int NW = NT / 32;
   constexpr bool FIX = NF > 0;
+  constexpr bool CMP = class_compact(NF, CLS, NW, MINB);
   const int N = FIX ? NF : ka.horizon;
   const int nb_cap = FIX ? class_nb_cap(NF, CLS) : ka.nb_cap;
-  const int qmax = FIX ? class_qmax(NF > 0 ? NF : 1, CLS) : ka.qmax;
+  const int qmax = FIX ? class_qmax(NF > 0 ? NF : 1, CLS, CMP) : ka.qmax;
   const int rec_stride = FIX ? record_stride(NF) : ka.rec_stride;
   const int tcap = FIX ? class_tcap(NF > 0 ? NF : 1, CLS) : ka.tcap;
   Layout L;
   if constexpr (FIX) {
-    constexpr Layout LC = class_layout(NF, CLS, NW);
+    constexpr Layout LC = class_layout(NF, CLS, NW, CMP);
     L = LC;
   } else {
     L = ka.L;
   }
+  constexpr int NCAP = 6 * class_nb_cap(CMP ? NF : 1, 0), HL = CMP ? (NCAP + 7) / 8 - 1 : -1, HR = CMP ? NCAP - 8 * HL : 8;
+  using NrmT = typename std::conditional<CMP, float, double>::type;
+  constexpr MiscMap MM = misc_map(CMP, NW, class_qmax(CMP ? NF : 1, 0, true));
+  static_assert(!CMP || MM.redv % 8 == 0, "misc_map: an even number of warps");
+  static_assert(!CMP || 10 * class_nb_cap(NF, 0) <= 32 * MM.wmark_words, "misc_map: the row bitmap holds every row");
   const bool dump = (ka.dbg_H != nullptr);
 
   float* Hf = reinterpret_cast<float*>(smem + L.H);
   double* Hd = reinterpret_cast<double*>(smem + L.H);
   double* gq = reinterpret_cast<double*>(smem + L.gq);
   double* x0 = reinterpret_cast<double*>(smem + L.x0);
-  double* nrm = reinterpret_cast<double*>(smem + L.nrm);
+  NrmT* nrm = reinterpret_cast<NrmT*>(smem + L.nrm);
   double* fz = reinterpret_cast<double*>(smem + L.fz);
   int* blk_sl = reinterpret_cast<int*>(smem + L.blk);
   int* sl_blk = blk_sl + nb_cap;
   unsigned* redk = reinterpret_cast<unsigned*>(smem + L.misc);
-  int* redi = reinterpret_cast<int*>(smem + L.misc + 128);
-  double* redv = reinterpret_cast<double*>(smem + L.misc + 256);
-  int* flags = reinterpret_cast<int*>(smem + L.misc + 384);
-  uint64_t* bar = reinterpret_cast<uint64_t*>(smem + L.misc + 448);
-  double* dsc = reinterpret_cast<double*>(smem + L.misc + 456);
-  unsigned* amask = reinterpret_cast<unsigned*>(smem + L.misc + 480);
+  int* redi = reinterpret_cast<int*>(smem + L.misc + MM.redi);
+  double* redv = reinterpret_cast<double*>(smem + L.misc + MM.redv);
+  int* flags = reinterpret_cast<int*>(smem + L.misc + MM.flags);
+  uint64_t* bar = reinterpret_cast<uint64_t*>(smem + L.misc + MM.bar);
+  double* dsc = reinterpret_cast<double*>(smem + L.misc + MM.dsc);
+  unsigned* amask = reinterpret_cast<unsigned*>(smem + L.misc + MM.amask);
 
   double* T = reinterpret_cast<double*>(smem + L.T);
   double* Sv = reinterpret_cast<double*>(smem + L.Sv);
@@ -1131,7 +1166,7 @@
       const int row = (t < 5) ? t : (t == 5 ? 4 : (t < 8 ? t - 1 : 7));
       const bool neg = (t == 5 || t == 6 || t == 7 || t == 9);
       const float v = Fblk[(8 * leg + row) * 12 + col];
-      nrm[e] = (double)(neg ? -v : v);
+      nrm[e] = (NrmT)(neg ? -v : v);
     }
 
     float* const mqs = MQ ? ka.mq_scratch + (size_t)blockIdx.x * mq_scratch_floats(N) : nullptr;
@@ -1301,8 +1336,8 @@
             if (!dump && delta > 0) {
               const int col = 6 * sl_blk[2 * a + li] + ci, row0 = 6 * sl_blk[2 * b + lj];
               const int I0 = row0 >> 3, r0 = row0 & 7, Jc = col >> 3, cb = col & 7;
-              float* t0 = Hf + toff(I0, Jc);
-              float* t1 = t0 + (I0 + 1) * 64;
+              float* t0 = Hf + toff<HL, HR>(I0, Jc);
+              float* t1 = (HL < 0) ? t0 + (I0 + 1) * 64 : Hf + toff<HL, HR>(I0 + 1, Jc);
 #pragma unroll
               for (int cj = 0; cj < 6; cj++) {
                 const float hv = FM(2.f, FA(acc[cj], 0.f));
@@ -1325,7 +1360,7 @@
                   oH[(size_t)(12 * b + jj) * (12 * N) + 12 * a + ii] = hv;
                 } else {
                   const int gi = 6 * ka_ + ci, gj = 6 * kb_ + cj;
-                  hput(Hf, gi > gj ? gi : gj, gi > gj ? gj : gi, hv);
+                  hput<HL, HR>(Hf, gi > gj ? gi : gj, gi > gj ? gj : gi, hv);
                 }
               }
             }
@@ -1401,25 +1436,27 @@
       double c0[TS], c1[TS];
 #pragma unroll
       for (int t = 0; t < TS; t++) { c0[t] = 0.0; c1[t] = 0.0; }
-      for (int i = tid; i < n; i += NT) x0[i] = (double)Hf[toff(i >> 3, i >> 3) + (i & 7) * 9];
+      for (int i = tid; i < n; i += NT) x0[i] = (double)Hf[toff<HL, HR>(i >> 3, i >> 3) + (i & 7) * 9];
       {
         const int i = 8 * rB + g, j = 2 * t4;
-        const float* src = Hf + toff(rB, 0) + g * 8 + 2 * t4;
+        const float* src = Hf + toff<HL, HR>(rB, 0) + g * 8 + 2 * t4;
+        const int ts = (HL >= 0 && rB == HL) ? 8 * HR : 64;
 #pragma unroll
         for (int J = 0; J < 2 * NW; J++)
           if (hasB && J <= rB) {
-            const float2 v = *reinterpret_cast<const float2*>(src + J * 64);
+            const float2 v = *reinterpret_cast<const float2*>(src + J * ts);
             c0[J] = (i < n && 8 * J + j < n) ? (double)v.x : (i == 8 * J + j ? 1.0 : 0.0);
             c1[J] = (i < n && 8 * J + j + 1 < n) ? (double)v.y : (i == 8 * J + j + 1 ? 1.0 : 0.0);
           }
       }
       {
         const int i = 8 * rA + g, j = 2 * t4;
-        const float* src = Hf + toff(rA, 0) + g * 8 + 2 * t4;
+        const float* src = Hf + toff<HL, HR>(rA, 0) + g * 8 + 2 * t4;
+        const int ts = (HL >= 0 && rA == HL) ? 8 * HR : 64;
 #pragma unroll
         for (int J = 0; J < NW; J++)
           if (hasA && J <= rA) {
-            const float2 v = *reinterpret_cast<const float2*>(src + J * 64);
+            const float2 v = *reinterpret_cast<const float2*>(src + J * ts);
             c0[TS - 1 - J] = (i < n && 8 * J + j < n) ? (double)v.x : (i == 8 * J + j ? 1.0 : 0.0);
             c1[TS - 1 - J] = (i < n && 8 * J + j + 1 < n) ? (double)v.y : (i == 8 * J + j + 1 ? 1.0 : 0.0);
           }
@@ -1553,13 +1590,16 @@
         if (k == 0) HMPC_STAMP(19);
       }
       {
-        double* dstB = Hd + toff(rB, 0) + g * 8 + 2 * t4;
-        double* dstA = Hd + toff(rA, 0) + g * 8 + 2 * t4;
+        double* dstB = Hd + toff<HL, HR>(rB, 0) + g * 8 + 2 * t4;
+        double* dstA = Hd + toff<HL, HR>(rA, 0) + g * 8 + 2 * t4;
+        const bool shortB = HL >= 0 && rB == HL, shortA = HL >= 0 && rA == HL;
+        const bool stB = hasB && (!shortB || g < HR), stA = hasA && (!shortA || g < HR);
+        const int tsB = shortB ? 8 * HR : 64, tsA = shortA ? 8 * HR : 64;
 #pragma unroll
         for (int J = 0; J < 2 * NW; J++) {
-          if (hasB && J <= rB) *reinterpret_cast<double2*>(dstB + J * 64) = make_double2(-c0[J], -c1[J]);
-          if (J < NW && hasA && J <= rA)
-            *reinterpret_cast<double2*>(dstA + J * 64) = make_double2(-c0[TS - 1 - (J < NW ? J : 0)], -c1[TS - 1 - (J < NW ? J : 0)]);
+          if (stB && J <= rB) *reinterpret_cast<double2*>(dstB + J * tsB) = make_double2(-c0[J], -c1[J]);
+          if (J < NW && stA && J <= rA)
+            *reinterpret_cast<double2*>(dstA + J * tsA) = make_double2(-c0[TS - 1 - (J < NW ? J : 0)], -c1[TS - 1 - (J < NW ? J : 0)]);
         }
       }
       if (__any_sync(0xffffffffu, bad) && lane == 0) flags[3] = ST_NOT_SPD;
@@ -1574,23 +1614,23 @@
     double xreg = 0.0;
     bool illc = false;
     if (isvar) {
-      xreg = -hinv_rowdot(Hd, vi, NT8, gq);
-      if (!MQ || first) illc_h = x0[vi] * Hd[toff(vi >> 3, vi >> 3) + (vi & 7) * 9] > ka.kappa_max;
+      xreg = -hinv_rowdot<HL, HR>(Hd, vi, NT8, gq);
+      if (!MQ || first) illc_h = x0[vi] * Hd[toff<HL, HR>(vi >> 3, vi >> 3) + (vi & 7) * 9] > ka.kappa_max;
       illc = illc_h;
       x0[vi] = xreg;
     }
     {
       const unsigned key = __float_as_uint(fabsf((float)xreg));
       const unsigned kmax = __reduce_max_sync(0xffffffffu, key);
-      if (lane == 0) redk[16 + wid] = kmax;
-    }
-    if (tid < 8) amask[tid] = 0u;
+      if (lane == 0) redk[MM.kh + wid] = kmax;
+    }
+    if (tid < MM.amask_words) amask[tid] = 0u;
     if (tid == 0) { flags[7] = 0; flags[8] = 0; flags[9] = 0; flags[11] = 0; }
     const int ill = __syncthreads_or((int)illc);
     double tol;
     {
-      unsigned kx = redk[16];
-      for (int w = 1; w < NW; w++) kx = redk[16 + w] > kx ? redk[16 + w] : kx;
+      unsigned kx = redk[MM.kh];
+      for (int w = 1; w < NW; w++) kx = redk[MM.kh + w] > kx ? redk[MM.kh + w] : kx;
       tol = ka.tol_kkt * fmax(1.0, (double)__uint_as_float(kx));
     }
     double ne[6] = {0.0, 0.0, 0.0, 0.0, 0.0, 0.0};
@@ -1600,7 +1640,7 @@
     if (iscon) {
       const int te = lane - 10 * (lane / 10);
       nie = (blk_sl[ke] & 1) * 10 + te;
-      const double* nn = nrm + nie * 6;
+      const NrmT* nn = nrm + nie * 6;
 #pragma unroll
       for (int c = 0; c < 6; c++) ne[c] = nn[c];
       rhs_e = (te == 5) ? -(double)0.01f : ((te == 9) ? -fz[ke] : 0.0);
@@ -1620,13 +1660,13 @@
       double* colb = dvs;
       const int cst = qmax + 3;
       bool warm = false;
-      unsigned* wmark = reinterpret_cast<unsigned*>(redi + 16);
+      unsigned* wmark = reinterpret_cast<unsigned*>(smem + L.misc + MM.wmark);
       if (ka.warm_start && ka.ws_state) {
         const int* ws = ka.ws_state + (size_t)inst * WS_STATE_INTS;
         const int cnt = ws[0];
         const int shift = ka.ws_shifts ? ka.ws_shifts[inst] : ka.ws_shift;
         if (shift >= 0 && cnt > 0 && cnt < WS_STATE_INTS) {
-          if (tid < 16) wmark[tid] = 0u;
+          if (tid < MM.wmark_words) wmark[tid] = 0u;
           __syncthreads();
           if (tid < cnt) {
             const int ent = ws[1 + tid];
@@ -1697,7 +1737,7 @@
         if (isvar) {
           for (int r = 0; r < nadd; r++) {
             const int sl = newslot[r], w = wsl[sl];
-            T[sl * n + vi] = hinv_dot6(Hd, vi, 6 * (w >> 8), nrm + (w & 0xff) * 6);
+            T[sl * n + vi] = hinv_dot6<HL, HR>(Hd, vi, 6 * (w >> 8), nrm + (w & 0xff) * 6);
           }
         }
         __syncthreads();
@@ -1718,7 +1758,7 @@
             a = (i == j) ? 1.0 : 0.0;
             if (ui && uj) {
               const int w = wsl[i], ki = w >> 8;
-              const double* ni = nrm + (w & 0xff) * 6;
+              const NrmT* ni = nrm + (w & 0xff) * 6;
               a = dot6(ni, T + j * n + 6 * ki);
               if (i == j) {
                 const int te = (w & 0xff) % 10;
@@ -1840,10 +1880,10 @@
       double sp = redv[wb];
       if (!(sp < -tol)) break;
       const int kp = p / 10, nip = (blk_sl[kp] & 1) * 10 + (p - 10 * kp);
-      const double* np_ = nrm + nip * 6;
+      const NrmT* np_ = nrm + nip * 6;
       const int f = flags[7];
       double* Tf = T + (f < tcap ? f : tcap) * n;
-      if (isvar) Tf[vi] = hinv_dot6(Hd, vi, 6 * kp, np_);
+      if (isvar) Tf[vi] = hinv_dot6<HL, HR>(Hd, vi, 6 * kp, np_);
       __syncthreads();
 
       double lam_p = 0.0;
@@ -1978,12 +2018,12 @@
               double acc = 0.0;
               for (int j = tcap; j < qhe; j++) {
                 const int w = wsl[j];
-                if ((w >> 8) == kb) acc = fma(rr[j], nrm[(w & 0xff) * 6 + c], acc);
+                if ((w >> 8) == kb) acc = fma(rr[j], (double)nrm[(w & 0xff) * 6 + c], acc);
               }
               gq[vi] = acc;
             }
             __syncthreads();
-            if (isvar) z -= hinv_rowdot(Hd, vi, NT8, gq);
+            if (isvar) z -= hinv_rowdot<HL, HR>(Hd, vi, NT8, gq);
             __syncthreads();
           }
           if (isvar) {
@@ -2020,7 +2060,7 @@
           double acc = 0.0;
           for (int j = tcap; j < qhf; j++) {
             const int w = wsl[j];
-            if (((amask[j >> 5] >> (j & 31)) & 1u) && (w >> 8) == kb) acc = fma(lam[j], nrm[(w & 0xff) * 6 + c], acc);
+            if (((amask[j >> 5] >> (j & 31)) & 1u) && (w >> 8) == kb) acc = fma(lam[j], (double)nrm[(w & 0xff) * 6 + c], acc);
           }
           gq[vi] = acc;
         }
@@ -2032,7 +2072,7 @@
         const int qc = qhf < tcap ? qhf : tcap;
         for (int j = 0; j < qc; j++)
           if ((amask[j >> 5] >> (j & 31)) & 1u) xfin = fma(lam[j], T[j * n + vi], xfin);
-        if (beyond) xfin += hinv_rowdot(Hd, vi, NT8, gq);
+        if (beyond) xfin += hinv_rowdot<HL, HR>(Hd, vi, NT8, gq);
       }
       if (beyond) __syncthreads();
       if (isvar) zb[vi] = xfin;
@@ -2095,7 +2135,7 @@
             double atl = 0.0;
             for (int j = 0; j < qhf; j++) {
               const int w = wsl[j];
-              if (((amask[j >> 5] >> (j & 31)) & 1u) && (w >> 8) == kb) atl = fma(lam[j], nrm[(w & 0xff) * 6 + c], atl);
+              if (((amask[j >> 5] >> (j & 31)) & 1u) && (w >> 8) == kb) atl = fma(lam[j], (double)nrm[(w & 0xff) * 6 + c], atl);
             }
             rx = DS(DS(atl, hx), gc[vi]);
             ub[vi] = rx;
@@ -2111,7 +2151,7 @@
             }
           }
           __syncthreads();
-          if (isvar) yb[vi] = hinv_rowdot(Hd, vi, NT8, ub);
+          if (isvar) yb[vi] = hinv_rowdot<HL, HR>(Hd, vi, NT8, ub);
           __syncthreads();
           if (wid == 0) {
             for (int s2 = lane; s2 < qhf; s2 += 32) {
@@ -2139,23 +2179,23 @@
             double acc = rx;
             for (int j = 0; j < qhf; j++) {
               const int w = wsl[j];
-              if (((amask[j >> 5] >> (j & 31)) & 1u) && (w >> 8) == kb) acc = fma(dvs[j], nrm[(w & 0xff) * 6 + c], acc);
+              if (((amask[j >> 5] >> (j & 31)) & 1u) && (w >> 8) == kb) acc = fma(dvs[j], (double)nrm[(w & 0xff) * 6 + c], acc);
             }
             ub[vi] = acc;
           }
           __syncthreads();
           double dx = 0.0;
           if (isvar) {
-            dx = hinv_rowdot(Hd, vi, NT8, ub);
+            dx = hinv_rowdot<HL, HR>(Hd, vi, NT8, ub);
             xr[vi] += dx;
           }
           {
             const unsigned km = __reduce_max_sync(0xffffffffu, __float_as_uint((float)fabs(dx)));
-            if (lane == 0) redk[16 + wid] = km;
+            if (lane == 0) redk[MM.kh + wid] = km;
           }
           __syncthreads();
-          unsigned kx = redk[16];
-          for (int w = 1; w < NW; w++) kx = redk[16 + w] > kx ? redk[16 + w] : kx;
+          unsigned kx = redk[MM.kh];
+          for (int w = 1; w < NW; w++) kx = redk[MM.kh + w] > kx ? redk[MM.kh + w] : kx;
           const double dmax = (double)__uint_as_float(kx);
           contracting = dmax <= 0.5 * dlast;
           dlast = dmax;
diff --git a/hector_simulation_b200/interface.py b/hector_simulation_b200/interface.py
--- a/hector_simulation_b200/interface.py
+++ b/hector_simulation_b200/interface.py
@@ -35,6 +35,7 @@
                               ("n_active", "<i4"), ("flags", "<i4")])
 CERT_PASS, CERT_NONFINITE, CERT_SWING, CERT_STATIONARITY, CERT_PRIMAL, CERT_COMPLEMENTARITY = 1, 2, 4, 8, 16, 32
 REFINEMENT_CLASS = 3
+ONE_WAVE_CLASS = 4
 
 SETUP_DTYPE = np.dtype([("dt", "<f4"), ("mu", "<f4"), ("f_max", "<f4"), ("horizon", "<i4")], align=True)
 
diff --git a/include/hector_mpc_b200.h b/include/hector_mpc_b200.h
--- a/include/hector_mpc_b200.h
+++ b/include/hector_mpc_b200.h
@@ -216,6 +216,7 @@
 
 HMPC_EXTERNC int hmpc_launches_per_solve(const hmpc_ctx* ctx);
 #define HMPC_REFINEMENT_CLASS 3
+#define HMPC_ONE_WAVE_CLASS 4
 HMPC_EXTERNC int hmpc_class_config(const hmpc_ctx* ctx, int cls, int* out);
 
 HMPC_EXTERNC int hmpc_assemble_device(hmpc_ctx* ctx, const void* d_records, int B, float* d_H,
```

After: 6.909 million, median of 6. +11.1%, better.
